# virtuoso/clap

Hardware: AMD Instinct MI355X
Metric: entity updates/sec (transform hierarchy + inverse + AABB + frustum cull + visible list) (higher is better)
Workload: dtype f32; 1 GPU; BASELINE configs[1]: 1000000 entities/GPU, 125000 chains x depth 8, tiles SoA layout, all dirty, fused frustum cull + ordered visible list (303309 visible); entities_per_gpu=1000000, levels=8, particles_per_gpu=0, exchange=none

## Files before the change

### clap_amd/_lib.py

```python
import ctypes as C
import os
import subprocess

_HERE = os.path.dirname(os.path.abspath(__file__))
LIB_PATH = os.environ.get("CLAPGPU_LIB") or os.path.join(_HERE, "lib", "libclapgpu.so")
CSRC = os.path.join(_HERE, "csrc")
ABI_VERSION = 34

OK = 0
ERR_NOMEM = -1
ERR_INVALID_ARGUMENTS = -2
ERR_NOT_SUPPORTED = -3
ERR_TOO_LARGE = -11
ERR_INIT_FAILED = -14
ERR_OUT_OF_BOUNDS = -26
ERR_UNKNOWN = -32

E_VISIBLE = 1 << 0
E_SKIP_CULLING = 1 << 14
E_DIRTY = 1 << 16
E_JOINT_ATTACHED = 1 << 17
E_ALIVE = 1 << 31
RAY_INVALID = 1 << 0
RAY_UNRESOLVED = 1 << 1
RAY_MOVED_TARGET = 1 << 2
UPDATE_ALL_DIRTY = 1 << 0

_ERR_NAMES = {ERR_NOMEM: "NOMEM", ERR_INVALID_ARGUMENTS: "INVALID_ARGUMENTS", ERR_NOT_SUPPORTED: "NOT_SUPPORTED",
              ERR_TOO_LARGE: "TOO_LARGE", ERR_INIT_FAILED: "INITIALIZATION_FAILED",
              ERR_OUT_OF_BOUNDS: "OUT_OF_BOUNDS", ERR_UNKNOWN: "UNKNOWN_ERROR"}


class ClapGpuError(RuntimeError):
    def __init__(self, code, where, detail=""):
        self.code = code
        super().__init__(f"{where}: CERR_{_ERR_NAMES.get(code, code)} ({code}) {detail}".rstrip())


class Frustum(C.Structure):
    _fields_ = [("planes", C.c_float * 24), ("corners", C.c_float * 32)]


class BvQuery(C.Structure):
    _fields_ = [("cam_pos", C.c_float * 3), ("has_ctl", C.c_uint32), ("ctl_pos", C.c_float * 3),
                ("ctl_entity", C.c_uint32), ("result", C.c_void_p), ("inside_mask", C.c_void_p)]


EXTRA_VIEWS_MAX = 4


class Views(C.Structure):
    _fields_ = [("n", C.c_uint32), ("pad", C.c_uint32), ("frustum", Frustum * EXTRA_VIEWS_MAX),
                ("vis_mask", C.c_void_p * EXTRA_VIEWS_MAX), ("vis_row_pop", C.c_void_p * EXTRA_VIEWS_MAX),
                ("host_vis_mask", C.c_void_p * EXTRA_VIEWS_MAX)]


class Entities(C.Structure):
    _fields_ = [("n", C.c_uint32), ("n_models", C.c_uint32),
                ("pos_scale", C.c_void_p), ("rot", C.c_void_p), ("parent", C.c_void_p),
                ("model", C.c_void_p), ("model_table", C.c_void_p), ("flags", C.c_void_p),
                ("seqs", C.c_void_p), ("mx", C.c_void_p), ("inv_mx", C.c_void_p),
                ("aabb", C.c_void_p), ("center", C.c_void_p), ("vis_mask", C.c_void_p),
                ("vis_row_pop", C.c_void_p), ("n_attach", C.c_uint32), ("pad", C.c_uint32),
                ("attach", C.c_void_p), ("jt_pool", C.c_void_p), ("bind_pool", C.c_void_p),
                ("attach_local", C.c_void_p), ("bv", C.POINTER(BvQuery)), ("rebuilt_mask", C.c_void_p),
                ("views", C.POINTER(Views))]


class Particles(C.Structure):
    _fields_ = [("n", C.c_uint32), ("n_sys", C.c_uint32), ("sys", C.c_void_p), ("row_sys", C.c_void_p),
                ("pos", C.c_void_p), ("vel", C.c_void_p), ("rng_state", C.c_void_p),
                ("billboard_mx", C.c_void_p), ("respawn_mask", C.c_void_p), ("respawn_row_pop", C.c_void_p),
                ("respawn_list", C.c_void_p), ("respawn_count", C.c_void_p), ("scratch", C.c_void_p),
                ("respawn_groups", C.c_void_p)]


class AnimClock(C.Structure):
    _fields_ = [("n_chars", C.c_uint32), ("n_anims", C.c_uint32), ("anim", C.c_void_p), ("time_end", C.c_void_p),
                ("ani_time", C.c_void_p), ("speed", C.c_void_p), ("restart", C.c_void_p), ("frame_time", C.c_void_p),
                ("ended", C.c_void_p)]


class Skeleton(C.Structure):
    _fields_ = [("nr_joints", C.c_uint32), ("n_levels", C.c_uint32), ("parent", C.c_void_p), ("depth", C.c_void_p),
                ("root_pose", C.c_void_p), ("invmx", C.c_void_p), ("bind", C.c_void_p)]


class Animations(C.Structure):
    _fields_ = [("n_anims", C.c_uint32), ("n_times", C.c_uint32), ("chan_table", C.c_void_p),
                ("times", C.c_void_p), ("data", C.c_void_p), ("packed", C.c_void_p), ("packed_keys", C.c_uint32),
                ("packed_layout", C.c_uint32), ("n_data", C.c_uint32), ("pad", C.c_uint32)]


class PoseBatch(C.Structure):
    _fields_ = [("n_chars", C.c_uint32), ("skip", C.c_uint32), ("anim", C.c_void_p), ("frame_time", C.c_void_p), ("entity", C.c_void_p),
                ("entity_mx", C.c_void_p), ("trs", C.c_void_p), ("joint_transforms", C.c_void_p),
                ("joint_pos", C.c_void_p)]


class SkinBatch(C.Structure):
    _fields_ = [("n_chars", C.c_uint32), ("nr_joints", C.c_uint32), ("vert_first", C.c_void_p),
                ("vert_count", C.c_void_p), ("out_first", C.c_void_p), ("position", C.c_void_p),
                ("normal", C.c_void_p), ("joints", C.c_void_p), ("weights", C.c_void_p),
                ("joint_transforms", C.c_void_p), ("out_position", C.c_void_p), ("out_normal", C.c_void_p),
                ("out_w", C.c_void_p)]


class World(C.Structure):
    _fields_ = [("gravity", C.c_double * 3), ("linear_damping", C.c_double),
                ("linear_damping_threshold_sq", C.c_double), ("adis_linear_threshold_sq", C.c_double),
                ("adis_angular_threshold_sq", C.c_double), ("adis_time", C.c_double),
                ("adis_steps", C.c_int32), ("pad", C.c_int32)]


class Bodies(C.Structure):
    _fields_ = [("n", C.c_uint32), ("adis_average_samples", C.c_uint32), ("pos", C.c_void_p), ("quat", C.c_void_p),
                ("lvel", C.c_void_p), ("avel", C.c_void_p), ("mass", C.c_void_p), ("radius", C.c_void_p),
                ("yoffset", C.c_void_p), ("bflags", C.c_void_p), ("adis_steps_left", C.c_void_p),
                ("adis_time_left", C.c_void_p), ("body_entity", C.c_void_p),
                ("length", C.c_void_p), ("inertia", C.c_void_p), ("geom_offset_R", C.c_double * 12),
                ("aabb", C.c_void_p), ("axis", C.c_void_p), ("adis_samples", C.c_void_p), ("adis_counter", C.c_void_p),
                ("geom_records", C.c_void_p)]


class Geoms(C.Structure):
    _fields_ = [("n", C.c_uint32), ("pad", C.c_uint32), ("pos", C.c_void_p), ("axis", C.c_void_p),
                ("radius", C.c_void_p), ("length", C.c_void_p), ("kind", C.c_void_p), ("aabb", C.c_void_p),
                ("material", C.c_void_p), ("records", C.c_void_p)]


class TrimeshDesc(C.Structure):
    _fields_ = [("n_meshes", C.c_uint32), ("n_statics", C.c_uint32), ("static_index", C.c_void_p), ("vx_first", C.c_void_p),
                ("tri_first", C.c_void_p), ("vx", C.c_void_p), ("idx", C.c_void_p), ("scale", C.c_void_p),
                ("pos", C.c_void_p), ("quat", C.c_void_p)]


POSE_SKIP_TRS, POSE_SKIP_JOINT_POS, POSE_JOINT_POS_MODEL = 1, 2, 4
BODY_DISABLED, BODY_AUTO_DISABLE, BODY_NO_GRAVITY, BODY_GYROSCOPIC, BODY_HAS_JOINT = 1, 2, 4, 8, 16
GEOM_SPHERE, GEOM_CAPSULE, GEOM_BOX, GEOM_OTHER = 0, 1, 2, 3
CONTACT_DEEP = 0x80000000


def mesh_contact_scratch(static_capacity):
    return (int(static_capacity) + 63) // 64 + 1


class Characters(C.Structure):
    _fields_ = [("n", C.c_uint32), ("limbo_height", C.c_float), ("entity", C.c_void_p), ("body", C.c_void_p),
                ("hist_pos", C.c_void_p), ("hist_head", C.c_void_p), ("hist_wrapped", C.c_void_p),
                ("airborne", C.c_void_p), ("moved", C.c_void_p)]


class Lights(C.Structure):
    _fields_ = [("nr_lights", C.c_uint32), ("pad", C.c_uint32), ("pos", C.c_void_p), ("color", C.c_void_p),
                ("attenuation", C.c_void_p), ("is_dir", C.c_void_p), ("active", C.c_void_p)]


class Frame(C.Structure):
    _fields_ = [("entities", C.POINTER(Entities)), ("tile_row_start", C.c_void_p), ("n_tiles", C.c_uint32),
                ("level_start", C.c_void_p), ("n_levels", C.c_uint32), ("frustum", C.POINTER(Frustum)),
                ("bodies", C.POINTER(Bodies)), ("world", C.POINTER(World)), ("bp", C.c_void_p),
                ("pairs", C.c_void_p), ("pair_capacity", C.c_uint32), ("pair_total", C.c_void_p),
                ("static_pairs", C.c_void_p), ("static_pair_capacity", C.c_uint32), ("static_pair_total", C.c_void_p),
                ("body_geoms", C.POINTER(Geoms)), ("static_geoms", C.POINTER(Geoms)),
                ("contacts", C.c_void_p), ("static_contacts", C.c_void_p),
                ("contact_total", C.c_void_p), ("static_contact_total", C.c_void_p),
                ("n_body_links", C.c_uint32), ("link_body", C.c_void_p), ("link_entity", C.c_void_p),
                ("characters", C.POINTER(Characters)),
                ("lights", C.POINTER(Lights)),
                ("n_light_carriers", C.c_uint32), ("carrier_entity", C.c_void_p), ("carrier_light", C.c_void_p),
                ("carrier_offset", C.c_void_p),
                ("light_width", C.c_uint32), ("light_height", C.c_uint32), ("light_cell", C.c_uint32), ("light_tiles", C.c_void_p),
                ("view_mx", C.POINTER(C.c_float)), ("proj_mx", C.POINTER(C.c_float)),
                ("anim_clock", C.POINTER(AnimClock)), ("now_dev", C.c_void_p),
                ("skeleton", C.POINTER(Skeleton)), ("animations", C.POINTER(Animations)), ("pose", C.POINTER(PoseBatch)),
                ("skin", C.POINTER(SkinBatch)),
                ("particles", C.POINTER(Particles)),
                ("index_base", C.c_uint32), ("visible", C.c_void_p), ("visible_count", C.c_void_p), ("visible_scratch", C.c_void_p),
                ("cam_pos", C.c_float * 3), ("force_lod", C.c_void_p), ("cur_lod", C.c_void_p), ("draw_lod", C.c_void_p),
                ("flags", C.c_uint32),
                ("meshes", C.c_void_p), ("mesh_contacts", C.c_void_p), ("mesh_ref", C.c_void_p),
                ("mesh_contact_capacity", C.c_uint32), ("mesh_contact_total", C.c_void_p), ("mesh_capped", C.c_void_p),
                ("mesh_scratch", C.c_void_p)]


LIGHTS_MAX = 128


SYMBOLS = {
    "clapgpu_device_count": (C.c_int, []),
    "clapgpu_init": (C.c_int, [C.c_int]),
    "clapgpu_last_error": (C.c_char_p, []),
    "clapgpu_test_fail_after": (None, [C.c_int]),
    "clapgpu_abi_version": (C.c_uint32, []),
    "clapgpu_malloc": (C.c_int, [C.POINTER(C.c_void_p), C.c_size_t]),
    "clapgpu_free": (C.c_int, [C.c_void_p]),
    "clapgpu_host_malloc": (C.c_int, [C.POINTER(C.c_void_p), C.c_size_t]),
    "clapgpu_host_free": (C.c_int, [C.c_void_p]),
    "clapgpu_memcpy_h2d": (C.c_int, [C.c_void_p, C.c_void_p, C.c_size_t, C.c_void_p]),
    "clapgpu_memcpy_d2h": (C.c_int, [C.c_void_p, C.c_void_p, C.c_size_t, C.c_void_p]),
    "clapgpu_memset": (C.c_int, [C.c_void_p, C.c_int, C.c_size_t, C.c_void_p]),
    "clapgpu_stream_sync": (C.c_int, [C.c_void_p]),
    "clapgpu_view_matrix": (None, [C.POINTER(C.c_float), C.POINTER(C.c_float), C.POINTER(C.c_float)]),
    "clapgpu_perspective": (None, [C.c_float, C.c_float, C.c_float, C.c_float, C.c_int, C.POINTER(C.c_float)]),
    "clapgpu_frustum_calc": (None, [C.POINTER(C.c_float), C.POINTER(C.c_float), C.c_int, C.POINTER(Frustum)]),
    "clapgpu_entities_update": (C.c_int, [C.c_void_p, C.POINTER(Entities), C.POINTER(C.c_uint32), C.c_uint32,
                                          C.c_uint32, C.POINTER(Frustum)]),
    "clapgpu_entities_update_level": (C.c_int, [C.c_void_p, C.POINTER(Entities), C.c_uint32, C.c_uint32,
                                                C.c_uint32, C.POINTER(Frustum)]),
    "clapgpu_entities_update_tiles": (C.c_int, [C.c_void_p, C.POINTER(Entities), C.c_void_p, C.c_uint32,
                                                C.c_uint32, C.POINTER(Frustum)]),
    "clapgpu_entities_lod": (C.c_int, [C.c_void_p, C.POINTER(Entities), C.c_void_p, C.c_void_p, C.c_uint32,
                                       C.POINTER(C.c_float), C.c_void_p, C.c_void_p, C.c_void_p]),
    "clapgpu_entities_cull": (C.c_int, [C.c_void_p, C.POINTER(Entities), C.POINTER(Frustum)]),
    "clapgpu_visible_scratch_bytes": (C.c_size_t, [C.c_uint32]),
    "clapgpu_visible_compact": (C.c_int, [C.c_void_p, C.c_void_p, C.c_void_p, C.c_uint32, C.c_uint32, C.c_void_p,
                                          C.c_void_p, C.c_void_p]),
    "clapgpu_animation_time": (C.c_int, [C.c_void_p, C.POINTER(AnimClock), C.c_double]),
    "clapgpu_animation_time_dev": (C.c_int, [C.c_void_p, C.POINTER(AnimClock), C.c_void_p]),
    "clapgpu_animations_packed_bytes": (C.c_size_t, [C.c_uint32, C.c_uint32, C.c_uint32]),
    "clapgpu_animations_pack": (C.c_int, [C.c_void_p, C.POINTER(Animations), C.c_uint32, C.c_uint32, C.c_void_p, C.POINTER(C.c_uint32)]),
    "clapgpu_joint_pos_world": (C.c_int, [C.c_void_p, C.POINTER(Skeleton), C.POINTER(PoseBatch)]),
    "clapgpu_pose_update": (C.c_int, [C.c_void_p, C.POINTER(Skeleton), C.POINTER(Animations), C.POINTER(PoseBatch)]),
    "clapgpu_skin": (C.c_int, [C.c_void_p, C.POINTER(SkinBatch)]),
    "clapgpu_phys_step_schedule": (C.c_int, [C.POINTER(C.c_double), C.c_double]),
    "clapgpu_world_defaults": (None, [C.POINTER(World)]),
    "clapgpu_bodies_step": (C.c_int, [C.c_void_p, C.POINTER(Bodies), C.POINTER(World), C.c_double]),
    "clapgpu_phys_body_update": (C.c_int, [C.c_void_p, C.POINTER(Bodies), C.c_uint32, C.c_void_p, C.c_void_p, C.c_void_p,
                                           C.c_void_p]),
    "clapgpu_geom_offset_rotation": (None, [C.POINTER(C.c_double)]),
    "clapgpu_mass_sphere_total": (None, [C.c_double, C.c_double, C.POINTER(C.c_double)]),
    "clapgpu_mass_capsule_total": (None, [C.c_double, C.c_int, C.c_double, C.c_double, C.POINTER(C.c_double)]),
    "clapgpu_capsule_geom": (None, [C.c_float, C.c_float, C.c_float, C.c_double, C.c_double, C.POINTER(C.c_float),
                                    C.POINTER(C.c_float), C.POINTER(C.c_float), C.POINTER(C.c_int), C.POINTER(C.c_float)]),
    "clapgpu_bodies_aabb": (C.c_int, [C.c_void_p, C.POINTER(Bodies)]),
    "clapgpu_bp_create": (C.c_int, [C.POINTER(C.c_void_p), C.c_uint32, C.c_double, C.c_uint32, C.c_void_p]),
    "clapgpu_bp_destroy": (None, [C.c_void_p]),
    "clapgpu_bp_collide": (C.c_int, [C.c_void_p, C.c_void_p, C.c_uint32, C.c_void_p, C.c_void_p, C.c_uint32, C.c_void_p,
                                     C.c_void_p, C.c_uint32, C.c_void_p]),
    "clapgpu_bp_status": (C.c_int, [C.c_void_p, C.c_void_p, C.POINTER(C.c_uint32)]),
    "clapgpu_bp_static_aabb": (C.c_void_p, [C.c_void_p]),
    "clapgpu_contacts_geoms": (C.c_int, [C.c_void_p, C.POINTER(Geoms), C.POINTER(Geoms), C.c_void_p, C.c_void_p, C.c_uint32,
                                         C.c_void_p, C.c_void_p, C.c_void_p, C.c_void_p]),
    "clapgpu_contacts_geoms_both": (C.c_int, [C.c_void_p, C.c_void_p, C.POINTER(Geoms), C.POINTER(Geoms), C.c_void_p, C.c_void_p,
                                              C.c_uint32, C.c_void_p, C.c_void_p, C.c_void_p, C.c_void_p, C.c_uint32, C.c_void_p,
                                              C.c_void_p, C.c_void_p]),
    "clapgpu_sweep_capsules": (C.c_int, [C.c_void_p, C.POINTER(Geoms), C.POINTER(Geoms), C.c_uint32, C.c_void_p, C.c_void_p,
                                         C.c_void_p, C.c_void_p, C.c_void_p, C.c_void_p, C.c_void_p]),
    "clapgpu_bodies_rotate_from_entities": (C.c_int, [C.c_void_p, C.POINTER(Bodies), C.POINTER(Entities), C.c_uint32,
                                                      C.c_uint32, C.c_void_p, C.c_void_p]),
    "clapgpu_contacts_spheres": (C.c_int, [C.c_void_p, C.POINTER(Bodies), C.c_void_p, C.c_void_p, C.c_uint32,
                                           C.c_void_p, C.c_void_p, C.c_void_p]),
    "clapgpu_contacts_sphere_box": (C.c_int, [C.c_void_p, C.POINTER(Bodies), C.c_uint32, C.c_void_p, C.c_void_p,
                                              C.c_void_p, C.c_uint32, C.c_void_p, C.c_void_p, C.c_void_p, C.c_void_p]),
    "clapgpu_shard_tile_range": (C.c_int, [C.c_void_p, C.c_uint32, C.c_uint32, C.c_uint32, C.POINTER(C.c_uint32),
                                           C.POINTER(C.c_uint32)]),
    "clapgpu_bodies_step_prebin": (C.c_int, [C.c_void_p, C.POINTER(Bodies), C.POINTER(World), C.c_double, C.c_void_p]),
    "clapgpu_bp_invalidate": (C.c_int, [C.c_void_p, C.c_void_p]),
    "clapgpu_bp_index": (C.c_int, [C.c_void_p, C.c_void_p, C.c_uint32, C.c_void_p]),
    "clapgpu_bp_index_status": (C.c_int, [C.c_void_p, C.c_void_p, C.POINTER(C.c_uint32)]),
    "clapgpu_ray_cast": (C.c_int, [C.c_void_p, C.c_void_p, C.POINTER(Geoms), C.POINTER(Geoms), C.c_uint32, C.c_void_p,
                                   C.c_void_p, C.c_void_p, C.c_void_p, C.c_void_p, C.c_void_p]),
    "clapgpu_bodies_ground_collide": (C.c_int, [C.c_void_p, C.c_void_p, C.POINTER(Bodies), C.POINTER(Geoms), C.c_uint32,
                                                C.c_void_p, C.c_void_p, C.c_void_p, C.c_void_p, C.c_void_p, C.c_void_p,
                                                C.c_void_p, C.c_void_p, C.c_void_p]),
    "clapgpu_trimesh_create": (C.c_int, [C.c_void_p, C.POINTER(C.c_void_p), C.POINTER(TrimeshDesc)]),
    "clapgpu_trimesh_pose": (C.c_int, [C.c_void_p, C.c_void_p, C.c_void_p, C.c_void_p]),
    "clapgpu_trimesh_status": (C.c_int, [C.c_void_p, C.c_void_p, C.POINTER(C.c_uint32), C.POINTER(C.c_uint32)]),
    "clapgpu_trimesh_destroy": (None, [C.c_void_p]),
    "clapgpu_ray_cast_meshes": (C.c_int, [C.c_void_p, C.c_void_p, C.POINTER(Geoms), C.POINTER(Geoms), C.c_void_p, C.c_uint32,
                                          C.c_void_p, C.c_void_p, C.c_void_p, C.c_void_p, C.c_void_p, C.c_void_p]),
    "clapgpu_bodies_ground_collide_meshes": (C.c_int, [C.c_void_p, C.c_void_p, C.POINTER(Bodies), C.POINTER(Geoms), C.c_void_p,
                                                       C.c_uint32, C.c_void_p, C.c_void_p, C.c_void_p, C.c_void_p, C.c_void_p,
                                                       C.c_void_p, C.c_void_p, C.c_void_p, C.c_void_p]),
    "clapgpu_contacts_meshes": (C.c_int, [C.c_void_p, C.POINTER(Geoms), C.POINTER(Geoms), C.c_void_p, C.c_void_p, C.c_void_p,
                                          C.c_uint32, C.c_void_p, C.c_uint32, C.c_void_p, C.c_void_p, C.c_void_p, C.c_void_p,
                                          C.c_void_p]),
    "clapgpu_sweep_capsules_meshes": (C.c_int, [C.c_void_p, C.POINTER(Geoms), C.POINTER(Geoms), C.c_void_p, C.c_uint32, C.c_void_p,
                                                C.c_void_p, C.c_void_p, C.c_void_p, C.c_void_p, C.c_void_p, C.c_void_p]),
    "clapgpu_visible_compact_lod": (C.c_int, [C.c_void_p, C.c_void_p, C.c_uint32, C.c_void_p, C.c_void_p, C.c_void_p, C.c_void_p,
                                              C.c_void_p, C.c_void_p, C.c_void_p]),
    "clapgpu_characters_update_clock": (C.c_int, [C.c_void_p, C.c_void_p, C.c_void_p, C.c_void_p, C.c_void_p, C.c_double, C.c_void_p]),
    "clapgpu_host_malloc_mapped": (C.c_int, [C.POINTER(C.c_void_p), C.POINTER(C.c_void_p), C.c_size_t]),
    "clapgpu_entities_apply_inputs": (C.c_int, [C.c_void_p, C.c_void_p, C.c_void_p, C.c_uint32]),
    "clapgpu_entities_place": (C.c_int, [C.c_void_p, C.c_void_p, C.c_void_p, C.c_uint32, C.c_void_p]),
    "clapgpu_entities_export_rebuilt": (C.c_int, [C.c_void_p, C.c_void_p, C.c_void_p]),
    "clapgpu_entities_export_rows": (C.c_int, [C.c_void_p, C.c_void_p, C.c_void_p, C.c_void_p]),
    "clapgpu_entities_update_tiles_hostio": (C.c_int, [C.c_void_p, C.c_void_p, C.c_void_p, C.c_uint32, C.c_uint32, C.c_void_p,
                                                       C.c_void_p]),
    "clapgpu_wait_word": (C.c_int, [C.c_void_p, C.c_uint32, C.c_void_p]),
    "clapgpu_exchange_set_library": (None, [C.c_char_p]),
    "clapgpu_exchange_available": (C.c_int, []),
    "clapgpu_exchange_unique_id": (C.c_int, [C.c_void_p]),
    "clapgpu_exchange_create": (C.c_int, [C.POINTER(C.c_void_p), C.c_void_p, C.c_int, C.c_int]),
    "clapgpu_exchange_info": (C.c_int, [C.c_void_p, C.POINTER(C.c_int), C.POINTER(C.c_int), C.c_char_p]),
    "clapgpu_exchange_destroy": (None, [C.c_void_p]),
    "clapgpu_exchange_visible": (C.c_int, [C.c_void_p, C.c_void_p, C.c_void_p, C.c_uint32, C.c_void_p, C.c_void_p, C.c_void_p,
                                           C.c_void_p]),
    "clapgpu_exchange_visible_ranges": (C.c_int, [C.c_void_p, C.c_void_p, C.c_void_p, C.c_uint32, C.c_void_p, C.c_void_p, C.c_void_p,
                                                  C.c_void_p, C.c_void_p, C.c_void_p]),
    "clapgpu_visible_compact_ranges": (C.c_int, [C.c_void_p, C.c_void_p, C.c_uint32, C.c_uint32, C.c_void_p, C.c_void_p, C.c_void_p,
                                                 C.c_void_p, C.c_void_p]),
    "clapgpu_visible_expand_ranges_host": (C.c_uint32, [C.c_void_p, C.c_uint32, C.c_uint32, C.c_void_p, C.c_void_p, C.c_void_p, C.c_uint32]),
    "clapgpu_shard_bases": (C.c_int, [C.c_void_p, C.c_uint32, C.c_uint32, C.c_void_p, C.c_void_p, C.POINTER(C.c_uint32)]),
    "clapgpu_mat4_invert": (None, [C.POINTER(C.c_float), C.POINTER(C.c_float)]),
    "clapgpu_mat4_from_quat": (None, [C.POINTER(C.c_float), C.POINTER(C.c_float)]),
    "clapgpu_frame_issue": (C.c_int, [C.c_void_p, C.POINTER(Frame), C.c_double, C.c_uint32]),
    "clapgpu_particles_update": (C.c_int, [C.c_void_p, C.POINTER(Particles), C.POINTER(C.c_float)]),
    "clapgpu_characters_update": (C.c_int, [C.c_void_p, C.POINTER(Characters), C.POINTER(Entities),
                                            C.POINTER(Bodies)]),
    "clapgpu_light_grid_dims": (None, [C.c_uint32, C.c_uint32, C.c_uint32, C.POINTER(C.c_uint32),
                                       C.POINTER(C.c_uint32)]),
    "clapgpu_light_grid_compute": (C.c_int, [C.c_void_p, C.POINTER(Lights), C.POINTER(C.c_float),
                                             C.POINTER(C.c_float), C.c_uint32, C.c_uint32, C.c_uint32, C.c_void_p]),
    "clapgpu_lights_from_entities": (C.c_int, [C.c_void_p, C.POINTER(Entities), C.c_uint32, C.c_uint32, C.c_void_p,
                                               C.c_void_p, C.c_void_p, C.POINTER(Lights)]),
}

_lib = None


def build(verbose=False):
    subprocess.run(["make", "-C", CSRC] + ([] if verbose else ["-s"]), check=True)


def lib():
    global _lib
    if _lib is None:
        if not os.path.exists(LIB_PATH):
            raise ClapGpuError(ERR_INIT_FAILED, "clap_amd",
                               f"{LIB_PATH} is missing: run `python -c 'import __graft_entry__ as g; g.build()'` "
                               "(there is no CPU fallback)")
        try:
            import torch
        except ImportError:
            pass
        L = C.CDLL(LIB_PATH)
        for name, (res, args) in SYMBOLS.items():
            fn = getattr(L, name)
            fn.restype = res
            fn.argtypes = args
        got = L.clapgpu_abi_version()
        if got & 0x80000000 and os.environ.get("CLAPGPU_ALLOW_EXPERIMENT") == "1":
            got &= 0x7FFFFFFF
        if got != ABI_VERSION:
            raise ClapGpuError(ERR_INIT_FAILED, "clap_amd",
                               "libclapgpu ABI version mismatch; rebuild" if not got & 0x80000000 else
                               "libclapgpu is an EXPERIMENT build (-DCLAPGPU_EXPERIMENT: kernels compiled with parts "
                               "switched off); rebuild without EXTRA=, or set CLAPGPU_ALLOW_EXPERIMENT=1 for an A/B run")
        _lib = L
    return _lib


def check(rc, where):
    if rc != OK:
        detail = lib().clapgpu_last_error()
        raise ClapGpuError(rc, where, detail.decode() if detail else "")
```

### clap_amd/csrc/entities.hip

```cpp
#include <string.h>
#include <math.h>
#include <type_traits>
#include "common.h"
#include "lm_dev.h"
#include "entities_row.h"

namespace clapgpu {

template <bool CULL, bool XV = false>
__device__ __forceinline__ void process_row_fast(const EntK &e, const RowIn &in, float4 *tile, const float4 *mt,
                                                 const int lane, const uint32_t row_first, const uint32_t mode,
                                                 const lmd::FrustumK &fr, const int src, const uint32_t parent_seq_now,
                                                 float (&carry_mx)[16], uint32_t &carry_seq, const XViewsK *xv = nullptr)
{
    const uint32_t i = row_first + lane;
    const uint32_t fl = in.fl;
    const int32_t p = in.p;
    uint32_t seq = in.sq & 0xffffu, pseq = in.sq >> 16;
    float pm[16];
#pragma unroll
    for (int k = 0; k < 16; k++) pm[k] = __shfl(carry_mx[k], src);
    if (p >= 0) pseq = parent_seq_now;

    const float4 lo = mt[2 * in.mi], hi = mt[2 * in.mi + 1];
    float mx[16], inv[16], bb[6], ctr[3], local_mx[16];
    lmd::trs(local_mx, in.ps.x, in.ps.y, in.ps.z, in.ps.w, in.q.x, in.q.y, in.q.z, in.q.w);
    if (p >= 0) {
        lmd::mul(mx, pm, local_mx);
    } else {
#pragma unroll
        for (int k = 0; k < 16; k++) mx[k] = local_mx[k];
    }
#ifdef CLAPGPU_EXP_NO_INVERT
#pragma unroll
    for (int k = 0; k < 16; k++) inv[k] = mx[k];
#else
    lmd::invert(inv, mx);
#endif
#ifdef CLAPGPU_EXP_NO_AABB
#pragma unroll
    for (int k = 0; k < 6; k++) bb[k] = mx[12 + k % 3] + (k < 3 ? lo.x : hi.x);
#pragma unroll
    for (int k = 0; k < 3; k++) ctr[k] = mx[12 + k];
#else
    lmd::world_aabb(bb, ctr, mx, lo.x, lo.y, lo.z, hi.x, hi.y, hi.z);
#endif
    seq = (seq + 1) & 0xffffu;
#pragma unroll
    for (int k = 0; k < 16; k++) carry_mx[k] = mx[k];
    carry_seq = seq;

    const size_t e0 = row_first;
    float4 *tile_a = tile, *tile_b = tile + 256;
    float *tile_f = reinterpret_cast<float *>(tile);
    float4 va[4], vb[4];
    stage_mat4(tile_a, mx, lane);
    stage_mat4(tile_b, inv, lane);
    wave_lds_fence();
    unstage_mat4(tile_a, va, lane);
    unstage_mat4(tile_b, vb, lane);
    store_mat4_rows(e.mx + 16 * e0, va, lane, WAVE);
    store_mat4_rows(e.inv_mx + 16 * e0, vb, lane, WAVE);
    e.seqs[i] = seq | (pseq << 16);
    wave_lds_fence();
    stage_rows<6>(tile_f, bb, lane);
    wave_lds_fence();
    {
        float *ab = e.aabb + 6 * e0;
        store_stream(&reinterpret_cast<float4 *>(ab)[lane], reinterpret_cast<const float4 *>(tile_f)[lane]);
        const float2 t2 = reinterpret_cast<const float2 *>(tile_f + 4 * WAVE)[lane];
        const clapgpu_f2 v2 = { t2.x, t2.y };
        const clapgpu_f3 v3 = { ctr[0], ctr[1], ctr[2] };
#ifdef CLAPGPU_PLAIN_STORES
        reinterpret_cast<clapgpu_f2 *>(ab + 4 * WAVE)[lane] = v2;
        *reinterpret_cast<clapgpu_f3 *>(e.center + 3 * (e0 + lane)) = v3;
#else
        __builtin_nontemporal_store(v2, reinterpret_cast<clapgpu_f2 *>(ab + 4 * WAVE) + lane);
        __builtin_nontemporal_store(v3, reinterpret_cast<clapgpu_f3 *>(e.center + 3 * (e0 + lane)));
#endif
    }
    wave_lds_fence();
    if (!(mode & CLAPGPU_UPDATE_ALL_DIRTY) && (fl & CLAPGPU_E_DIRTY))
        e.flags[i] = fl & ~CLAPGPU_E_DIRTY;
    if (e.rebuilt_mask && lane == 0) e.rebuilt_mask[row_first >> 6] = ~0ull;
    if (CULL) {
        bool vis = (fl & CLAPGPU_E_VISIBLE) != 0;
        if (vis && !(fl & CLAPGPU_E_SKIP_CULLING))
            vis = lmd::aabb_in_frustum_fast(fr, bb);
        const uint64_t m = __ballot(vis);
        e.vis_mask[e0 >> 6] = m;
        e.vis_row_pop[e0 >> 6] = (uint8_t)__popcll(m);
        if constexpr (XV) cull_extra_views(*xv, (fl & CLAPGPU_E_VISIBLE) != 0, fl, bb, (uint32_t)(e0 >> 6), lane);
    }
}

__global__ __launch_bounds__(ENT_BLOCK)
void k_attach_prepare(EntK e)
{
    const uint32_t k = blockIdx.x * ENT_BLOCK + threadIdx.x;
    if (k >= e.n_attach) return;
    const clapgpu_attach at = e.attach[k];
    const float4 ps = e.pos_scale[at.entity], q = e.rot[at.entity];
    float local_mx[16], jt[16], bd[16], joint_mx[16], out[16];
    lmd::trs(local_mx, ps.x, ps.y, ps.z, ps.w, q.x, q.y, q.z, q.w);
    load_mat4(jt, e.jt_pool + 16 * (size_t)at.jt);
    load_mat4(bd, e.bind_pool + 16 * (size_t)at.bind);
    lmd::mul(joint_mx, jt, bd);
    lmd::mul(out, joint_mx, local_mx);
    float4 *d = reinterpret_cast<float4 *>(e.attach_local + 16 * (size_t)k);
#pragma unroll
    for (int c = 0; c < 4; c++)
        d[c] = make_float4(out[4 * c], out[4 * c + 1], out[4 * c + 2], out[4 * c + 3]);
}


template <bool CULL>
__global__ __launch_bounds__(ENT_BLOCK)
void k_entities_level(EntK e, uint32_t first, uint32_t count, uint32_t mode, lmd::FrustumK fr)
{
    __shared__ float4 lds_tiles[ENT_BLOCK / WAVE][LDS_F4_PER_WAVE];
    const int lane = lane_id();
    const int wave = threadIdx.x / WAVE;
    const uint32_t wave_local0 = blockIdx.x * ENT_BLOCK + wave * WAVE;
    if (wave_local0 >= count)
        return;
    const uint32_t row_count = count - wave_local0 < WAVE ? count - wave_local0 : WAVE;
    float carry_mx[16];
    uint32_t carry_seq = 0;
    bool carry_valid = false;
    const RowIn in = load_row(e, lane, first + wave_local0, row_count);
    process_row<CULL, false>(e, in, lds_tiles[wave], lane, first + wave_local0, row_count, mode, fr,
                             false, 0, carry_mx, carry_seq, carry_valid);
}

constexpr int ENT_MT_CAP = 256;
constexpr int ENT_TILE_WAVES = 1;
template <bool CULL>
__global__ __launch_bounds__(ENT_BLOCK, ENT_TILE_WAVES)
void k_entities_tiles(lmd::FrustumK fr_arg, EntK e, const uint32_t *tile_row_start, uint32_t n_tiles, uint32_t n,
                      uint32_t mode)
{
#define TILES_XV 0
#define TILES_XV_PTR nullptr
#include "entities_tiles_body.inc"
#undef TILES_XV
#undef TILES_XV_PTR
}

__global__ __launch_bounds__(ENT_BLOCK, ENT_TILE_WAVES)
void k_entities_tiles_xv(lmd::FrustumK fr_arg, EntK e, const uint32_t *tile_row_start, uint32_t n_tiles, uint32_t n,
                         uint32_t mode, XViewsK xv)
{
    constexpr bool CULL = true;
#define TILES_XV 1
#define TILES_XV_PTR (&xv)
#include "entities_tiles_body.inc"
#undef TILES_XV
#undef TILES_XV_PTR
}

__global__ __launch_bounds__(ENT_BLOCK)
void k_entities_level_xv(EntK e, uint32_t first, uint32_t count, uint32_t mode, lmd::FrustumK fr, XViewsK xv)
{
    __shared__ float4 lds_tiles[ENT_BLOCK / WAVE][LDS_F4_PER_WAVE];
    const int lane = lane_id();
    const int wave = threadIdx.x / WAVE;
    const uint32_t wave_local0 = blockIdx.x * ENT_BLOCK + wave * WAVE;
    if (wave_local0 >= count)
        return;
    const uint32_t row_count = count - wave_local0 < WAVE ? count - wave_local0 : WAVE;
    float carry_mx[16];
    uint32_t carry_seq = 0;
    bool carry_valid = false;
    const RowIn in = load_row(e, lane, first + wave_local0, row_count);
    process_row<true, false, false, true>(e, in, lds_tiles[wave], lane, first + wave_local0, row_count, mode, fr,
                                          false, 0, carry_mx, carry_seq, carry_valid, nullptr, nullptr, &xv);
}

__global__ __launch_bounds__(ENT_BLOCK)
void k_entities_cull_xv(const uint32_t *flags, const float *aabb, uint64_t *vis_mask, uint8_t *vis_row_pop,
                        uint32_t n, lmd::FrustumK fr, XViewsK xv)
{
    const uint32_t i = blockIdx.x * ENT_BLOCK + threadIdx.x;
    const int lane = lane_id();
    bool base = false, vis = false;
    uint32_t fl = 0;
    float bb[6] = { 0, 0, 0, 0, 0, 0 };
    if (i < n) {
        fl = flags[i];
        base = (fl & CLAPGPU_E_ALIVE) && (fl & CLAPGPU_E_VISIBLE);
        vis = base;
        if (base && !(fl & CLAPGPU_E_SKIP_CULLING)) {
#pragma unroll
            for (int k = 0; k < 6; k++) bb[k] = aabb[6 * (size_t)i + k];
            vis = lmd::aabb_in_frustum_fast(fr, bb);
        }
    }
    if ((i - lane) >= n) return;
    const uint64_t m = __ballot(vis);
    if (lane == 0) {
        vis_mask[i >> 6] = m;
        vis_row_pop[i >> 6] = (uint8_t)__popcll(m);
    }
    cull_extra_views(xv, base, fl, bb, i >> 6, lane);
}

__global__ __launch_bounds__(ENT_BLOCK)
void k_entities_cull(const uint32_t *flags, const float *aabb, uint64_t *vis_mask, uint8_t *vis_row_pop,
                     uint32_t n, lmd::FrustumK fr)
{
    const uint32_t i = blockIdx.x * ENT_BLOCK + threadIdx.x;
    bool vis = false;
    if (i < n) {
        const uint32_t fl = flags[i];
        vis = (fl & CLAPGPU_E_ALIVE) && (fl & CLAPGPU_E_VISIBLE);
        if (vis && !(fl & CLAPGPU_E_SKIP_CULLING)) {
            float bb[6];
#pragma unroll
            for (int k = 0; k < 6; k++) bb[k] = aabb[6 * (size_t)i + k];
            vis = lmd::aabb_in_frustum_fast(fr, bb);
        }
    }
    const uint64_t m = __ballot(vis);
    if (lane_id() == 0 && (i - lane_id()) < n) {
        vis_mask[i >> 6] = m;
        vis_row_pop[i >> 6] = (uint8_t)__popcll(m);
    }
}

constexpr int GROUP_WORDS = 64;

__device__ __forceinline__ uint64_t load_mask_word(const uint64_t *vis_mask, uint32_t w, uint32_t n)
{
    const uint32_t nwords = (n + 63) / 64;
    if (w >= nwords)
        return 0;
    uint64_t v = vis_mask[w];
    const uint32_t rem = n - w * 64;
    if (rem < 64)
        v &= (1ull << rem) - 1ull;
    return v;
}

__device__ __forceinline__ uint32_t wave_sum(uint32_t v)
{
#pragma unroll
    for (int off = 32; off > 0; off >>= 1)
        v += __shfl_xor(v, off);
    return v;
}

__global__ __launch_bounds__(WAVE)
void k_mask_group_count(const uint64_t *vis_mask, uint32_t n, uint32_t *group_count)
{
    const uint32_t w = blockIdx.x * GROUP_WORDS + threadIdx.x;
    const uint32_t c = wave_sum(__popcll(load_mask_word(vis_mask, w, n)));
    if (threadIdx.x == 0)
        group_count[blockIdx.x] = c;
}

__global__ __launch_bounds__(WAVE)
void k_visible_expand(const uint64_t *vis_mask, uint32_t n, const uint32_t *group_count,
                      uint32_t n_groups, uint32_t index_base, uint32_t *visible, uint32_t *count)
{
    const int lane = threadIdx.x;
    const uint32_t g = blockIdx.x;

    uint32_t pre = 0;
    for (uint32_t j = lane; j < g; j += WAVE)
        pre += group_count[j];
    pre = wave_sum(pre);

    const uint64_t word = load_mask_word(vis_mask, g * GROUP_WORDS + lane, n);
    const uint32_t cnt = __popcll(word);
    uint32_t incl = cnt;
#pragma unroll
    for (int off = 1; off < WAVE; off <<= 1) {
        uint32_t t = __shfl_up(incl, off);
        if (lane >= off) incl += t;
    }
    const uint32_t excl = incl - cnt;

    for (int k = 0; k < GROUP_WORDS; k++) {
        const uint64_t wk = __shfl(word, k);
        if (wk == 0) continue;
        const uint32_t base = pre + __shfl(excl, k);
        if ((wk >> lane) & 1ull) {
            const uint32_t rank = __popcll(wk & ((1ull << lane) - 1ull));
            visible[base + rank] = index_base + (g * GROUP_WORDS + k) * 64u + lane;
        }
    }
    if (g == n_groups - 1 && lane == WAVE - 1)
        *count = pre + incl;
}

constexpr int MAX_SEGMENTS = 64;
struct SegK { uint32_t cap_words, n_seg; uint32_t base[MAX_SEGMENTS], n_words[MAX_SEGMENTS]; };

__device__ __forceinline__ uint64_t load_seg_word(const uint64_t *mask, const SegK &sg, uint32_t w, uint32_t *id_base)
{
    const uint32_t r = w / sg.cap_words, lw = w - r * sg.cap_words;
    if (r >= sg.n_seg || lw >= sg.n_words[r]) { *id_base = 0; return 0ull; }
    *id_base = sg.base[r] + lw * 64u;
    return mask[w];
}

__global__ __launch_bounds__(WAVE)
void k_mask_group_count_seg(const uint64_t *mask, SegK sg, uint32_t *group_count)
{
    uint32_t idb;
    const uint32_t c = wave_sum(__popcll(load_seg_word(mask, sg, blockIdx.x * GROUP_WORDS + threadIdx.x, &idb)));
    if (threadIdx.x == 0)
        group_count[blockIdx.x] = c;
}

__global__ __launch_bounds__(WAVE)
void k_visible_expand_seg(const uint64_t *mask, SegK sg, const uint32_t *group_count, uint32_t n_groups, uint32_t *visible,
                          uint32_t *count)
{
    const int lane = threadIdx.x;
    const uint32_t g = blockIdx.x;
    uint32_t pre = 0;
    for (uint32_t j = lane; j < g; j += WAVE)
        pre += group_count[j];
    pre = wave_sum(pre);
    uint32_t idb;
    const uint64_t word = load_seg_word(mask, sg, g * GROUP_WORDS + lane, &idb);
    const uint32_t cnt = __popcll(word);
    uint32_t incl = cnt;
#pragma unroll
    for (int off = 1; off < WAVE; off <<= 1) {
        uint32_t t = __shfl_up(incl, off);
        if (lane >= off) incl += t;
    }
    const uint32_t excl = incl - cnt;
    for (int k = 0; k < GROUP_WORDS; k++) {
        const uint64_t wk = __shfl(word, k);
        if (wk == 0) continue;
        const uint32_t base = pre + __shfl(excl, k), ids = __shfl(idb, k);
        if ((wk >> lane) & 1ull) {
            const uint32_t rank = __popcll(wk & ((1ull << lane) - 1ull));
            visible[base + rank] = ids + lane;
        }
    }
    if (g == n_groups - 1 && lane == WAVE - 1)
        *count = pre + incl;
}

constexpr int RP_ROWS = 16;
constexpr uint32_t RP_MAX_ROWS = 1u << 16;

__device__ __forceinline__ uint32_t sum_bytes(uint32_t v, uint32_t acc)
{
    return __builtin_amdgcn_sad_u8(v, 0u, acc);
}

__global__ __launch_bounds__(ENT_BLOCK)
void k_visible_expand_rp(const uint64_t *vis_mask, const uint8_t *row_pop, uint32_t n,
                         uint32_t index_base, uint32_t *visible, uint32_t *count)
{
    const int lane = lane_id();
    const uint32_t g = blockIdx.x * (ENT_BLOCK / WAVE) + threadIdx.x / WAVE;
    const uint32_t n_rows = (n + 63) / 64;
    const uint32_t row0 = g * RP_ROWS;
    if (row0 >= n_rows)
        return;

    const uint32_t pre = wave_byte_sum(row_pop, row0, lane);

    const uint64_t word = lane < RP_ROWS ? load_mask_word(vis_mask, row0 + lane, n) : 0ull;
    const uint32_t cnt = __popcll(word);
    uint32_t incl = cnt;
#pragma unroll
    for (int off = 1; off < RP_ROWS; off <<= 1) {
        uint32_t t = __shfl_up(incl, off);
        if (lane >= off) incl += t;
    }
    const uint32_t excl = incl - cnt;
    const uint32_t lo = (uint32_t)word, hi = (uint32_t)(word >> 32);

#pragma unroll
    for (int k = 0; k < RP_ROWS; k++) {
        const uint64_t wk = (uint64_t)(uint32_t)__builtin_amdgcn_readlane(lo, k) |
                            ((uint64_t)(uint32_t)__builtin_amdgcn_readlane(hi, k) << 32);
        if (wk == 0) continue;
        const uint32_t base = pre + (uint32_t)__builtin_amdgcn_readlane(excl, k);
        if ((wk >> lane) & 1ull) {
            const uint32_t rank = __popcll(wk & ((1ull << lane) - 1ull));
            visible[base + rank] = index_base + (row0 + k) * 64u + lane;
        }
    }
    if (row0 + RP_ROWS >= n_rows && lane == RP_ROWS - 1)
        *count = pre + incl;
}

__device__ __forceinline__ float cbrtf_glibc(float x)
{
    int xe;
    const float xm = frexpf(fabsf(x), &xe);
    if (xe == 0 && (x == 0.0f || x != x || isinf(x)))
        return x + x;
    const float u = (float)(0.492659620528969547 + (0.697570460207922770 - 0.191502161678719066 * (double)xm) * (double)xm);
    const float t2 = u * u * u;
    const int r = xe % 3;
    const double f = r == -2 ? 1.0 / 1.5874010519681994748 : r == -1 ? 1.0 / 1.2599210498948731648
                   : r == 0 ? 1.0 : r == 1 ? 1.2599210498948731648 : 1.5874010519681994748;
    const float ym = (float)((double)u * ((double)t2 + 2.0 * (double)xm) / (2.0 * (double)t2 + (double)xm) * f);
    return ldexpf(x > 0.0f ? ym : -ym, xe / 3);
}

struct LodK {
    float cx, cy, cz;
    const float *aabb, *center;
    const float4 *pos_scale;
    const int32_t *model;
    const float4 *model_table;
    const int32_t *force_lod;
    int32_t *cur_lod;
    uint32_t n_models;
};

__device__ __forceinline__ int32_t lod_pick(const LodK &k, uint32_t i)
{
    int32_t lod = k.cur_lod[i];
    const int32_t forced = k.force_lod ? k.force_lod[i] : -1;
    if (forced >= 0) {
        lod = forced;
    } else {
        const float *b = k.aabb + 6 * (size_t)i;
        const bool inside = k.cx >= b[0] && k.cx <= b[3] && k.cy >= b[1] && k.cy <= b[4] && k.cz >= b[2] && k.cz <= b[5];
        if (!inside) {
            const float *c = k.center + 3 * (size_t)i;
            const float dx = c[0] - k.cx, dy = c[1] - k.cy, dz = c[2] - k.cz;
            float dd = 0.f;
            dd += dx * dx;
            dd += dy * dy;
            dd += dz * dz;
            const int32_t mraw = k.model[i];
            const int32_t mi = (uint32_t)mraw < k.n_models ? mraw : 0;
            const float4 lo = k.model_table[2 * mi], hi = k.model_table[2 * mi + 1];
            const float s = k.pos_scale[i].w;
            const float X = fabsf(hi.x - lo.x) * s, Y = fabsf(hi.y - lo.y) * s, Z = fabsf(hi.z - lo.z) * s;
            const float side = cbrtf_glibc(X * Y * Z);
            const float scale = (float)((double)fabsf(dd - side * side) / 3600.0);
            const uint32_t lm = __float_as_uint(hi.w);
            const int lmin = (int)(lm & 0xffu), lmax = (int)((lm >> 8) & 0xffu);
            const int req = (int)scale;
            lod = req < lmin ? lmin : (req > lmax ? lmax : req);
        }
    }
    k.cur_lod[i] = lod;
    return lod;
}

__global__ __launch_bounds__(ENT_BLOCK)
void k_entities_lod(const uint32_t *visible, const uint32_t *count, uint32_t index_base, LodK lk, int32_t *draw_lod, uint32_t n)
{
    const uint32_t total = *count < n ? *count : n;
    for (uint32_t k = blockIdx.x * ENT_BLOCK + threadIdx.x; k < total; k += gridDim.x * ENT_BLOCK) {
// ... 5 lines not shown

__global__ __launch_bounds__(ENT_BLOCK)
void k_entities_apply_inputs(float4 *pos_scale, float4 *rot, uint32_t *flags, const clapgpu_entity_input *list,
                             uint32_t n_list, uint32_t n)
{
    const uint32_t k = blockIdx.x * ENT_BLOCK + threadIdx.x;
    if (k >= n_list) return;
    const uint32_t *r = reinterpret_cast<const uint32_t *>(list + k);
    const uint2 h = *reinterpret_cast<const uint2 *>(r);
    const uint32_t slot = h.x;
    if (slot >= n) return;
    const uint2 a = *reinterpret_cast<const uint2 *>(r + 2), b = *reinterpret_cast<const uint2 *>(r + 4);
    const uint2 c = *reinterpret_cast<const uint2 *>(r + 6), d = *reinterpret_cast<const uint2 *>(r + 8);
    pos_scale[slot] = make_float4(__uint_as_float(a.x), __uint_as_float(a.y), __uint_as_float(b.x), __uint_as_float(b.y));
    rot[slot] = make_float4(__uint_as_float(c.x), __uint_as_float(c.y), __uint_as_float(d.x), __uint_as_float(d.y));
    flags[slot] = h.y;
}

__global__ __launch_bounds__(WAVE)
void k_entities_place(int32_t *parent, int32_t *model, float *aabb, float *center, const clapgpu_entity_place *list, uint32_t n_list,
                      uint32_t n, unsigned long long *stale)
{
    const uint32_t k = blockIdx.x * WAVE + threadIdx.x;
    if (k >= n_list) return;
    const uint4 r = *reinterpret_cast<const uint4 *>(list + k);
    const uint32_t slot = r.x;
    if (slot >= n) return;
    parent[slot] = (int32_t)r.y;
    model[slot] = (int32_t)r.z;
    if ((r.w & CLAPGPU_PLACE_CLEAR_STALE) && stale)
        atomicAnd(&stale[slot >> 6], ~(1ull << (slot & 63)));
    if (r.w & CLAPGPU_PLACE_ZERO_BOX) {
        float2 *b = reinterpret_cast<float2 *>(aabb + 6 * (size_t)slot);
        b[0] = b[1] = b[2] = make_float2(0.f, 0.f);
        float *c = center + 3 * (size_t)slot;
        c[0] = c[1] = c[2] = 0.f;
    }
}

struct ExportK {
    const float *mx, *inv_mx, *aabb, *center;
    const uint64_t *vis_mask, *rebuilt_mask, *inside_mask;
    const uint64_t *select;
    uint64_t *stale;
    float *o_mx, *o_inv, *o_aabb, *o_center;
    uint64_t *o_vis, *o_rebuilt, *o_inside;
    uint32_t *counter, *done, done_value, n_rows;
};

__global__ __launch_bounds__(ENT_BLOCK)
void k_entities_export_rebuilt(ExportK x)
{
    const int lane = lane_id();
    const uint32_t row = blockIdx.x * (ENT_BLOCK / WAVE) + threadIdx.x / WAVE;
    if (row < x.n_rows) {
        const uint64_t m = x.select ? x.select[row] : x.rebuilt_mask[row];
        if (lane == 0 && x.select && x.stale && m) x.stale[row] &= ~m;
        if (lane == 0 && !x.select) {
            x.o_rebuilt[row] = m;
            if (x.vis_mask) x.o_vis[row] = x.vis_mask[row];
            if (x.o_inside) x.o_inside[row] = x.inside_mask ? x.inside_mask[row] : 0ull;
        }
        if ((m >> lane) & 1ull) {
            const size_t i = (size_t)row * WAVE + lane;
            const float4 *a = reinterpret_cast<const float4 *>(x.mx + 16 * i), *b = reinterpret_cast<const float4 *>(x.inv_mx + 16 * i);
            float4 *oa = reinterpret_cast<float4 *>(x.o_mx + 16 * i), *ob = reinterpret_cast<float4 *>(x.o_inv + 16 * i);
            const float4 a0 = a[0], a1 = a[1], a2 = a[2], a3 = a[3], b0 = b[0], b1 = b[1], b2 = b[2], b3 = b[3];
            const float2 *bb = reinterpret_cast<const float2 *>(x.aabb + 6 * i);
            const float2 c0 = bb[0], c1 = bb[1], c2 = bb[2];
            const float *ct = x.center + 3 * i;
            const float t0 = ct[0], t1 = ct[1], t2 = ct[2];
            oa[0] = a0; oa[1] = a1; oa[2] = a2; oa[3] = a3;
            ob[0] = b0; ob[1] = b1; ob[2] = b2; ob[3] = b3;
            float2 *obb = reinterpret_cast<float2 *>(x.o_aabb + 6 * i);
            obb[0] = c0; obb[1] = c1; obb[2] = c2;
            float *oc = x.o_center + 3 * i;
            oc[0] = t0; oc[1] = t1; oc[2] = t2;
        }
    }
    __threadfence_system();
    __syncthreads();
    if (threadIdx.x == 0) {
        const uint32_t arrived = atomicAdd(x.counter, 1u);
        if (arrived == gridDim.x - 1) {
            *x.counter = 0;
            __threadfence_system();
            __hip_atomic_store(x.done, x.done_value, __ATOMIC_RELEASE, __HIP_MEMORY_SCOPE_SYSTEM);
        }
    }
}

template <class F> struct first_param;
template <class R, class A0, class... A> struct first_param<R (*)(A0, A...)> { using type = A0; };
static_assert(std::is_same<first_param<decltype(&k_entities_tiles<true>)>::type, lmd::FrustumK>::value &&
              std::is_same<first_param<decltype(&k_entities_tiles<false>)>::type, lmd::FrustumK>::value,
              "k_entities_tiles: the frustum must stay the first kernel argument (it is read at kernarg offset 0)");
static_assert(std::is_same<first_param<decltype(&k_entities_tiles_xv)>::type, lmd::FrustumK>::value, "k_entities_tiles_xv: the same");
static_assert(alignof(lmd::FrustumK) <= 8, "kernarg offset 0 holds for any alignment the segment start guarantees");

}

using namespace clapgpu;

static EntK to_kernel_args(const clapgpu_entities *e)
{
    EntK k;
    k.pos_scale = reinterpret_cast<const float4 *>(e->pos_scale);
    k.rot = reinterpret_cast<const float4 *>(e->rot);
    k.parent = e->parent;
    k.model = e->model;
    k.model_table = reinterpret_cast<const float4 *>(e->model_table);
    k.flags = e->flags;
    k.seqs = e->seqs;
    k.mx = e->mx;
    k.inv_mx = e->inv_mx;
    k.aabb = e->aabb;
    k.center = e->center;
    k.vis_mask = e->vis_mask;
    k.vis_row_pop = e->vis_row_pop;
    k.n_attach = (e->attach && e->jt_pool && e->bind_pool && e->attach_local) ? e->n_attach : 0;
    k.attach = e->attach;
    k.attach_local = e->attach_local;
    k.jt_pool = e->jt_pool;
    k.bind_pool = e->bind_pool;
    k.n = e->n;
    k.n_models = e->n_models ? e->n_models : 1;
    k.bv_result = nullptr;
    k.bv_inside = nullptr;
    k.rebuilt_mask = e->rebuilt_mask;
    k.bv_has_ctl = k.bv_ctl_entity = k.bv_on = 0;
    for (int a = 0; a < 3; a++) k.bv_cam[a] = k.bv_ctl[a] = 0.f;
    if (e->bv && (e->bv->result || e->bv->inside_mask)) {
        k.bv_on = 1;
        memcpy(k.bv_cam, e->bv->cam_pos, 12);
        memcpy(k.bv_ctl, e->bv->ctl_pos, 12);
        k.bv_has_ctl = e->bv->has_ctl;
        k.bv_ctl_entity = e->bv->ctl_entity;
        k.bv_result = reinterpret_cast<unsigned long long *>(e->bv->result);
        k.bv_inside = e->bv->inside_mask;
    }
    return k;
}

static lmd::FrustumK make_frustum_k(const clapgpu_frustum *frustum)
{
    static_assert(sizeof(lmd::Frustum) == sizeof(clapgpu_frustum), "frustum layout");
    lmd::FrustumK k = {};
    if (!frustum)
        return k;
    memcpy(&k.f, frustum, sizeof(k.f));
    for (int ax = 0; ax < 3; ax++) {
        float lo = INFINITY, hi = -INFINITY;
        bool nan = false;
        for (int i = 0; i < 8; i++) {
            const float c = k.f.corners[i][ax];
            nan = nan || (c != c);
            lo = c < lo ? c : lo;
            hi = c > hi ? c : hi;
        }
        k.cmin[ax] = nan ? NAN : lo;
        k.cmax[ax] = nan ? NAN : hi;
    }
    k.finite = 1;
    for (int i = 0; i < 6; i++)
        for (int c = 0; c < 4; c++)
            if (!(fabsf(k.f.planes[i][c]) <= 3.402823466e+38f))
                k.finite = 0;
    return k;
}

static bool aligned16(const void *p) { return (reinterpret_cast<uintptr_t>(p) & 15u) == 0; }

namespace clapgpu {
bool make_xviews_k(const clapgpu_entities *e, bool hostio, XViewsK *out)
{
    memset(out, 0, sizeof(*out));
    const clapgpu_views *v = e->views;
    if (!v || !v->n) return true;
    if (v->n > CLAPGPU_EXTRA_VIEWS_MAX) return false;
    out->n = v->n;
    for (uint32_t k = 0; k < v->n; k++) {
        if (!v->vis_mask[k] || !v->vis_row_pop[k]) return false;
        out->mask[k] = v->vis_mask[k]; out->pop[k] = v->vis_row_pop[k];
        out->o_mask[k] = hostio ? v->host_vis_mask[k] : nullptr;
        out->fr[k] = make_frustum_k(&v->frustum[k]);
    }
    return true;
}
}

static int check_entities(const clapgpu_entities *e, bool need_mask)
{
    if (!e || !e->pos_scale || !e->rot || !e->parent || !e->model || !e->model_table || !e->flags ||
        !e->seqs || !e->mx || !e->inv_mx || !e->aabb || !e->center)
        return CLAPGPU_ERR_INVALID_ARGUMENTS;
    if (need_mask && (!e->vis_mask || !e->vis_row_pop))
        return CLAPGPU_ERR_INVALID_ARGUMENTS;
    if (!aligned16(e->pos_scale) || !aligned16(e->rot) || !aligned16(e->model_table) || !aligned16(e->mx) ||
        !aligned16(e->inv_mx) || !aligned16(e->aabb) || !aligned16(e->center))
        return CLAPGPU_ERR_INVALID_ARGUMENTS;
    return CLAPGPU_OK;
}

static int prepare_attachments(void *stream, const EntK &k)
{
    if (!k.n_attach)
        return CLAPGPU_OK;
    hipLaunchKernelGGL(k_attach_prepare, dim3((k.n_attach + ENT_BLOCK - 1) / ENT_BLOCK), dim3(ENT_BLOCK), 0,
                       as_stream(stream), k);
    CLAPGPU_LAUNCH_CHECK("k_attach_prepare");
    return CLAPGPU_OK;
}

static int launch_level(void *stream, const EntK &k, uint32_t first, uint32_t count, uint32_t mode,
                        const clapgpu_frustum *frustum, const XViewsK &xv)
{
    const lmd::FrustumK fr = make_frustum_k(frustum);
    const dim3 grid((count + ENT_BLOCK - 1) / ENT_BLOCK), block(ENT_BLOCK);
    if (frustum && xv.n)
        hipLaunchKernelGGL(k_entities_level_xv, grid, block, 0, as_stream(stream), k, first, count, mode, fr, xv);
    else if (frustum)
        hipLaunchKernelGGL(k_entities_level<true>, grid, block, 0, as_stream(stream), k, first, count, mode, fr);
    else
        hipLaunchKernelGGL(k_entities_level<false>, grid, block, 0, as_stream(stream), k, first, count, mode, fr);
    CLAPGPU_LAUNCH_CHECK("k_entities_level");
    return CLAPGPU_OK;
}

extern "C" int clapgpu_entities_update_level(void *stream, const clapgpu_entities *e,
                                             uint32_t first, uint32_t count,
                                             uint32_t mode, const clapgpu_frustum *frustum)
{
    int rc = check_entities(e, frustum != nullptr);
    if (rc) return rc;
    if (first & 63u)
        return CLAPGPU_ERR_INVALID_ARGUMENTS;
    if (first > e->n || count > e->n - first)
        return CLAPGPU_ERR_OUT_OF_BOUNDS;
    if (!count)
        return CLAPGPU_OK;
    const EntK k = to_kernel_args(e);
    XViewsK xv;
    if (!make_xviews_k(e, false, &xv)) return CLAPGPU_ERR_INVALID_ARGUMENTS;
    rc = prepare_attachments(stream, k);
    if (rc) return rc;
    return launch_level(stream, k, first, count, mode, frustum, xv);
}

extern "C" int clapgpu_entities_update(void *stream, const clapgpu_entities *e,
                                       const uint32_t *level_start, uint32_t n_levels,
                                       uint32_t mode, const clapgpu_frustum *frustum)
{
    int rc = check_entities(e, frustum != nullptr);
    if (rc) return rc;
    if (!level_start || (e->n && !n_levels))
        return CLAPGPU_ERR_INVALID_ARGUMENTS;
    if (e->n == 0)
        return CLAPGPU_OK;
    if (level_start[0] != 0 || level_start[n_levels] != e->n)
        return CLAPGPU_ERR_OUT_OF_BOUNDS;
    for (uint32_t l = 0; l < n_levels; l++)
        if (level_start[l] > level_start[l + 1] || (level_start[l] & 63u))
            return CLAPGPU_ERR_INVALID_ARGUMENTS;

    const EntK k = to_kernel_args(e);
    XViewsK xv;
    if (!make_xviews_k(e, false, &xv)) return CLAPGPU_ERR_INVALID_ARGUMENTS;
    if (k.bv_result)
        CLAPGPU_HIP(hipMemsetAsync(k.bv_result, 0, sizeof(uint64_t), as_stream(stream)));
    rc = prepare_attachments(stream, k);
    if (rc) return rc;
    for (uint32_t l = 0; l < n_levels; l++) {
        const uint32_t first = level_start[l], count = level_start[l + 1] - first;
        if (!count)
            continue;
        rc = launch_level(stream, k, first, count, mode, frustum, xv);
        if (rc) return rc;
    }
    return CLAPGPU_OK;
}

extern "C" int clapgpu_entities_update_tiles(void *stream, const clapgpu_entities *e,
                                             const uint32_t *tile_row_start, uint32_t n_tiles,
                                             uint32_t mode, const clapgpu_frustum *frustum)
{
    int rc = check_entities(e, frustum != nullptr);
    if (rc) return rc;
    if (e->n == 0 || n_tiles == 0)
        return CLAPGPU_OK;
    if (!tile_row_start)
        return CLAPGPU_ERR_INVALID_ARGUMENTS;
    const lmd::FrustumK fr = make_frustum_k(frustum);
    const EntK k = to_kernel_args(e);
    XViewsK xv;
    if (!make_xviews_k(e, false, &xv)) return CLAPGPU_ERR_INVALID_ARGUMENTS;
    if (k.bv_result)
        CLAPGPU_HIP(hipMemsetAsync(k.bv_result, 0, sizeof(uint64_t), as_stream(stream)));
    rc = prepare_attachments(stream, k);
    if (rc) return rc;
    const uint32_t per_block = ENT_BLOCK / WAVE;
    const dim3 grid((n_tiles + per_block - 1) / per_block), block(ENT_BLOCK);
    if (frustum && xv.n)
        hipLaunchKernelGGL(k_entities_tiles_xv, grid, block, 0, as_stream(stream), fr, k, tile_row_start, n_tiles, e->n, mode, xv);
    else if (frustum)
        hipLaunchKernelGGL(k_entities_tiles<true>, grid, block, 0, as_stream(stream), fr, k, tile_row_start, n_tiles,
                           e->n, mode);
    else
        hipLaunchKernelGGL(k_entities_tiles<false>, grid, block, 0, as_stream(stream), fr, k, tile_row_start, n_tiles,
                           e->n, mode);
    CLAPGPU_LAUNCH_CHECK("k_entities_tiles");
    return CLAPGPU_OK;
}

extern "C" int clapgpu_entities_cull(void *stream, const clapgpu_entities *e, const clapgpu_frustum *frustum)
{
    if (!e || !frustum || !e->flags || !e->aabb || !e->vis_mask || !e->vis_row_pop)
        return CLAPGPU_ERR_INVALID_ARGUMENTS;
    if (e->n == 0)
        return CLAPGPU_OK;
    const lmd::FrustumK fr = make_frustum_k(frustum);
    XViewsK xv;
    if (!make_xviews_k(e, false, &xv)) return CLAPGPU_ERR_INVALID_ARGUMENTS;
    const dim3 grid((e->n + ENT_BLOCK - 1) / ENT_BLOCK), block(ENT_BLOCK);
    if (xv.n)
        hipLaunchKernelGGL(k_entities_cull_xv, grid, block, 0, as_stream(stream), e->flags, e->aabb, e->vis_mask,
                           e->vis_row_pop, e->n, fr, xv);
    else
    hipLaunchKernelGGL(k_entities_cull, grid, block, 0, as_stream(stream), e->flags, e->aabb, e->vis_mask,
                       e->vis_row_pop, e->n, fr);
    CLAPGPU_LAUNCH_CHECK("k_entities_cull");
    return CLAPGPU_OK;
}

extern "C" int clapgpu_entities_apply_inputs(void *stream, const clapgpu_entities *e, const clapgpu_entity_input *list,
                                             uint32_t n_list)
{
    static_assert(sizeof(clapgpu_entity_input) == 40, "record layout");
    if (!e || !e->pos_scale || !e->rot || !e->flags || (n_list && !list))
        return CLAPGPU_ERR_INVALID_ARGUMENTS;
    if (!n_list || !e->n)
        return CLAPGPU_OK;
    hipLaunchKernelGGL(k_entities_apply_inputs, dim3((n_list + ENT_BLOCK - 1) / ENT_BLOCK), dim3(ENT_BLOCK), 0, as_stream(stream),
                       reinterpret_cast<float4 *>(const_cast<float *>(e->pos_scale)),
                       reinterpret_cast<float4 *>(const_cast<float *>(e->rot)), e->flags, list, n_list, e->n);
    CLAPGPU_LAUNCH_CHECK("k_entities_apply_inputs");
    return CLAPGPU_OK;
}

extern "C" int clapgpu_entities_place(void *stream, const clapgpu_entities *e, const clapgpu_entity_place *list, uint32_t n_list,
                                      uint64_t *stale_mask)
{
    if (!e || !e->parent || !e->model || !e->aabb || !e->center || (n_list && !list))
        return CLAPGPU_ERR_INVALID_ARGUMENTS;
    if (!n_list || !e->n)
        return CLAPGPU_OK;
    hipLaunchKernelGGL(k_entities_place, dim3((n_list + WAVE - 1) / WAVE), dim3(WAVE), 0, as_stream(stream),
                       const_cast<int32_t *>(e->parent), const_cast<int32_t *>(e->model), e->aabb, e->center, list, n_list, e->n,
                       reinterpret_cast<unsigned long long *>(stale_mask));
    CLAPGPU_LAUNCH_CHECK("k_entities_place");
    return CLAPGPU_OK;
}

extern "C" int clapgpu_entities_export_rebuilt(void *stream, const clapgpu_entities *e, const clapgpu_entities_export *x)
{
    if (!e || !x || !e->mx || !e->inv_mx || !e->aabb || !e->center || !e->rebuilt_mask || !x->mx || !x->inv_mx || !x->aabb ||
        !x->center || !x->rebuilt_mask || !x->counter || !x->done || (e->vis_mask && !x->vis_mask))
        return CLAPGPU_ERR_INVALID_ARGUMENTS;
    if (e->n & 63u)
        return CLAPGPU_ERR_INVALID_ARGUMENTS;
    ExportK k;
    k.mx = e->mx; k.inv_mx = e->inv_mx; k.aabb = e->aabb; k.center = e->center;
    k.vis_mask = e->vis_mask; k.rebuilt_mask = e->rebuilt_mask; k.select = nullptr; k.stale = nullptr;
    k.inside_mask = (e->bv && e->bv->inside_mask) ? e->bv->inside_mask : nullptr;
    k.o_mx = x->mx; k.o_inv = x->inv_mx; k.o_aabb = x->aabb; k.o_center = x->center;
    k.o_vis = x->vis_mask; k.o_rebuilt = x->rebuilt_mask; k.o_inside = x->inside_mask;
    k.counter = x->counter; k.done = x->done; k.done_value = x->done_value; k.n_rows = e->n / 64;
    const uint32_t per_block = ENT_BLOCK / WAVE;
    const uint32_t blocks = k.n_rows ? (k.n_rows + per_block - 1) / per_block : 1;
    hipLaunchKernelGGL(k_entities_export_rebuilt, dim3(blocks), dim3(ENT_BLOCK), 0, as_stream(stream), k);
    CLAPGPU_LAUNCH_CHECK("k_entities_export_rebuilt");
    return CLAPGPU_OK;
}

extern "C" int clapgpu_entities_export_rows(void *stream, const clapgpu_entities *e, const clapgpu_entities_export *x,
                                            const uint64_t *select_mask)
{
    if (!e || !x || !select_mask || !e->mx || !e->inv_mx || !e->aabb || !e->center || !x->mx || !x->inv_mx || !x->aabb ||
        !x->center || !x->counter || !x->done)
        return CLAPGPU_ERR_INVALID_ARGUMENTS;
    if (e->n & 63u)
        return CLAPGPU_ERR_INVALID_ARGUMENTS;
    ExportK k = {};
    k.mx = e->mx; k.inv_mx = e->inv_mx; k.aabb = e->aabb; k.center = e->center;
    k.select = select_mask; k.stale = x->stale_mask;
    k.o_mx = x->mx; k.o_inv = x->inv_mx; k.o_aabb = x->aabb; k.o_center = x->center;
    k.counter = x->counter; k.done = x->done; k.done_value = x->done_value; k.n_rows = e->n / 64;
    const uint32_t per_block = ENT_BLOCK / WAVE;
    const uint32_t blocks = k.n_rows ? (k.n_rows + per_block - 1) / per_block : 1;
    hipLaunchKernelGGL(k_entities_export_rebuilt, dim3(blocks), dim3(ENT_BLOCK), 0, as_stream(stream), k);
    CLAPGPU_LAUNCH_CHECK("k_entities_export_rows");
    return CLAPGPU_OK;
}

extern "C" int clapgpu_entities_update_tiles_hostio(void *stream, const clapgpu_entities *e,
                                                    const uint32_t *tile_row_start, uint32_t n_tiles, uint32_t mode,
                                                    const clapgpu_frustum *frustum, const clapgpu_entities_hostio *io)
{
    int rc = check_entities(e, frustum != nullptr);
    if (rc) return rc;
    if (!io || !io->mx || !io->inv_mx || !io->aabb || !io->center || !io->rebuilt_mask || !io->counter || !io->done ||
        (frustum && !io->vis_mask) || (io->touched && (!io->pos_scale || !io->rot || !io->flags)) || (n_tiles && !tile_row_start))
        return CLAPGPU_ERR_INVALID_ARGUMENTS;
    if (!aligned16(io->mx) || !aligned16(io->inv_mx) || (reinterpret_cast<uintptr_t>(io->aabb) & 7u) ||
        (io->touched && (!aligned16(io->pos_scale) || !aligned16(io->rot))))
        return CLAPGPU_ERR_INVALID_ARGUMENTS;
    const lmd::FrustumK fr = make_frustum_k(frustum);
    const EntK k = to_kernel_args(e);
    if (k.bv_result)
        CLAPGPU_HIP(hipMemsetAsync(k.bv_result, 0, sizeof(uint64_t), as_stream(stream)));
    rc = prepare_attachments(stream, k);
    if (rc) return rc;
    HostIO h;
    h.pos_scale = reinterpret_cast<const float4 *>(io->pos_scale); h.rot = reinterpret_cast<const float4 *>(io->rot);
    h.flags = io->flags; h.touched = io->touched;
    h.o_mx = io->mx; h.o_inv = io->inv_mx; h.o_aabb = io->aabb; h.o_center = io->center;
    h.o_vis = io->vis_mask; h.o_rebuilt = io->rebuilt_mask; h.o_inside = io->inside_mask;
    h.counter = io->counter; h.done = io->done; h.done_value = io->done_value;
    h.keep = io->keep_mask; h.o_exported = io->exported_mask; h.stale = io->stale_mask;
    h.late_ok = io->options & CLAPGPU_HOSTIO_EXPORT_STALE_READ;
    const uint32_t tiles = e->n ? n_tiles : 0;
    XViewsK xv;
    if (!make_xviews_k(e, true, &xv)) return CLAPGPU_ERR_INVALID_ARGUMENTS;
    rc = launch_entities_tiles_host(as_stream(stream), frustum != nullptr, fr, k, h, tile_row_start, tiles, e->n, mode, xv);
    if (rc) return rc;
    return CLAPGPU_OK;
}

extern "C" size_t clapgpu_visible_scratch_bytes(uint32_t n)
{
    const uint32_t n_groups = (n + GROUP_WORDS * 64 - 1) / (GROUP_WORDS * 64);
    return (size_t)(n_groups ? n_groups : 1) * sizeof(uint32_t);
}

extern "C" int clapgpu_visible_compact(void *stream, const uint64_t *vis_mask, const uint8_t *vis_row_pop,
                                       uint32_t n, uint32_t index_base, uint32_t *visible, uint32_t *count,
                                       void *scratch)
{
    if (!count || (n && (!vis_mask || !visible)))
        return CLAPGPU_ERR_INVALID_ARGUMENTS;
    if (n == 0) {
        CLAPGPU_HIP(hipMemsetAsync(count, 0, sizeof(uint32_t), as_stream(stream)));
        return CLAPGPU_OK;
    }
    const uint32_t n_rows = (n + 63) / 64;
    if (vis_row_pop && n_rows <= RP_MAX_ROWS && aligned16(vis_row_pop)) {
        const uint32_t waves = (n_rows + RP_ROWS - 1) / RP_ROWS, per_block = ENT_BLOCK / WAVE;
        hipLaunchKernelGGL(k_visible_expand_rp, dim3((waves + per_block - 1) / per_block), dim3(ENT_BLOCK), 0,
                           as_stream(stream), vis_mask, vis_row_pop, n, index_base, visible, count);
        CLAPGPU_LAUNCH_CHECK("k_visible_expand_rp");
        return CLAPGPU_OK;
    }
    if (!scratch)
        return CLAPGPU_ERR_INVALID_ARGUMENTS;
    const uint32_t n_groups = (n + GROUP_WORDS * 64 - 1) / (GROUP_WORDS * 64);
    uint32_t *group_count = static_cast<uint32_t *>(scratch);
    hipLaunchKernelGGL(k_mask_group_count, dim3(n_groups), dim3(WAVE), 0, as_stream(stream), vis_mask, n, group_count);
    CLAPGPU_LAUNCH_CHECK("k_mask_group_count");
    hipLaunchKernelGGL(k_visible_expand, dim3(n_groups), dim3(WAVE), 0, as_stream(stream), vis_mask, n,
                       group_count, n_groups, index_base, visible, count);
    CLAPGPU_LAUNCH_CHECK("k_visible_expand");
    return CLAPGPU_OK;
}

static int check_ranges(uint32_t n_ranges, uint32_t cap_pad, const uint32_t *base, const uint32_t *n_pad)
{
    if (!n_ranges || n_ranges > (uint32_t)MAX_SEGMENTS || !cap_pad || (cap_pad & 63u) || !base) return CLAPGPU_ERR_INVALID_ARGUMENTS;
    uint64_t end = 0;
    for (uint32_t r = 0; r < n_ranges; r++) {
        const uint32_t np = n_pad ? n_pad[r] : cap_pad;
        if ((np & 63u) || np > cap_pad || (base[r] & 63u) || base[r] < end) return CLAPGPU_ERR_INVALID_ARGUMENTS;
        end = (uint64_t)base[r] + np;
        if (end > 0xffffffffull) return CLAPGPU_ERR_TOO_LARGE;
    }
    return CLAPGPU_OK;
}

extern "C" int clapgpu_visible_compact_ranges(void *stream, const uint64_t *gathered_mask, uint32_t n_ranges, uint32_t cap_pad,
                                              const uint32_t *base, const uint32_t *n_pad, uint32_t *visible, uint32_t *count,
                                              void *scratch)
{
    if (!gathered_mask || !visible || !count || !scratch) return CLAPGPU_ERR_INVALID_ARGUMENTS;
    int rc = check_ranges(n_ranges, cap_pad, base, n_pad);
    if (rc) return rc;
    SegK sg = {};
    sg.cap_words = cap_pad / 64; sg.n_seg = n_ranges;
    for (uint32_t r = 0; r < n_ranges; r++) { sg.base[r] = base[r]; sg.n_words[r] = (n_pad ? n_pad[r] : cap_pad) / 64; }
    const uint64_t total_words = (uint64_t)sg.cap_words * n_ranges;
    if (total_words * 64 > 0xffffffffull) return CLAPGPU_ERR_TOO_LARGE;
    const uint32_t n_groups = (uint32_t)((total_words + GROUP_WORDS - 1) / GROUP_WORDS);
    uint32_t *group_count = static_cast<uint32_t *>(scratch);
    hipLaunchKernelGGL(k_mask_group_count_seg, dim3(n_groups), dim3(WAVE), 0, as_stream(stream), gathered_mask, sg, group_count);
    CLAPGPU_LAUNCH_CHECK("k_mask_group_count_seg");
    hipLaunchKernelGGL(k_visible_expand_seg, dim3(n_groups), dim3(WAVE), 0, as_stream(stream), gathered_mask, sg, group_count, n_groups,
                       visible, count);
    CLAPGPU_LAUNCH_CHECK("k_visible_expand_seg");
    return CLAPGPU_OK;
}

extern "C" uint32_t clapgpu_visible_expand_ranges_host(const uint64_t *gathered_mask, uint32_t n_ranges, uint32_t cap_pad,
                                                       const uint32_t *base, const uint32_t *n_pad, uint32_t *visible, uint32_t capacity)
{
    if (!gathered_mask || check_ranges(n_ranges, cap_pad, base, n_pad)) return 0;
    const uint32_t cap_words = cap_pad / 64;
    uint32_t cnt = 0;
    for (uint32_t r = 0; r < n_ranges; r++) {
        const uint32_t words = (n_pad ? n_pad[r] : cap_pad) / 64;
        for (uint32_t w = 0; w < words; w++) {
            uint64_t m = gathered_mask[(size_t)r * cap_words + w];
            while (m) {
                const uint32_t id = base[r] + w * 64u + (uint32_t)__builtin_ctzll(m);
                m &= m - 1;
                if (visible && cnt < capacity) visible[cnt] = id;
                cnt++;
            }
        }
    }
    return cnt;
}

static LodK lod_args(const clapgpu_entities *e, const float cam_pos[3], const int32_t *force_lod, int32_t *cur_lod)
{
    LodK k;
    k.cx = cam_pos[0]; k.cy = cam_pos[1]; k.cz = cam_pos[2];
    k.aabb = e->aabb; k.center = e->center;
    k.pos_scale = reinterpret_cast<const float4 *>(e->pos_scale);
    k.model = e->model;
    k.model_table = reinterpret_cast<const float4 *>(e->model_table);
    k.force_lod = force_lod; k.cur_lod = cur_lod;
    k.n_models = e->n_models ? e->n_models : 1;
    return k;
}

extern "C" int clapgpu_entities_lod(void *stream, const clapgpu_entities *e, const uint32_t *visible,
                                    const uint32_t *count, uint32_t index_base, const float cam_pos[3],
                                    const int32_t *force_lod, int32_t *cur_lod, int32_t *draw_lod)
{
    if (!e || !visible || !count || !cam_pos || !cur_lod || !draw_lod || !e->aabb || !e->center ||
        !e->pos_scale || !e->model || !e->model_table)
        return CLAPGPU_ERR_INVALID_ARGUMENTS;
    if (e->n == 0)
        return CLAPGPU_OK;
    uint32_t blocks = (e->n + ENT_BLOCK - 1) / ENT_BLOCK;
    if (blocks > 2048) blocks = 2048;
    hipLaunchKernelGGL(k_entities_lod, dim3(blocks), dim3(ENT_BLOCK), 0, as_stream(stream), visible, count, index_base,
                       lod_args(e, cam_pos, force_lod, cur_lod), draw_lod, e->n);
    CLAPGPU_LAUNCH_CHECK("k_entities_lod");
    return CLAPGPU_OK;
}

extern "C" int clapgpu_visible_compact_lod(void *stream, const clapgpu_entities *e, uint32_t index_base, const float cam_pos[3],
                                           const int32_t *force_lod, int32_t *cur_lod, uint32_t *visible, uint32_t *count,
                                           int32_t *draw_lod, void *scratch)
{
    if (!e || !count || !cam_pos || !cur_lod || !draw_lod || (e->n && (!e->vis_mask || !visible)) || !e->aabb || !e->center ||
        !e->pos_scale || !e->model || !e->model_table)
        return CLAPGPU_ERR_INVALID_ARGUMENTS;
    const uint32_t n = e->n;
    int rc = clapgpu_visible_compact(stream, e->vis_mask, e->vis_row_pop, n, index_base, visible, count, scratch);
    if (rc) return rc;
    return clapgpu_entities_lod(stream, e, visible, count, index_base, cam_pos, force_lod, cur_lod, draw_lod);
}
```

### clap_amd/csrc/entities_row.h

```cpp
#pragma once
#include <string.h>
#include <math.h>
#include "common.h"
#include "lm_dev.h"

namespace clapgpu {

struct EntK {
    const float4   *pos_scale;
    const float4   *rot;
    const int32_t  *parent;
    const int32_t  *model;
    const float4   *model_table;
    uint32_t       *flags;
    uint32_t       *seqs;
    float          *mx;
    float          *inv_mx;
    float          *aabb;
    float          *center;
    uint64_t       *vis_mask;
    uint8_t        *vis_row_pop;
    uint32_t        n_attach;
    const clapgpu_attach *attach;
    const float    *jt_pool;
    const float    *bind_pool;
    float          *attach_local;
    float           bv_cam[3], bv_ctl[3];
    uint32_t        bv_has_ctl, bv_ctl_entity, bv_on;
    unsigned long long *bv_result;
    uint64_t       *bv_inside;
    uint64_t       *rebuilt_mask;
    uint32_t        n, n_models;
};

struct XViewsK {
    uint32_t n, pad;
    uint64_t *mask[CLAPGPU_EXTRA_VIEWS_MAX];
    uint8_t  *pop[CLAPGPU_EXTRA_VIEWS_MAX];
    uint64_t *o_mask[CLAPGPU_EXTRA_VIEWS_MAX];
    lmd::FrustumK fr[CLAPGPU_EXTRA_VIEWS_MAX];
};

__device__ __forceinline__ bool extra_view_test(const lmd::FrustumK &k, const float (&bb)[6], const float (&lo)[3], const float (&hi)[3],
                                                const bool box_finite)
{
    if (!(k.finite && box_finite))
        return lmd::aabb_in_frustum(k.f, bb);
    bool in = true;
#pragma unroll
    for (int i = 0; i < 6; i++) {
        const float x = (k.f.planes[i][0] >= 0.f) ? hi[0] : lo[0];
        const float y = (k.f.planes[i][1] >= 0.f) ? hi[1] : lo[1];
        const float z = (k.f.planes[i][2] >= 0.f) ? hi[2] : lo[2];
        float p = 0.f;
        p += x * k.f.planes[i][0];
        p += y * k.f.planes[i][1];
        p += z * k.f.planes[i][2];
        p += 1.0f * k.f.planes[i][3];
        in = in & !(p < 0.0f);
    }
#pragma unroll
    for (int ax = 0; ax < 3; ax++)
        in = in & !(k.cmin[ax] > bb[3 + ax]) & !(k.cmax[ax] < bb[ax]);
    return in;
}

__device__ __forceinline__ uint64_t cull_extra_views(const XViewsK &xv, const bool base, const uint32_t fl, const float (&bb)[6],
                                                     const uint32_t word, const int lane)
{
    uint64_t any = 0;
    const float lo[3] = { fminf(bb[0], bb[3]), fminf(bb[1], bb[4]), fminf(bb[2], bb[5]) };
    const float hi[3] = { fmaxf(bb[0], bb[3]), fmaxf(bb[1], bb[4]), fmaxf(bb[2], bb[5]) };
    bool box_finite = true;
#pragma unroll
    for (int a = 0; a < 6; a++) box_finite = box_finite && (fabsf(bb[a]) <= 3.402823466e+38f);
    const bool tested = base && !(fl & CLAPGPU_E_SKIP_CULLING);
    for (uint32_t v = 0; v < xv.n; v++) {
        const bool vis = tested ? extra_view_test(xv.fr[v], bb, lo, hi, box_finite) : base;
        const uint64_t m = __ballot(vis);
        if (lane == 0) {
            xv.mask[v][word] = m;
            xv.pop[v][word] = (uint8_t)__popcll(m);
            if (xv.o_mask[v]) xv.o_mask[v][word] = m;
        }
        any |= m;
    }
    return any;
}

constexpr int ENT_BLOCK = 256;
constexpr int LDS_F4_PER_WAVE = 512;

__device__ __forceinline__ void load_mat4(float (&m)[16], const float *src)
{
    const float4 *p = reinterpret_cast<const float4 *>(src);
#pragma unroll
    for (int c = 0; c < 4; c++) {
        float4 v = p[c];
        m[4 * c] = v.x; m[4 * c + 1] = v.y; m[4 * c + 2] = v.z; m[4 * c + 3] = v.w;
    }
}

struct RowIn {
    uint32_t fl, sq;
    int32_t  p, mi;
    float4   ps, q;
};

__device__ __forceinline__ RowIn load_row(const EntK &e, const int lane, const uint32_t row_first,
                                          const uint32_t row_count)
{
    const uint32_t i = row_first + ((uint32_t)lane < row_count ? lane : 0);
    RowIn r;
    r.fl = e.flags[i];
    r.p = e.parent[i];
    r.sq = e.seqs[i];
    r.mi = e.model[i];
    if ((uint32_t)r.p >= e.n) r.p = -1;
    if ((uint32_t)r.mi >= e.n_models) r.mi = 0;
    r.ps = e.pos_scale[i];
    r.q = e.rot[i];
    return r;
}

struct HostIO {
    const float4   *pos_scale, *rot;
    const uint32_t *flags;
    const uint64_t *touched;
    uint64_t *stale;
    uint32_t late_ok;
    float          *o_mx, *o_inv, *o_aabb, *o_center;
    uint64_t       *o_vis, *o_rebuilt, *o_inside;
    uint32_t       *counter, *done, done_value;
    const uint64_t *keep;
    uint64_t       *o_exported;
};

__device__ __forceinline__ RowIn load_row_host(const EntK &e, const HostIO &h, const int lane, const uint32_t row_first,
                                               const uint32_t row_count, const uint64_t touched)
{
    RowIn r = load_row(e, lane, row_first, row_count);
    if ((uint32_t)lane < row_count && ((touched >> lane) & 1ull)) {
        const uint32_t i = row_first + lane;
        r.fl = h.flags[i];
        r.ps = h.pos_scale[i];
        r.q = h.rot[i];
    }
    return r;
}

struct RowPre {
    float2   bb0, bb1, bb2;
    float4   lo, hi;
    float4   pm[4];
    uint32_t pseq;
};

__device__ __forceinline__ void load_row_box(const EntK &e, RowPre &r, const int lane, const uint32_t row_first, const uint32_t row_count)
{
    const uint32_t i = row_first + ((uint32_t)lane < row_count ? lane : 0);
    const float2 *b = reinterpret_cast<const float2 *>(e.aabb + 6 * (size_t)i);
    r.bb0 = b[0]; r.bb1 = b[1]; r.bb2 = b[2];
}

__device__ __forceinline__ void load_row_pre(const EntK &e, RowPre &r, const RowIn &in)
{
    r.lo = e.model_table[2 * in.mi];
    r.hi = e.model_table[2 * in.mi + 1];
    const size_t p = in.p >= 0 ? (size_t)in.p : 0;
    const float4 *m = reinterpret_cast<const float4 *>(e.mx + 16 * p);
    r.pm[0] = m[0]; r.pm[1] = m[1]; r.pm[2] = m[2]; r.pm[3] = m[3];
    r.pseq = e.seqs[p];
}

__device__ __forceinline__ int find_attach(const EntK &e, uint32_t i)
{
    uint32_t lo = 0, hi = e.n_attach;
    while (lo < hi) {
        const uint32_t mid = (lo + hi) >> 1;
        if (e.attach[mid].entity < i) lo = mid + 1; else hi = mid;
    }
    return (lo < e.n_attach && e.attach[lo].entity == i) ? (int)lo : -1;
}

__device__ __forceinline__ bool point_in_box(const float (&p)[3], const float (&bb)[6])
{
    return p[0] >= bb[0] && p[0] <= bb[3] && p[1] >= bb[1] && p[1] <= bb[4] && p[2] >= bb[2] && p[2] <= bb[5];
}

template <bool CULL, bool TILE, bool HOST = false, bool XV = false>
__device__ __forceinline__ void process_row(const EntK &e, const RowIn &in, float4 *tile, const int lane,
                                            const uint32_t row_first, const uint32_t row_count,
                                            const uint32_t mode, const lmd::FrustumK &fr,
                                            const bool have_prev, const uint32_t prev_first,
                                            float (&carry_mx)[16], uint32_t &carry_seq, bool &carry_valid,
                                            const HostIO *hio = nullptr, const RowPre *pre = nullptr,
                                            const XViewsK *xv = nullptr)
{
    const bool in_range = (uint32_t)lane < row_count;
    const uint32_t i = row_first + (in_range ? lane : 0);
    uint64_t host_want = ~0ull;
    bool host_filter = false;
    uint64_t stale_w = 0;
    if constexpr (HOST) {
        host_filter = hio->keep != nullptr;
        host_want = host_filter ? hio->keep[row_first >> 6] : ~0ull;
        if (hio->stale) stale_w = hio->stale[row_first >> 6];
    }

    const uint32_t fl = in.fl;
    const bool alive = in_range && (fl & CLAPGPU_E_ALIVE);
    const bool dirty = (mode & CLAPGPU_UPDATE_ALL_DIRTY) ? true : (fl & CLAPGPU_E_DIRTY) != 0;
    const int32_t p = in.p;
    uint32_t seq = in.sq & 0xffffu, pseq = in.sq >> 16;

    bool in_prev = false;
    float pm[16];
    uint32_t parent_seq_now = 0;
    bool parent_in_regs = false;
    if (TILE) {
        in_prev = have_prev && p >= 0 && (uint32_t)p >= prev_first && (uint32_t)p < prev_first + WAVE;
        const int src = in_prev ? (int)((uint32_t)p - prev_first) : lane;
#pragma unroll
        for (int k = 0; k < 16; k++) pm[k] = __shfl(carry_mx[k], src);
        parent_seq_now = __shfl(carry_seq, src);
        if constexpr (HOST) {
            const int valid = __shfl((int)carry_valid, src);
            parent_in_regs = in_prev && valid != 0;
        } else
            parent_in_regs = in_prev && (__shfl((int)carry_valid, src) != 0);
    }
    if (p >= 0 && !in_prev)
        parent_seq_now = (HOST ? pre->pseq : e.seqs[p]) & 0xffffu;

    bool rebuild = alive;
    int at = -1;
    if (alive && p >= 0 && (fl & CLAPGPU_E_JOINT_ATTACHED) && e.n_attach)
        at = find_attach(e, i);
    const bool attached = at >= 0;
    if (p >= 0) {
        if (!attached && pseq == parent_seq_now && !dirty)
            rebuild = false;
        else
            pseq = parent_seq_now;
    } else if (!dirty) {
        rebuild = false;
    }

    float mx[16], inv[16], bb[6], ctr[3];
    bool has_aabb = false;

    if (rebuild) {
        const float4 lo = HOST ? pre->lo : e.model_table[2 * in.mi];
        const float4 hi = HOST ? pre->hi : e.model_table[2 * in.mi + 1];
        float local_mx[16];
        if (attached)
            load_mat4(local_mx, e.attach_local + 16 * (size_t)at);
        else
            lmd::trs(local_mx, in.ps.x, in.ps.y, in.ps.z, in.ps.w, in.q.x, in.q.y, in.q.z, in.q.w);
        if (p >= 0) {
            if (!parent_in_regs) {
                if constexpr (HOST) {
#pragma unroll
                    for (int c = 0; c < 4; c++) {
                        pm[4 * c] = pre->pm[c].x; pm[4 * c + 1] = pre->pm[c].y; pm[4 * c + 2] = pre->pm[c].z; pm[4 * c + 3] = pre->pm[c].w;
                    }
                } else
                    load_mat4(pm, e.mx + 16 * (size_t)p);
            }
            lmd::mul(mx, pm, local_mx);
        } else {
#pragma unroll
            for (int k = 0; k < 16; k++) mx[k] = local_mx[k];
        }
#ifdef CLAPGPU_EXP_NO_INVERT
#pragma unroll
        for (int k = 0; k < 16; k++) inv[k] = mx[k];
#else
        lmd::invert(inv, mx);
#endif

        has_aabb = __float_as_uint(lo.w) == 0u;
#ifdef CLAPGPU_EXP_NO_AABB
        if (has_aabb) {
#pragma unroll
            for (int k = 0; k < 6; k++) bb[k] = mx[12 + k % 3] + (k < 3 ? lo.x : hi.x);
#pragma unroll
            for (int k = 0; k < 3; k++) ctr[k] = mx[12 + k];
        }
#else
        if (has_aabb)
            lmd::world_aabb(bb, ctr, mx, lo.x, lo.y, lo.z, hi.x, hi.y, hi.z);
#endif

        seq = (seq + 1) & 0xffffu;
        e.seqs[i] = seq | (pseq << 16);
        if (!(mode & CLAPGPU_UPDATE_ALL_DIRTY) && (fl & CLAPGPU_E_DIRTY))
            e.flags[i] = fl & ~CLAPGPU_E_DIRTY;
    }

    if (TILE) {
#pragma unroll
        for (int k = 0; k < 16; k++) carry_mx[k] = mx[k];
        carry_seq = seq;
        carry_valid = rebuild;
    }

    const uint64_t rebuilt_mask = __ballot(rebuild);
    if (e.rebuilt_mask && lane == 0) e.rebuilt_mask[row_first >> 6] = rebuilt_mask;
    const uint64_t aabb_mask = __ballot(rebuild && has_aabb);
    const uint64_t full = row_count == WAVE ? ~0ull : ((1ull << row_count) - 1ull);
    const size_t e0 = row_first;
    float4 *tile_a = tile, *tile_b = tile + 256;
    float *tile_f = reinterpret_cast<float *>(tile);

    if (rebuilt_mask == full) {
        float4 va[4], vb[4];
        stage_mat4(tile_a, mx, lane);
        stage_mat4(tile_b, inv, lane);
        wave_lds_fence();
        unstage_mat4(tile_a, va, lane);
        unstage_mat4(tile_b, vb, lane);
        store_mat4_rows(e.mx + 16 * e0, va, lane, (int)row_count);
        store_mat4_rows(e.inv_mx + 16 * e0, vb, lane, (int)row_count);
        wave_lds_fence();
    } else if (rebuild) {
        float4 *dm = reinterpret_cast<float4 *>(e.mx + 16 * (size_t)i);
        float4 *di = reinterpret_cast<float4 *>(e.inv_mx + 16 * (size_t)i);
#pragma unroll
        for (int c = 0; c < 4; c++) {
            dm[c] = make_float4(mx[4 * c], mx[4 * c + 1], mx[4 * c + 2], mx[4 * c + 3]);
            di[c] = make_float4(inv[4 * c], inv[4 * c + 1], inv[4 * c + 2], inv[4 * c + 3]);
        }
    }
    if (aabb_mask == full) {
        stage_rows<6>(tile_f, bb, lane);
        stage_rows<3>(tile_f + 6 * WAVE, ctr, lane);
        wave_lds_fence();
        store_rows<6>(tile_f, e.aabb + 6 * e0, lane, (int)row_count);
        store_rows<3>(tile_f + 6 * WAVE, e.center + 3 * e0, lane, (int)row_count);
        wave_lds_fence();
    } else if (rebuild && has_aabb) {
#pragma unroll
        for (int k = 0; k < 6; k++) e.aabb[6 * (size_t)i + k] = bb[k];
#pragma unroll
        for (int k = 0; k < 3; k++) e.center[3 * (size_t)i + k] = ctr[k];
    }

    const bool want_bv = e.bv_on != 0;
    if (CULL || want_bv) {
        if (in_range && !(rebuild && has_aabb)) {
            if constexpr (HOST) {
                bb[0] = pre->bb0.x; bb[1] = pre->bb0.y; bb[2] = pre->bb1.x; bb[3] = pre->bb1.y; bb[4] = pre->bb2.x; bb[5] = pre->bb2.y;
            } else {
#pragma unroll
                for (int k = 0; k < 6; k++) bb[k] = e.aabb[6 * (size_t)i + k];
            }
        }
    }
    if (want_bv) {
        bool inside = in_range && (fl & CLAPGPU_E_ALIVE) && point_in_box(e.bv_cam, bb);
        if (!inside && e.bv_has_ctl)
            inside = in_range && (fl & CLAPGPU_E_ALIVE) && point_in_box(e.bv_ctl, bb);
        if (inside && e.bv_has_ctl && i == e.bv_ctl_entity)
            inside = false;
        const uint64_t inside_mask = __ballot(inside);
        if (e.bv_inside && lane == 0) e.bv_inside[e0 >> 6] = inside_mask;
        if constexpr (HOST) {
            if (hio->o_inside && lane == 0) hio->o_inside[e0 >> 6] = inside_mask;
            host_want |= inside_mask;
        }
        if (inside_mask) {
            unsigned long long key = 0;
            if (inside) {
                const float4 lo = e.model_table[2 * in.mi], hi = e.model_table[2 * in.mi + 1];
                const float X = fabsf(hi.x - lo.x) * in.ps.w, Y = fabsf(hi.y - lo.y) * in.ps.w,
                            Z = fabsf(hi.z - lo.z) * in.ps.w;
                const float vol = X * Y * Z;
                key = ((unsigned long long)__float_as_uint(vol) << 32) | (0xFFFFFFFFu - i);
            }
#pragma unroll
            for (int off = 32; off > 0; off >>= 1) {
                const unsigned long long o = __shfl_xor(key, off);
                key = o > key ? o : key;
            }
            if (lane == 0 && key && e.bv_result)
                atomicMax(e.bv_result, key);
        }
    }
    if (CULL) {
        bool vis = in_range && (fl & CLAPGPU_E_ALIVE) && (fl & CLAPGPU_E_VISIBLE);
        if (vis && !(fl & CLAPGPU_E_SKIP_CULLING))
            vis = lmd::aabb_in_frustum_fast(fr, bb);
        const uint64_t m = __ballot(vis);
        if (lane == 0) {
            e.vis_mask[e0 >> 6] = m;
            e.vis_row_pop[e0 >> 6] = (uint8_t)__popcll(m);
            if constexpr (HOST) hio->o_vis[e0 >> 6] = m;
        }
        if constexpr (HOST) host_want |= m;
        if constexpr (XV) {
            const uint64_t mx_any = cull_extra_views(*xv, in_range && (fl & CLAPGPU_E_ALIVE) && (fl & CLAPGPU_E_VISIBLE), fl, bb,
                                                     (uint32_t)(e0 >> 6), lane);
            if constexpr (HOST) host_want |= mx_any;
        }
    } else {
        if constexpr (HOST) host_want = ~0ull;
    }

    if constexpr (HOST) {
        const uint64_t exported = host_filter ? (rebuilt_mask & host_want) : rebuilt_mask;
        if (rebuild && ((exported >> lane) & 1ull)) {
            float4 *hm = reinterpret_cast<float4 *>(hio->o_mx + 16 * (size_t)i);
            float4 *hi = reinterpret_cast<float4 *>(hio->o_inv + 16 * (size_t)i);
#pragma unroll
            for (int c = 0; c < 4; c++) {
                hm[c] = make_float4(mx[4 * c], mx[4 * c + 1], mx[4 * c + 2], mx[4 * c + 3]);
                hi[c] = make_float4(inv[4 * c], inv[4 * c + 1], inv[4 * c + 2], inv[4 * c + 3]);
            }
            if (has_aabb) {
                float2 *hb = reinterpret_cast<float2 *>(hio->o_aabb + 6 * (size_t)i);
                hb[0] = make_float2(bb[0], bb[1]); hb[1] = make_float2(bb[2], bb[3]); hb[2] = make_float2(bb[4], bb[5]);
                float *hc = hio->o_center + 3 * (size_t)i;
                hc[0] = ctr[0]; hc[1] = ctr[1]; hc[2] = ctr[2];
            }
        }
        const uint64_t late = hio->late_ok ? stale_w & host_want & ~rebuilt_mask & __ballot(alive) : 0ull;
        if ((late >> lane) & 1ull) {
            const float4 *sm = reinterpret_cast<const float4 *>(e.mx + 16 * (size_t)i);
            const float4 *si = reinterpret_cast<const float4 *>(e.inv_mx + 16 * (size_t)i);
            float4 *hm = reinterpret_cast<float4 *>(hio->o_mx + 16 * (size_t)i);
            float4 *hi = reinterpret_cast<float4 *>(hio->o_inv + 16 * (size_t)i);
#pragma unroll
            for (int c = 0; c < 4; c++) { hm[c] = sm[c]; hi[c] = si[c]; }
            const float2 *sb = reinterpret_cast<const float2 *>(e.aabb + 6 * (size_t)i);
            float2 *hb = reinterpret_cast<float2 *>(hio->o_aabb + 6 * (size_t)i);
            hb[0] = sb[0]; hb[1] = sb[1]; hb[2] = sb[2];
            const float *sc = e.center + 3 * (size_t)i;
            float *hc = hio->o_center + 3 * (size_t)i;
            hc[0] = sc[0]; hc[1] = sc[1]; hc[2] = sc[2];
        }
        if (lane == 0) {
            hio->o_rebuilt[row_first >> 6] = rebuilt_mask;
            if (hio->o_exported) hio->o_exported[row_first >> 6] = exported | late;
            if (hio->stale) {
                const uint64_t ns = (stale_w | rebuilt_mask) & ~(exported | late);
                if (ns != stale_w) hio->stale[row_first >> 6] = ns;
            }
        }
    }
}


int launch_entities_tiles_host(hipStream_t stream, bool cull, const lmd::FrustumK &fr, const EntK &e, const HostIO &h,
                               const uint32_t *tile_row_start, uint32_t n_tiles, uint32_t n, uint32_t mode, const XViewsK &xv);

}
```

### clap_amd/csrc/entities_tiles_body.inc

```
#if defined(__HIP_DEVICE_COMPILE__)
    (void)fr_arg;
    typedef const __attribute__((address_space(4))) lmd::FrustumK *frustum_ptr;
    frustum_ptr frp = (frustum_ptr)__builtin_amdgcn_kernarg_segment_ptr();
#else
    typedef const lmd::FrustumK *frustum_ptr;
    frustum_ptr frp = &fr_arg;
#endif
    __shared__ float4 lds_tiles[ENT_BLOCK / WAVE][LDS_F4_PER_WAVE];
    __shared__ float4 mt_lds[2 * ENT_MT_CAP];
    const int lane = lane_id();
    const int wave = __builtin_amdgcn_readfirstlane(threadIdx.x / WAVE);
    const bool mt_cached = e.n_models <= (uint32_t)ENT_MT_CAP;
    if (mt_cached)
        for (uint32_t k = threadIdx.x; k < 2 * e.n_models; k += ENT_BLOCK) mt_lds[k] = e.model_table[k];
    __syncthreads();
    const uint32_t t = blockIdx.x * (ENT_BLOCK / WAVE) + wave;
    if (t >= n_tiles)
        return;
    const uint32_t n_rows = (n + WAVE - 1) / WAVE;
    uint32_t row = tile_row_start[t], row_end = tile_row_start[t + 1];
    if (row_end > n_rows) row_end = n_rows;
    if (row >= row_end)
        return;

    float carry_mx[16];
#pragma unroll
    for (int k = 0; k < 16; k++) carry_mx[k] = 0.f;
    uint32_t carry_seq = 0;
    bool carry_valid = false;
    bool have_prev = false;

    uint32_t row_first = row * WAVE;
    uint32_t row_count = n - row_first < WAVE ? n - row_first : WAVE;
    RowIn cur = load_row(e, lane, row_first, row_count);

    if (mt_cached && !e.bv_on) {
        asm volatile("" : : "v"(cur.ps.w), "v"(cur.q.w), "v"(cur.fl), "v"(cur.sq), "v"(cur.mi), "v"(cur.p));
        for (;;) {
            const uint32_t fl = cur.fl;
            const int32_t p = cur.p;
            const bool in_prev = have_prev && p >= 0 && (uint32_t)p >= row_first - WAVE && (uint32_t)p < row_first;
            const int src = in_prev ? (int)((uint32_t)p - (row_first - WAVE)) : lane;
            const uint32_t parent_seq_now = __shfl(carry_seq, src);
            const bool parent_ok = p < 0 || (in_prev && __shfl((int)carry_valid, src) != 0);
            const bool dirty = (mode & CLAPGPU_UPDATE_ALL_DIRTY) ? true : (fl & CLAPGPU_E_DIRTY) != 0;
            const bool rebuild = p >= 0 ? !((cur.sq >> 16) == parent_seq_now && !dirty) : dirty;
            const bool lane_ok = (fl & CLAPGPU_E_ALIVE) && rebuild && parent_ok &&
                                 !((fl & CLAPGPU_E_JOINT_ATTACHED) && e.n_attach) &&
                                 __float_as_uint(mt_lds[2 * cur.mi].w) == 0u;
            if (row_count != WAVE || __ballot(lane_ok) != ~0ull)
                break;
            const uint32_t next = row + 1;
            const bool more = next < row_end;
            const uint32_t nfirst = more ? next * WAVE : row_first;
            const uint32_t ncount = n - nfirst < WAVE ? n - nfirst : WAVE;
            const RowIn nxt = load_row(e, lane, nfirst, ncount);
            frustum_ptr frr = frp;
            asm volatile("" : "+s"(frr));
            process_row_fast<CULL, TILES_XV != 0>(e, cur, lds_tiles[wave], mt_lds, lane, row_first, mode, *(const lmd::FrustumK *)frr, src, parent_seq_now,
                                       carry_mx, carry_seq, TILES_XV_PTR);
            carry_valid = true;
            if (!more)
                return;
            have_prev = true;
            cur = nxt;
            row = next;
            row_first = nfirst;
            row_count = ncount;
        }
    }
    for (;;) {
        const uint32_t next = row + 1;
        const bool more = next < row_end;
        const uint32_t nfirst = more ? next * WAVE : row_first;
        const uint32_t ncount = n - nfirst < WAVE ? n - nfirst : WAVE;
        const RowIn nxt = load_row(e, lane, nfirst, ncount);
        frustum_ptr frr = frp;
        asm volatile("" : "+s"(frr));
        process_row<CULL, true, false, TILES_XV != 0>(e, cur, lds_tiles[wave], lane, row_first, row_count, mode, *(const lmd::FrustumK *)frr,
                                           have_prev, row_first - WAVE, carry_mx, carry_seq, carry_valid, nullptr, nullptr, TILES_XV_PTR);
        if (!more)
            break;
        have_prev = true;
        cur = nxt;
        row = next;
        row_first = nfirst;
        row_count = ncount;
    }
```

### clap_amd/csrc/physics2.hip

```cpp
#include <string.h>
#include <stdlib.h>
#include <vector>
#include "common.h"
#include "phys_dev.h"
#include "bp_grid.h"

namespace clapgpu {

constexpr int PB = 256;

struct WorldK2 {
    double  gravity[3];
    double  linear_damping;
    double  linear_damping_threshold_sq;
    double  adis_linear_threshold_sq;
    double  adis_angular_threshold_sq;
    double  adis_time;
    int32_t adis_steps;
    int32_t pad;
};
static_assert(sizeof(WorldK2) == sizeof(clapgpu_world), "world layout");
static_assert(true, "");

struct BodiesK {
    uint32_t n, samples;
    double *pos, *quat, *lvel, *avel;
    const double *mass, *radius;
    uint32_t *bflags;
    int32_t *adis_steps_left;
    double *adis_time_left;
    const double *length, *inertia;
    double Roff[12];
    double *aabb, *axis, *adis_samples;
    uint32_t *adis_counter;
    double *geom_records;
};

struct BinK { double cell; uint32_t mask; uint32_t *key, *rank, *cell_cnt, *ctrl; };
__device__ __forceinline__ void bin_body(const BinK &bin, uint32_t i, const double (&bb)[6]);

__device__ __forceinline__ void write_geom(const BodiesK &b, uint32_t i, const double (&p)[3], const double (&q)[4],
                                           double (*bb_out)[6] = nullptr)
{
    if (!b.aabb && !b.axis && !b.geom_records) return;
    double R[12], axis[3], bb[6];
    phd::q_to_R(q, R);
    phd::capsule_axis(R, b.Roff, axis);
    const double lz = b.length ? b.length[i] : 0.0;
    phd::geom_aabb(p, b.radius[i], lz, axis, bb);
    if (b.geom_records) {
        double2 *r = reinterpret_cast<double2 *>(b.geom_records + 8 * (size_t)i);
        r[0] = make_double2(p[0], p[1]); r[1] = make_double2(p[2], axis[0]);
        r[2] = make_double2(axis[1], axis[2]); r[3] = make_double2(b.radius[i], lz);
    }
    if (b.axis) { double *a = b.axis + 3 * (size_t)i; a[0] = axis[0]; a[1] = axis[1]; a[2] = axis[2]; }
    if (b.aabb) {
        double2 *o = reinterpret_cast<double2 *>(b.aabb + 6 * (size_t)i);
        o[0] = make_double2(bb[0], bb[1]); o[1] = make_double2(bb[2], bb[3]); o[2] = make_double2(bb[4], bb[5]);
    }
    if (bb_out)
#pragma unroll
        for (int a = 0; a < 6; a++) (*bb_out)[a] = bb[a];
}

__device__ __forceinline__ void bin_stored(const BinK &bin, const BodiesK &b, uint32_t i)
{
    const double2 *p = reinterpret_cast<const double2 *>(b.aabb + 6 * (size_t)i);
    const double2 x = p[0], y = p[1], z = p[2];
    const double bb[6] = { x.x, x.y, y.x, y.y, z.x, z.y };
    bin_body(bin, i, bb);
}

__global__ __launch_bounds__(PB)
void k_bodies_aabb(BodiesK b)
{
    const uint32_t i = blockIdx.x * PB + threadIdx.x;
    if (i >= b.n) return;
    const double p[3] = { b.pos[3 * (size_t)i], b.pos[3 * (size_t)i + 1], b.pos[3 * (size_t)i + 2] };
    const double q[4] = { b.quat[4 * (size_t)i], b.quat[4 * (size_t)i + 1], b.quat[4 * (size_t)i + 2], b.quat[4 * (size_t)i + 3] };
    write_geom(b, i, p, q);
}

template <bool BIN>
__global__ __launch_bounds__(PB)
void k_bodies_step(BodiesK b, WorldK2 w, double h, BinK bin)
{
    const uint32_t i = blockIdx.x * PB + threadIdx.x;
    if (BIN && i == 0) bin.ctrl[3] = bin.ctrl[3] + 1;
    if (i >= b.n) return;
    uint32_t fl = b.bflags[i];
    if (fl & CLAPGPU_BODY_DISABLED) { if (BIN) bin_stored(bin, b, i); return; }
    double *pp = b.pos + 3 * (size_t)i, *qp = b.quat + 4 * (size_t)i, *vp = b.lvel + 3 * (size_t)i, *op = b.avel + 3 * (size_t)i;
    double v[3] = { vp[0], vp[1], vp[2] }, om[3] = { op[0], op[1], op[2] };

    if ((fl & CLAPGPU_BODY_AUTO_DISABLE) && (fl & CLAPGPU_BODY_HAS_JOINT)) {
        bool idle = false;
        double al[3], aa[3];
        const uint32_t S = b.samples > 1 ? b.samples : 1;
        if (S == 1) {
            for (int a = 0; a < 3; a++) { al[a] = v[a]; aa[a] = om[a]; }
            idle = true;
        } else {
            double *ring = b.adis_samples + (size_t)i * S * 6;
            uint32_t c = b.adis_counter[i] & 0x7fffffffu, ready = b.adis_counter[i] >> 31;
            for (int a = 0; a < 3; a++) { ring[6 * (size_t)c + a] = v[a]; ring[6 * (size_t)c + 3 + a] = om[a]; }
            if (++c >= S) { c = 0; ready = 1; }
            b.adis_counter[i] = c | ready << 31;
            if (ready) {
                idle = true;
                for (int a = 0; a < 3; a++) { al[a] = ring[a]; aa[a] = ring[3 + a]; }
                for (uint32_t s = 1; s < S; s++)
                    for (int a = 0; a < 3; a++) { al[a] += ring[6 * (size_t)s + a]; aa[a] += ring[6 * (size_t)s + 3 + a]; }
                const double r1 = 1.0 / (double)S;
                for (int a = 0; a < 3; a++) { al[a] *= r1; aa[a] *= r1; }
            }
        }
        if (idle) {
            if (al[0] * al[0] + al[1] * al[1] + al[2] * al[2] > w.adis_linear_threshold_sq) idle = false;
            else if (aa[0] * aa[0] + aa[1] * aa[1] + aa[2] * aa[2] > w.adis_angular_threshold_sq) idle = false;
        }
        int32_t sl = b.adis_steps_left[i];
        double tl = b.adis_time_left[i];
        if (idle) { sl--; tl -= h; } else { sl = w.adis_steps; tl = w.adis_time; }
        b.adis_steps_left[i] = sl;
        b.adis_time_left[i] = tl;
        if (sl <= 0 && tl <= 0) {
            b.bflags[i] = (fl | CLAPGPU_BODY_DISABLED) & ~CLAPGPU_BODY_HAS_JOINT;
            vp[0] = vp[1] = vp[2] = 0;
            op[0] = op[1] = op[2] = 0;
            if (BIN) bin_stored(bin, b, i);
            return;
        }
    }
    if (fl & CLAPGPU_BODY_HAS_JOINT)
        b.bflags[i] = fl & ~CLAPGPU_BODY_HAS_JOINT;

    double q[4] = { qp[0], qp[1], qp[2], qp[3] };
    double tacc[3] = { 0, 0, 0 }, invIw[12];
    const bool have_inertia = b.inertia != nullptr;
    if (have_inertia) {
        const double Ib[3] = { b.inertia[3 * (size_t)i], b.inertia[3 * (size_t)i + 1], b.inertia[3 * (size_t)i + 2] };
        const double invIb[3] = { 1.0 / Ib[0], 1.0 / Ib[1], 1.0 / Ib[2] };
        double R[12];
        phd::q_to_R(q, R);
        phd::world_tensor(R, invIb, invIw);
        if (fl & CLAPGPU_BODY_GYROSCOPIC) {
            double Iw[12], L[3], Itild[12], itInv[12];
            phd::world_tensor(R, Ib, Iw);
            phd::mul331(L, Iw, om);
            for (int k = 0; k < 12; k++) Itild[k] = 0;
            Itild[1] = L[2]; Itild[2] = -L[1];
            Itild[4] = -L[2]; Itild[6] = L[0];
            Itild[8] = L[1]; Itild[9] = -L[0];
            for (int k = 0; k < 12; k++) Itild[k] = Itild[k] * h + Iw[k];
            const double rh = 1.0 / h;
            L[0] *= rh; L[1] *= rh; L[2] *= rh;
            if (phd::invert3(itInv, Itild)) {
                double T[12], tau0[3];
                for (int r = 0; r < 3; r++) {
                    for (int c = 0; c < 3; c++)
                        T[4 * r + c] = Iw[4 * r] * itInv[c] + Iw[4 * r + 1] * itInv[4 + c] + Iw[4 * r + 2] * itInv[8 + c];
                    T[4 * r + 3] = 0;
                }
                T[0] -= 1; T[5] -= 1; T[10] -= 1;
                phd::mul331(tau0, T, L);
                tacc[0] += tau0[0]; tacc[1] += tau0[1]; tacc[2] += tau0[2];
            }
        }
    }
    const double m = b.mass[i];
    const double k = h * (1.0 / m);
    const bool grav = !(fl & CLAPGPU_BODY_NO_GRAVITY);
    for (int j = 0; j < 3; j++)
        v[j] += k * (grav ? m * w.gravity[j] : 0.0);
    if (have_inertia) {
        double d[3];
        tacc[0] *= h; tacc[1] *= h; tacc[2] *= h;
        phd::mul331(d, invIw, tacc);
        om[0] += d[0]; om[1] += d[1]; om[2] += d[2];
        op[0] = om[0]; op[1] = om[1]; op[2] = om[2];
    }
    double p[3] = { pp[0], pp[1], pp[2] };
    for (int j = 0; j < 3; j++) p[j] += h * v[j];
    pp[0] = p[0]; pp[1] = p[1]; pp[2] = p[2];
    const double d0 = 0.5 * (-om[0] * q[1] - om[1] * q[2] - om[2] * q[3]);
    const double d1 = 0.5 * ( om[0] * q[0] + om[1] * q[3] - om[2] * q[2]);
    const double d2 = 0.5 * (-om[0] * q[3] + om[1] * q[0] + om[2] * q[1]);
    const double d3 = 0.5 * ( om[0] * q[2] - om[1] * q[1] + om[2] * q[0]);
    q[0] += h * d0; q[1] += h * d1; q[2] += h * d2; q[3] += h * d3;
    double l = q[0] * q[0] + q[1] * q[1] + q[2] * q[2] + q[3] * q[3];
    if (l > 0) {
        l = 1.0 / sqrt(l);
        q[0] *= l; q[1] *= l; q[2] *= l; q[3] *= l;
    } else {
        q[0] = 1; q[1] = q[2] = q[3] = 0;
    }
    qp[0] = q[0]; qp[1] = q[1]; qp[2] = q[2]; qp[3] = q[3];
    if (w.linear_damping != 0.0) {
        const double speed2 = v[0] * v[0] + v[1] * v[1] + v[2] * v[2];
        if (speed2 > w.linear_damping_threshold_sq) {
            const double s = 1 - w.linear_damping;
            v[0] *= s; v[1] *= s; v[2] *= s;
        }
    }
    vp[0] = v[0]; vp[1] = v[1]; vp[2] = v[2];
    if (BIN) {
        double bb[6];
        write_geom(b, i, p, q, &bb);
        bin_body(bin, i, bb);
    } else
        write_geom(b, i, p, q);
}

constexpr int BP_LIST = 16;
constexpr int BP_TILE = 16;
constexpr int BP_WORK = 512;
constexpr int BP_EMIT_TILE = 1024;
#ifndef BP_SEARCH_IN_FLIGHT
#define BP_SEARCH_IN_FLIGHT 1
#endif
constexpr int CTRL_STATUS = 2, CTRL_EPOCH = 3, CTRL_CONTACT_WORD = 8;


struct BpRec { double bb[6]; uint32_t idx; int32_t cell[3]; };
static_assert(CTRL_EPOCH == CTRL_BIN_EPOCH, "bp_grid.h's view of the control words");
static_assert(sizeof(BpRec) == sizeof(GridRec) && offsetof(BpRec, idx) == offsetof(GridRec, idx) &&
              offsetof(BpRec, cell) == offsetof(GridRec, cell), "bp_grid.h's view of the records");

struct BpK {
    uint32_t n;
    double cell;
    uint32_t mask;
    const double *aabb;
    uint32_t *cell_cnt;
    uint2    *cell_range;
    uint32_t *key, *rank;
    uint32_t *entries;
    struct BpRec *recs;
    uint32_t *cnt, *scnt;
    uint32_t *partners, *spartners;
    uint64_t *lb_body, *lb_static;
    uint64_t *lb_cells;
    uint32_t *ctrl;
    uint32_t n_tiles;
    const uint32_t *s_start;
    const uint32_t *s_entries;
    const double *s_aabb;
    const uint32_t *s_large;
    const struct BpRec *s_recs;
    const struct BpRec *s_lrecs;
    uint32_t n_large, n_static;
    uint32_t *pairs, capacity, *pair_total;
    uint32_t *spairs, scapacity, *spair_total;
};

__device__ __forceinline__ void load_box(const double *aabb, uint32_t i, double (&bb)[6])
{
    const double2 *p = reinterpret_cast<const double2 *>(aabb + 6 * (size_t)i);
    const double2 a = p[0], b = p[1], c = p[2];
    bb[0] = a.x; bb[1] = a.y; bb[2] = b.x; bb[3] = b.y; bb[4] = c.x; bb[5] = c.y;
}

__device__ __forceinline__ void box_cell(const double (&bb)[6], double cell, int32_t &cx, int32_t &cy, int32_t &cz)
{
    cx = cell_coord((bb[0] + bb[1]) * 0.5, cell);
    cy = cell_coord((bb[2] + bb[3]) * 0.5, cell);
    cz = cell_coord((bb[4] + bb[5]) * 0.5, cell);
}

__device__ __forceinline__ bool boxes_overlap(const double (&a)[6], const double (&b)[6])
{
    return !(a[0] > b[1] || a[1] < b[0] || a[2] > b[3] || a[3] < b[2] || a[4] > b[5] || a[5] < b[4]);
}

__device__ __forceinline__ void bin_body(const BinK &bin, uint32_t i, const double (&bb)[6])
{
    if (bb[1] - bb[0] > bin.cell || bb[3] - bb[2] > bin.cell || bb[5] - bb[4] > bin.cell)
        atomicOr(&bin.ctrl[CTRL_STATUS], 1u);
    int32_t cx, cy, cz;
    box_cell(bb, bin.cell, cx, cy, cz);
    const uint32_t slot = cell_slot(cx, cy, cz, bin.mask);
    bin.key[i] = slot;
    bin.rank[i] = atomicAdd(&bin.cell_cnt[slot], 1u);
}

__global__ __launch_bounds__(PB)
void k_bp_bin(BpK k)
{
    const uint32_t i = blockIdx.x * PB + threadIdx.x;
    if (i == 0) k.ctrl[CTRL_EPOCH] = k.ctrl[CTRL_EPOCH] + 1;
    if (i >= k.n) return;
    double bb[6];
    load_box(k.aabb, i, bb);
    if (bb[1] - bb[0] > k.cell || bb[3] - bb[2] > k.cell || bb[5] - bb[4] > k.cell)
        atomicOr(&k.ctrl[CTRL_STATUS], 1u);
    int32_t cx, cy, cz;
    box_cell(bb, k.cell, cx, cy, cz);
    const uint32_t slot = cell_slot(cx, cy, cz, k.mask);
    k.key[i] = slot;
    k.rank[i] = atomicAdd(&k.cell_cnt[slot], 1u);
}

constexpr uint64_t LB_AGG = 1ull << 62, LB_PREFIX = 2ull << 62, LB_FLAGS = 3ull << 62;
__device__ __forceinline__ uint64_t lb_word(uint64_t flag, uint32_t epoch, uint32_t value)
{
    return flag | ((uint64_t)(epoch & 0x3fffffffu) << 32) | value;
}

__device__ __forceinline__ uint32_t lb_exclusive(uint64_t *state, uint32_t b, uint32_t sum, uint32_t epoch, uint32_t *status)
{
    const int lane = lane_id();
    if (b == 0) {
        if (lane == 0) __hip_atomic_store(&state[0], lb_word(LB_PREFIX, epoch, sum), __ATOMIC_RELAXED, __HIP_MEMORY_SCOPE_AGENT);
        return 0;
    }
    if (lane == 0) __hip_atomic_store(&state[b], lb_word(LB_AGG, epoch, sum), __ATOMIC_RELAXED, __HIP_MEMORY_SCOPE_AGENT);
    uint32_t excl = 0;
    for (int64_t top = (int64_t)b - 1; top >= 0; top -= WAVE) {
        const int64_t t = top - lane;
        uint64_t w = 0;
        if (t >= 0) {
            uint32_t spins = 0;
            do {
                w = __hip_atomic_load(&state[t], __ATOMIC_RELAXED, __HIP_MEMORY_SCOPE_AGENT);
                if ((w & LB_FLAGS) && (uint32_t)((w >> 32) & 0x3fffffffu) == (epoch & 0x3fffffffu)) break;
                w = 0;
                __builtin_amdgcn_s_sleep(1);
            } while (++spins < (1u << 22));
            if (!w) atomicOr(status, 4u);
        }
        const uint64_t is_prefix = __ballot(t >= 0 && (w & LB_FLAGS) == LB_PREFIX);
        const int stop = is_prefix ? __builtin_ctzll(is_prefix) : WAVE - 1;
        uint32_t v = (t >= 0 && lane <= stop) ? (uint32_t)w : 0u;
#pragma unroll
        for (int o = 32; o > 0; o >>= 1) v += __shfl_xor(v, o);
        excl += v;
        if (is_prefix) break;
    }
    if (lane == 0) __hip_atomic_store(&state[b], lb_word(LB_PREFIX, epoch, excl + sum), __ATOMIC_RELAXED, __HIP_MEMORY_SCOPE_AGENT);
    return excl;
}

constexpr int BP_CELLS_BLOCK = 1024;
__global__ __launch_bounds__(BP_CELLS_BLOCK)
void k_bp_cells(BpK k)
{
    __shared__ uint32_t tot[BP_CELLS_BLOCK / WAVE];
    __shared__ uint32_t excl_s;
    const int lane = lane_id(), wave = threadIdx.x / WAVE;
    const uint32_t b = blockIdx.x * (BP_CELLS_BLOCK / WAVE) + wave;
    uint32_t block_total = 0, c = 0, before = 0;
    if (b <= k.mask) {
        c = k.cell_cnt[(size_t)b * 64 + lane];
        k.cell_cnt[(size_t)b * 64 + lane] = 0;
        uint32_t incl = c;
#pragma unroll
        for (int o = 1; o < WAVE; o <<= 1) {
            const uint32_t u = __shfl_up(incl, o);
            if (lane >= o) incl += u;
        }
        before = incl - c;
        block_total = __shfl(incl, WAVE - 1);
    }
    if (lane == 0) tot[wave] = block_total;
    __syncthreads();
    if (wave == 0) {
        uint32_t sum = 0;
#pragma unroll
        for (int q = 0; q < BP_CELLS_BLOCK / WAVE; q++) sum += tot[q];
        const uint32_t excl = lb_exclusive(k.lb_cells, blockIdx.x, sum, k.ctrl[CTRL_EPOCH], k.ctrl + CTRL_STATUS);
        if (lane == 0) excl_s = excl;
    }
    __syncthreads();
    if (b <= k.mask) {
        uint32_t start = excl_s;
        for (int q = 0; q < wave; q++) start += tot[q];
        k.cell_range[(size_t)b * 64 + lane] = make_uint2(start + before, c);
    }
}

__global__ __launch_bounds__(PB)
void k_bp_scatter(BpK k)
{
    const uint32_t i = blockIdx.x * PB + threadIdx.x;
    if (i >= k.n) return;
    const uint32_t slot = k.key[i];
    const uint32_t at = k.cell_range[slot].x + k.rank[i];
    k.entries[at] = i;
    const double2 *p = reinterpret_cast<const double2 *>(k.aabb + 6 * (size_t)i);
    double2 *o = reinterpret_cast<double2 *>(k.recs + at);
    const double2 b0 = p[0], b1 = p[1], b2 = p[2];
    o[0] = b0; o[1] = b1; o[2] = b2;
    const int32_t cx = cell_coord((b0.x + b0.y) * 0.5, k.cell), cy = cell_coord((b1.x + b1.y) * 0.5, k.cell),
                  cz = cell_coord((b2.x + b2.y) * 0.5, k.cell);
    reinterpret_cast<int4 *>(o)[3] = make_int4((int)i, cx, cy, cz);
}

__global__ __launch_bounds__(PB)
void k_bp_search(BpK k)
{
    constexpr int WAVES = PB / WAVE, T = BP_TILE, LOOKUPS = 4;
    constexpr uint32_t WL = BP_WORK, OWN = 0x80000000u, STAT = 0x40000000u, IDX = 0x3fffffffu;
    constexpr int LARGE_TILE = 32;
    constexpr uint32_t HITS = 64;
    static_assert(T * 15 <= WAVE * LOOKUPS && T <= 16, "tile lookups");
    __shared__ __attribute__((aligned(8))) uint32_t work[WAVES][WL][2];
    __shared__ double abox[WAVES][T][6];
    __shared__ uint32_t aidx[WAVES][T];
    __shared__ int32_t lead[WAVES][2 * T][4];
    __shared__ uint32_t shits[WAVES][T];
    __shared__ uint32_t hits[WAVES][HITS][2], nhits[WAVES];
    __shared__ BpRec large[LARGE_TILE];
    const int lane = lane_id(), wave = threadIdx.x / WAVE;
    const uint32_t t0 = (blockIdx.x * WAVES + wave) * T;
    const uint32_t nA = t0 < k.n ? (k.n - t0 < (uint32_t)T ? k.n - t0 : (uint32_t)T) : 0;
    const bool statics = k.n_static != 0;

    const uint32_t m0 = statics ? (k.n_large < LARGE_TILE ? k.n_large : LARGE_TILE) : 0;
    if (threadIdx.x < m0) large[threadIdx.x] = k.s_lrecs[threadIdx.x];
    int32_t cx = 0, cy = 0, cz = 0;
    uint32_t ob = 0;
    const bool isA = (uint32_t)lane < nA;
    if (isA) {
        const BpRec me = k.recs[t0 + lane];
#pragma unroll
        for (int x = 0; x < 6; x++) abox[wave][lane][x] = me.bb[x];
        aidx[wave][lane] = me.idx;
        cx = me.cell[0]; cy = me.cell[1]; cz = me.cell[2];
        ob = block_hash(cx >> 2, cy >> 2, cz >> 2, k.mask);
    }
    if (lane < T) shits[wave][lane] = 0;
    if (lane == 0) nhits[wave] = 0;
    const int32_t px = __shfl_up(cx, 1), py = __shfl_up(cy, 1), pz = __shfl_up(cz, 1);
    const uint32_t pob = __shfl_up(ob, 1);
    const bool cell_leader = isA && (lane == 0 || px != cx || py != cy || pz != cz);
    const bool block_leader = isA && statics && (lane == 0 || pob != ob);
    const uint32_t cmask = (uint32_t)__ballot(cell_leader), bmask = (uint32_t)__ballot(block_leader);
    const uint32_t n_lead = __popc(cmask), n_blead = __popc(bmask);
    if (isA) {
        const uint32_t below = (1u << lane) - 1u;
        if (cell_leader) {
            const uint32_t above = cmask >> (lane + 1);
            const uint32_t hi = above ? lane + 1 + __builtin_ctz(above) : nA;
            int32_t *d = lead[wave][__popc(cmask & below)];
            d[0] = cx; d[1] = cy; d[2] = cz; d[3] = (int32_t)((uint32_t)lane | hi << 8);
        }
        if (block_leader) {
            const uint32_t above = bmask >> (lane + 1);
            const uint32_t hi = above ? lane + 1 + __builtin_ctz(above) : nA;
            int32_t *d = lead[wave][T + __popc(bmask & below)];
            d[0] = (int32_t)ob; d[3] = (int32_t)((uint32_t)lane | hi << 8);
        }
    }
    wave_lds_fence();
    const uint32_t n_cell_runs = n_lead * 14u, n_runs = n_cell_runs + n_blead;
    uint32_t b0[LOOKUPS], len[LOOKUPS], rng[LOOKUPS], mylen = 0;
    uint32_t slot[LOOKUPS], sidx[LOOKUPS];
    bool is_cell[LOOKUPS], is_stat[LOOKUPS], own[LOOKUPS];
#pragma unroll
    for (int r = 0; r < LOOKUPS; r++) {
        const uint32_t u = lane + WAVE * r;
        is_cell[r] = u < n_cell_runs;
        is_stat[r] = !is_cell[r] && u < n_runs;
        const uint32_t l = is_cell[r] ? u / 14u : 0u, cq = 13u + u % 14u;
        const int32_t *d = lead[wave][is_stat[r] ? T + (u - n_cell_runs) : l];
        const int32_t d0 = d[0], d1 = d[1], d2 = d[2];
        rng[r] = (is_cell[r] || is_stat[r]) ? (uint32_t)d[3] : 0u;
        own[r] = is_cell[r] && cq == 13u;
        slot[r] = is_cell[r] ? cell_slot(d0 - 1 + (int32_t)(cq % 3), d1 - 1 + (int32_t)((cq / 3) % 3), d2 - 1 + (int32_t)(cq / 9), k.mask) : 0u;
        sidx[r] = is_stat[r] ? (uint32_t)d0 : 0u;
    }
    uint2 v_cr[LOOKUPS];
    uint32_t v_s0[LOOKUPS], v_s1[LOOKUPS];
#pragma unroll
    for (int r = 0; r < LOOKUPS; r++) v_cr[r] = k.cell_range[slot[r]];
    if (statics) {
#pragma unroll
        for (int r = 0; r < LOOKUPS; r++) { v_s0[r] = k.s_start[sidx[r]]; v_s1[r] = k.s_start[sidx[r] + 1]; }
    } else {
#pragma unroll
        for (int r = 0; r < LOOKUPS; r++) { v_s0[r] = 0; v_s1[r] = 0; }
    }
#pragma unroll
    for (int r = 0; r < LOOKUPS; r++) {
        b0[r] = is_cell[r] ? (v_cr[r].x | (own[r] ? OWN : 0u)) : is_stat[r] ? (v_s0[r] | STAT) : 0u;
        len[r] = is_cell[r] ? v_cr[r].y : is_stat[r] ? v_s1[r] - v_s0[r] : 0u;
        mylen += len[r];
    }
    uint32_t incl = mylen;
#pragma unroll
    for (int o = 1; o < WAVE; o <<= 1) {
        const uint32_t up = __shfl_up(incl, o);
        if (lane >= o) incl += up;
    }
    const uint32_t total = __shfl(incl, WAVE - 1);
    const uint32_t first = incl - mylen;

    auto flush_hits = [&]() {
        wave_lds_fence();
        const uint32_t nh = nhits[wave] < HITS ? nhits[wave] : HITS;
        for (uint32_t h = lane; h < nh; h += WAVE) {
            const uint32_t lo = hits[wave][h][0], hi = hits[wave][h][1];
            const uint32_t at = atomicAdd(&k.cnt[lo], 1u);
            if (at < BP_LIST) k.partners[(size_t)lo * BP_LIST + at] = hi;
        }
        wave_lds_fence();
        if (lane == 0) nhits[wave] = 0;
        wave_lds_fence();
    };
    auto test = [&](uint32_t w, uint32_t range, const BpRec &r) {
        const uint32_t j = r.idx, a_hi = range >> 8;
        for (uint32_t x = range & 0xffu; x < a_hi; x++) {
            const double2 *ab = reinterpret_cast<const double2 *>(abox[wave][x]);
            const double2 a01 = ab[0], a23 = ab[1], a45 = ab[2];
            const bool apart = (a01.x > r.bb[1]) | (a01.y < r.bb[0]) | (a23.x > r.bb[3]) | (a23.y < r.bb[2]) |
                               (a45.x > r.bb[5]) | (a45.y < r.bb[4]);
            if (apart) continue;
            const uint32_t i = aidx[wave][x];
            if (w & STAT) {
                const uint32_t at = atomicAdd(&shits[wave][x], 1u);
                if (at < BP_LIST) k.spartners[(size_t)i * BP_LIST + at] = j;
            } else if (j != i && (!(w & OWN) || j > i)) {
                const uint32_t lo = i < j ? i : j, hi = i < j ? j : i;
                const uint32_t h = atomicAdd(&nhits[wave], 1u);
                if (h < HITS) { hits[wave][h][0] = lo; hits[wave][h][1] = hi; }
                else {
                    const uint32_t at = atomicAdd(&k.cnt[lo], 1u);
                    if (at < BP_LIST) k.partners[(size_t)lo * BP_LIST + at] = hi;
                }
            }
        }
    };

    for (uint32_t base = 0; base < total; base += WL) {
        uint32_t off = first;
#pragma unroll
        for (int r = 0; r < LOOKUPS; r++) {
            for (uint32_t e = 0; __any(e < len[r]); e++) {
                if (e < len[r]) {
                    const uint32_t o = off + e - base;
                    if (o < WL) *reinterpret_cast<uint2 *>(work[wave][o]) = make_uint2(b0[r] + e, rng[r]);
                }
            }
            off += len[r];
        }
        wave_lds_fence();
        const uint32_t todo = total - base < WL ? total - base : WL;
#if BP_SEARCH_IN_FLIGHT == 2
        for (uint32_t e = lane; e < todo + lane; e += 2 * WAVE) {
            const bool v0 = e < todo, v1 = e + WAVE < todo;
            const uint2 e0 = v0 ? *reinterpret_cast<const uint2 *>(work[wave][e]) : make_uint2(0u, 0u);
            const uint2 e1 = v1 ? *reinterpret_cast<const uint2 *>(work[wave][e + WAVE]) : make_uint2(0u, 0u);
            const uint32_t w0 = e0.x, g0 = e0.y, w1 = e1.x, g1 = e1.y;
            BpRec r0, r1;
            if (v0) r0 = ((w0 & STAT) ? k.s_recs : k.recs)[w0 & IDX];
            if (v1) r1 = ((w1 & STAT) ? k.s_recs : k.recs)[w1 & IDX];
            if (v0) test(w0, g0, r0);
            if (v1) test(w1, g1, r1);
        }
#else
        for (uint32_t e = lane; e < todo; e += WAVE) {
            const uint2 e0 = *reinterpret_cast<const uint2 *>(work[wave][e]);
            const BpRec r0 = ((e0.x & STAT) ? k.s_recs : k.recs)[e0.x & IDX];
            test(e0.x, e0.y, r0);
        }
#endif
        flush_hits();
    }
    if (!statics) return;
    for (uint32_t base = 0; base < k.n_large; base += LARGE_TILE) {
        const uint32_t m = k.n_large - base < LARGE_TILE ? k.n_large - base : LARGE_TILE;
        if (base) {
            __syncthreads();
            if (threadIdx.x < m) large[threadIdx.x] = k.s_lrecs[base + threadIdx.x];
        }
        __syncthreads();
        const uint32_t x = lane % T;
        if (x < nA) {
            double a[6];
#pragma unroll
            for (int y = 0; y < 6; y++) a[y] = abox[wave][x][y];
            for (uint32_t e = lane / T; e < m; e += WAVE / T) {
                double bs[6];
#pragma unroll
                for (int y = 0; y < 6; y++) bs[y] = large[e].bb[y];
                if (boxes_overlap(a, bs)) {
                    const uint32_t at = atomicAdd(&shits[wave][x], 1u);
                    if (at < BP_LIST) k.spartners[(size_t)aidx[wave][x] * BP_LIST + at] = large[e].idx;
                }
            }
        }
    }
    wave_lds_fence();
    if (isA) k.scnt[aidx[wave][lane]] = shits[wave][lane];
}

template <typename F>
__device__ __forceinline__ void research_body(const BpK &k, uint32_t i, F &&emit_sorted)
{
    double a[6];
    load_box(k.aabb, i, a);
    int32_t cx, cy, cz;
    box_cell(a, k.cell, cx, cy, cz);
    uint32_t last = i;
    for (;;) {
        uint32_t best = 0xffffffffu;
        for (int cq = 0; cq < 27; cq++) {
            const uint32_t slot = cell_slot(cx - 1 + cq % 3, cy - 1 + (cq / 3) % 3, cz - 1 + cq / 9, k.mask);
            const uint2 cr = k.cell_range[slot];
            const uint32_t s0 = cr.x, s1 = cr.x + cr.y;
            for (uint32_t s = s0; s < s1; s++) {
                const uint32_t j = k.entries[s];
                if (j <= last || j >= best) continue;
                double bj[6];
                load_box(k.aabb, j, bj);
                if (boxes_overlap(a, bj)) best = j;
            }
        }
        if (best == 0xffffffffu) break;
        emit_sorted(best);
        last = best;
    }
}

__global__ __launch_bounds__(BP_EMIT_TILE)
void k_bp_emit(BpK k)
{
    __shared__ uint32_t lds[2][BP_EMIT_TILE / WAVE];
    __shared__ uint32_t tile_excl[2];
    const uint32_t i = blockIdx.x * BP_EMIT_TILE + threadIdx.x;
    const int lane = lane_id(), wave = threadIdx.x / WAVE;
    const bool with_statics = k.n_static != 0;
    uint32_t c[2] = { 0, 0 };
    if (i < k.n) {
        c[0] = k.cnt[i];
        k.cnt[i] = 0;
        if (with_statics) { c[1] = k.scnt[i]; k.scnt[i] = 0; }
    }
    uint4 pl[2][BP_LIST / 4];
#pragma unroll
    for (int t = 0; t < 2; t++)
#pragma unroll
        for (int q = 0; q < BP_LIST / 4; q++) pl[t][q] = make_uint4(0, 0, 0, 0);
    if (c[0] && c[0] <= (uint32_t)BP_LIST) {
// ... 602 lines not shown
```

### clap_amd/csrc/runtime.hip

```cpp
#include <string.h>
#include <stdlib.h>
#include <math.h>
#include <string>
#include <atomic>
#include "common.h"
#include "lm_dev.h"

#ifdef CLAPGPU_EXPERIMENT
#define CLAPGPU_ABI_VERSION (34u | 0x80000000u)
#else
#define CLAPGPU_ABI_VERSION 34u
#endif

namespace clapgpu {

static thread_local std::string g_last_error;

int hip_fail(hipError_t err, const char *what)
{
    g_last_error = std::string(what) + ": " + hipGetErrorString(err);
    (void)hipGetLastError();
    if (err == hipErrorOutOfMemory)
        return CLAPGPU_ERR_NOMEM;
    if (err == hipErrorInvalidValue || err == hipErrorInvalidDevicePointer)
        return CLAPGPU_ERR_INVALID_ARGUMENTS;
    return CLAPGPU_ERR_UNKNOWN;
}

void set_last_error(const char *what) { g_last_error = what; }

static std::atomic<int> g_fail_after{-1};

hipError_t launch_error()
{
    const hipError_t e = hipGetLastError();
    int left = g_fail_after.load(std::memory_order_relaxed);
    if (left < 0 || e != hipSuccess) return e;
    while (left > 0)
        if (g_fail_after.compare_exchange_weak(left, left - 1, std::memory_order_relaxed)) return e;
    return left == 0 ? hipErrorLaunchFailure : e;
}

}

using namespace clapgpu;

extern "C" void clapgpu_test_fail_after(int launches)
{
    static const bool armed = getenv("CLAPGPU_TEST_HOOKS") != nullptr;
    if (armed || launches < 0) g_fail_after.store(launches, std::memory_order_relaxed);
}

extern "C" uint32_t clapgpu_abi_version(void) { return CLAPGPU_ABI_VERSION; }

extern "C" const char *clapgpu_last_error(void) { return g_last_error.c_str(); }

extern "C" int clapgpu_device_count(void)
{
    int n = 0;
    if (hipGetDeviceCount(&n) != hipSuccess) {
        (void)hipGetLastError();
        return 0;
    }
    return n;
}

extern "C" int clapgpu_init(int device)
{
    int n = 0;
    if (hipGetDeviceCount(&n) != hipSuccess || n <= 0) {
        (void)hipGetLastError();
        g_last_error = "no HIP device";
        return CLAPGPU_ERR_INIT_FAILED;
    }
    if (device < 0 || device >= n)
        return CLAPGPU_ERR_INVALID_ARGUMENTS;
    CLAPGPU_HIP(hipSetDevice(device));
    hipDeviceProp_t prop;
    CLAPGPU_HIP(hipGetDeviceProperties(&prop, device));
    if (!strstr(prop.gcnArchName, "gfx950")) {
        g_last_error = std::string("device is ") + prop.gcnArchName + ", libclapgpu is built for gfx950";
        return CLAPGPU_ERR_NOT_SUPPORTED;
    }
    return CLAPGPU_OK;
}

extern "C" int clapgpu_malloc(void **dev, size_t bytes)
{
    if (!dev) return CLAPGPU_ERR_INVALID_ARGUMENTS;
    CLAPGPU_HIP(hipMalloc(dev, bytes ? bytes : 1));
    return CLAPGPU_OK;
}

extern "C" int clapgpu_free(void *dev)
{
    CLAPGPU_HIP(hipFree(dev));
    return CLAPGPU_OK;
}

extern "C" int clapgpu_host_malloc(void **host, size_t bytes)
{
    if (!host) return CLAPGPU_ERR_INVALID_ARGUMENTS;
    CLAPGPU_HIP(hipHostMalloc(host, bytes ? bytes : 1, hipHostMallocDefault));
    return CLAPGPU_OK;
}

extern "C" int clapgpu_host_malloc_mapped(void **host, void **dev_alias, size_t bytes)
{
    if (!host || !dev_alias) return CLAPGPU_ERR_INVALID_ARGUMENTS;
    CLAPGPU_HIP(hipHostMalloc(host, bytes ? bytes : 1, hipHostMallocMapped | hipHostMallocCoherent));
    const hipError_t e = hipHostGetDevicePointer(dev_alias, *host, 0);
    if (e != hipSuccess) {
        (void)hipHostFree(*host);
        *host = nullptr;
        return hip_fail(e, "hipHostGetDevicePointer");
    }
    return CLAPGPU_OK;
}

extern "C" int clapgpu_wait_word(const volatile uint32_t *word, uint32_t value, void *stream)
{
    if (!word) return CLAPGPU_ERR_INVALID_ARGUMENTS;
    for (uint32_t spins = 0;; spins++) {
        if (*word == value) return CLAPGPU_OK;
        __builtin_ia32_pause();
        if ((spins & 0xffffu) == 0xffffu) {
            const hipError_t e = hipStreamQuery(as_stream(stream));
            if (e == hipSuccess) {
                if (*word == value) return CLAPGPU_OK;
                g_last_error = "clapgpu_wait_word: the stream drained without the word being stored";
                return CLAPGPU_ERR_UNKNOWN;
            }
            if (e != hipErrorNotReady) return hip_fail(e, "hipStreamQuery");
        }
    }
}

extern "C" int clapgpu_host_free(void *host)
{
    CLAPGPU_HIP(hipHostFree(host));
    return CLAPGPU_OK;
}

extern "C" int clapgpu_memcpy_h2d(void *dev, const void *host, size_t bytes, void *stream)
{
    CLAPGPU_HIP(hipMemcpyAsync(dev, host, bytes, hipMemcpyHostToDevice, as_stream(stream)));
    return CLAPGPU_OK;
}

extern "C" int clapgpu_memcpy_d2h(void *host, const void *dev, size_t bytes, void *stream)
{
    CLAPGPU_HIP(hipMemcpyAsync(host, dev, bytes, hipMemcpyDeviceToHost, as_stream(stream)));
    return CLAPGPU_OK;
}

extern "C" int clapgpu_memset(void *dev, int value, size_t bytes, void *stream)
{
    CLAPGPU_HIP(hipMemsetAsync(dev, value, bytes, as_stream(stream)));
    return CLAPGPU_OK;
}

extern "C" int clapgpu_stream_sync(void *stream)
{
    CLAPGPU_HIP(hipStreamSynchronize(as_stream(stream)));
    return CLAPGPU_OK;
}


extern "C" void clapgpu_view_matrix(const float pos[3], const float quat[4], float view_mx[16])
{
    float m[16], r[16];
    lmd::identity(m);
    lmd::from_quat(r, quat[0], quat[1], quat[2], quat[3]);
    lmd::mul(m, m, r);
    float t[16];
    for (int i = 0; i < 16; i++) t[i] = m[i];
    for (int c = 0; c < 3; c++)
        for (int rr = 0; rr < 3; rr++)
            t[4 * c + rr] = m[4 * rr + c];
    lmd::translate_in_place(t, -pos[0], -pos[1], -pos[2]);
    memcpy(view_mx, t, sizeof(t));
}

extern "C" void clapgpu_mat4_invert(const float m[16], float out[16])
{
    float a[16], t[16];
    memcpy(a, m, sizeof(a));
    lmd::invert(t, a);
    memcpy(out, t, sizeof(t));
}

extern "C" void clapgpu_mat4_from_quat(const float quat_xyzw[4], float out[16])
{
    float t[16];
    lmd::from_quat(t, quat_xyzw[0], quat_xyzw[1], quat_xyzw[2], quat_xyzw[3]);
    memcpy(out, t, sizeof(t));
}

extern "C" void clapgpu_perspective(float fov, float aspect, float n, float f,
                                    int ndc_z_zero_one, float proj_mx[16])
{
    const float a = (float)(1.0 / tan((double)(fov / 2.f)));
    memset(proj_mx, 0, 16 * sizeof(float));
    proj_mx[0] = a / aspect;
    proj_mx[5] = a;
    proj_mx[11] = -1.f;
    if (ndc_z_zero_one) {
        proj_mx[10] = -(f / (f - n));
        proj_mx[14] = -((f * n) / (f - n));
    } else {
        proj_mx[10] = -((f + n) / (f - n));
        proj_mx[14] = -((2.f * f * n) / (f - n));
    }
}

extern "C" void clapgpu_frustum_calc(const float view_mx[16], const float proj_mx[16],
                                     int ndc_z_zero_one, clapgpu_frustum *out)
{
    float v[16], p[16], mvp[16], inv[16];
    memcpy(v, view_mx, sizeof(v));
    memcpy(p, proj_mx, sizeof(p));
    lmd::mul(mvp, p, v);
    lmd::invert(inv, mvp);
    for (int k = 0; k < 4; k++) {
        const float r0 = mvp[4 * k + 0], r1 = mvp[4 * k + 1], r2 = mvp[4 * k + 2], r3 = mvp[4 * k + 3];
        out->planes[0][k] = r3 + r0;
        out->planes[1][k] = r3 - r0;
        out->planes[2][k] = r3 + r1;
        out->planes[3][k] = r3 - r1;
        out->planes[4][k] = r3 + r2;
        out->planes[5][k] = r3 - r2;
    }
    const float zn = ndc_z_zero_one ? 0.f : -1.f;
    for (int i = 0; i < 8; i++) {
        const float sx = (i == 0 || i == 3 || i == 4 || i == 7) ? -1.f : 1.f;
        const float sy = ((i & 3) < 2) ? -1.f : 1.f;
        const float c[4] = { sx, sy, i < 4 ? zn : 1.f, 1.f };
        float q[4];
        lmd::mul_vec4(q, inv, c);
        const float s = 1.f / q[3];
        for (int k = 0; k < 4; k++)
            out->corners[i][k] = q[k] * s;
    }
}
```

### clap_amd/entities.py

```python
import ctypes as C

import numpy as np
import torch

from . import _lib
from . import synth


def _ptr(t):
    return C.c_void_p(t.data_ptr()) if t is not None else C.c_void_p(0)


def _stream():
    return C.c_void_p(torch.cuda.current_stream().cuda_stream)


def view_calc_frustum(cam):
    L = _lib.lib()
    f32p = C.POINTER(C.c_float)
    pos = np.ascontiguousarray(cam["cam_pos"], np.float32)
    quat = np.ascontiguousarray(cam["cam_quat"], np.float32)
    view = np.zeros(16, np.float32)
    proj = np.zeros(16, np.float32)
    L.clapgpu_view_matrix(pos.ctypes.data_as(f32p), quat.ctypes.data_as(f32p), view.ctypes.data_as(f32p))
    fov, aspect, near, far = (float(v) for v in cam["persp"])
    z01 = int(cam["ndc_z_zero_one"][0])
    L.clapgpu_perspective(fov, aspect, near, far, z01, proj.ctypes.data_as(f32p))
    fr = _lib.Frustum()
    L.clapgpu_frustum_calc(view.ctypes.data_as(f32p), proj.ctypes.data_as(f32p), z01, C.byref(fr))
    return fr, view, proj


def frustum_arrays(fr):
    return (np.ctypeslib.as_array(fr.planes).reshape(6, 4).copy(),
            np.ctypeslib.as_array(fr.corners).reshape(8, 4).copy())


class EntityBatch:

    IN_KEYS = ("pos_scale", "rot", "parent", "model", "flags", "seqs")

    def __init__(self, scene, device="cuda:0"):
        self.device = torch.device(device)
        dev = self.device
        self.n = int(scene["n"])
        self.n_real = int(scene.get("n_real", self.n))
        self.tiled = "tile_row_start" in scene
        if self.tiled:
            trs = np.ascontiguousarray(scene["tile_row_start"], np.uint32)
            if int(trs[-1]) * 64 != self.n:
                raise ValueError("tile_row_start does not cover the scene")
            self.n_tiles = len(trs) - 1
            self.tile_row_start = torch.from_numpy(trs.view(np.int32)).to(dev)
            self.level_start, self.n_levels = None, 0
        else:
            ls = np.asarray(scene["level_start"], np.uint32)
            if np.any(ls[:-1] % 64):
                raise ValueError("level starts must be multiples of 64: use synth.pad_levels()")
            self.level_start = np.ascontiguousarray(ls)
            self.n_levels = len(ls) - 1
            self._ls_ptr = self.level_start.ctypes.data_as(C.POINTER(C.c_uint32))
        for k in self.IN_KEYS:
            a = scene[k]
            if a.dtype == np.uint32:
                a = a.view(np.int32)
            setattr(self, k, torch.from_numpy(np.ascontiguousarray(a)).to(dev))
        self.model_table = torch.from_numpy(synth.model_table(scene)).to(dev)
        n = self.n
        self.mx = torch.zeros((n, 16), dtype=torch.float32, device=dev)
        self.inv_mx = torch.zeros((n, 16), dtype=torch.float32, device=dev)
        self.aabb = torch.zeros((n, 6), dtype=torch.float32, device=dev)
        self.center = torch.zeros((n, 3), dtype=torch.float32, device=dev)
        self.vis_mask = torch.zeros(((n + 63) // 64 or 1,), dtype=torch.int64, device=dev)
        n_rows = (n + 63) // 64
        self.vis_row_pop = torch.zeros(((n_rows + 15) // 16 * 16 or 16,), dtype=torch.uint8, device=dev)
        self.visible = torch.zeros((max(n, 1),), dtype=torch.int32, device=dev)
        self.visible_count = torch.zeros((1,), dtype=torch.int32, device=dev)
        nscratch = _lib.lib().clapgpu_visible_scratch_bytes(n)
        self.scratch = torch.zeros((nscratch // 4 or 1,), dtype=torch.int32, device=dev)
        self._desc = _lib.Entities(
            n=n, n_models=self.model_table.shape[0],
            pos_scale=self.pos_scale.data_ptr(), rot=self.rot.data_ptr(), parent=self.parent.data_ptr(),
            model=self.model.data_ptr(), model_table=self.model_table.data_ptr(), flags=self.flags.data_ptr(),
            seqs=self.seqs.data_ptr(), mx=self.mx.data_ptr(), inv_mx=self.inv_mx.data_ptr(),
            aabb=self.aabb.data_ptr(), center=self.center.data_ptr(), vis_mask=self.vis_mask.data_ptr(),
            vis_row_pop=self.vis_row_pop.data_ptr())

    def use_vis_buffers(self, vis_mask, vis_row_pop):
        self.vis_mask, self.vis_row_pop = vis_mask, vis_row_pop
        self._desc.vis_mask = vis_mask.data_ptr()
        self._desc.vis_row_pop = vis_row_pop.data_ptr()

    def set_views(self, frusta):
        dev = self.device
        n_rows = (self.n + 63) // 64
        self._views = _lib.Views()
        self._views.n = len(frusta)
        self.view_masks, self.view_row_pops = [], []
        for v, fr in enumerate(frusta[:_lib.EXTRA_VIEWS_MAX]):
            C.memmove(C.byref(self._views.frustum[v]), C.byref(fr), C.sizeof(_lib.Frustum))
            m = torch.zeros((n_rows or 1,), dtype=torch.int64, device=dev)
            p = torch.zeros(((n_rows + 15) // 16 * 16 or 16,), dtype=torch.uint8, device=dev)
            self.view_masks.append(m); self.view_row_pops.append(p)
            self._views.vis_mask[v] = m.data_ptr(); self._views.vis_row_pop[v] = p.data_ptr()
        self._desc.views = C.pointer(self._views) if frusta else None

    def compact_view(self, v, index_base=0):
        rc = _lib.lib().clapgpu_visible_compact(_stream(), _ptr(self.view_masks[v]), _ptr(self.view_row_pops[v]), self.n,
                                                index_base, _ptr(self.visible), _ptr(self.visible_count), _ptr(self.scratch))
        _lib.check(rc, "clapgpu_visible_compact")

    def set_attachments(self, attach, jt_pool, bind_pool):
        a = np.ascontiguousarray(attach)
        assert np.all(np.diff(a["entity"].astype(np.int64)) > 0), "attach table must be sorted by entity"
        self._attach = torch.from_numpy(a.view(np.uint8).reshape(-1, 16).copy()).to(self.device)
        self._jt_pool = jt_pool if torch.is_tensor(jt_pool) else torch.from_numpy(
            np.ascontiguousarray(jt_pool, np.float32)).to(self.device)
        self._bind_pool = torch.from_numpy(np.ascontiguousarray(bind_pool, np.float32)).to(self.device)
        idx = torch.from_numpy(a["entity"].astype(np.int64)).to(self.device)
        self.flags[idx] |= np.int32(_lib.E_JOINT_ATTACHED)
        self._desc.n_attach = a.shape[0]
        self._desc.attach = self._attach.data_ptr()
        self._desc.jt_pool = self._jt_pool.data_ptr()
        self._desc.bind_pool = self._bind_pool.data_ptr()
        self._attach_local = torch.zeros((a.shape[0], 16), dtype=torch.float32, device=self.device)
        self._desc.attach_local = self._attach_local.data_ptr()

    def set_bv_query(self, cam_pos, ctl_pos=None, ctl_entity=0):
        self.bv_result = torch.zeros(1, dtype=torch.int64, device=self.device)
        q = _lib.BvQuery()
        q.cam_pos[:] = [float(v) for v in cam_pos]
        q.has_ctl = 0 if ctl_pos is None else 1
        q.ctl_pos[:] = [0.0, 0.0, 0.0] if ctl_pos is None else [float(v) for v in ctl_pos]
        q.ctl_entity = int(ctl_entity)
        q.result = self.bv_result.data_ptr()
        self._bv = q
        self._desc.bv = C.pointer(q)

    def camera_bv(self):
        key = int(self.bv_result.item()) & 0xFFFFFFFFFFFFFFFF
        if key == 0:
            return -1, 0.0
        return 0xFFFFFFFF - (key & 0xFFFFFFFF), float(np.asarray([key >> 32], np.uint32).view(np.float32)[0])

    def mq_update(self, frustum=None, all_dirty=False):
        mode = _lib.UPDATE_ALL_DIRTY if all_dirty else 0
        fr = C.byref(frustum) if frustum is not None else None
        if self.tiled:
            rc = _lib.lib().clapgpu_entities_update_tiles(_stream(), C.byref(self._desc), _ptr(self.tile_row_start),
                                                          self.n_tiles, mode, fr)
            _lib.check(rc, "clapgpu_entities_update_tiles")
        else:
            rc = _lib.lib().clapgpu_entities_update(_stream(), C.byref(self._desc), self._ls_ptr, self.n_levels,
                                                    mode, fr)
            _lib.check(rc, "clapgpu_entities_update")

    def update_level(self, level, frustum=None, all_dirty=False):
        first = int(self.level_start[level])
        count = int(self.level_start[level + 1]) - first
        mode = _lib.UPDATE_ALL_DIRTY if all_dirty else 0
        rc = _lib.lib().clapgpu_entities_update_level(_stream(), C.byref(self._desc), first, count, mode,
                                                      C.byref(frustum) if frustum is not None else None)
        _lib.check(rc, "clapgpu_entities_update_level")

    def cull(self, frustum):
        rc = _lib.lib().clapgpu_entities_cull(_stream(), C.byref(self._desc), C.byref(frustum))
        _lib.check(rc, "clapgpu_entities_cull")

    def compact_visible(self, index_base=0, two_pass=False):
        rc = _lib.lib().clapgpu_visible_compact(_stream(), _ptr(self.vis_mask),
                                                None if two_pass else _ptr(self.vis_row_pop), self.n, index_base,
                                                _ptr(self.visible), _ptr(self.visible_count), _ptr(self.scratch))
        _lib.check(rc, "clapgpu_visible_compact")

    def alloc_lod(self):
        if not hasattr(self, "cur_lod"):
            self.cur_lod = torch.zeros(max(self.n, 1), dtype=torch.int32, device=self.device)
            self.draw_lod = torch.zeros(max(self.n, 1), dtype=torch.int32, device=self.device)
            self.force_lod = None

    def select_lod(self, cam_pos, force_lod=None):
        self.alloc_lod()
        if force_lod is not None:
            self.force_lod = torch.from_numpy(np.ascontiguousarray(force_lod, np.int32)).to(self.device)
        cp = (C.c_float * 3)(*[float(v) for v in cam_pos])
        rc = _lib.lib().clapgpu_entities_lod(_stream(), C.byref(self._desc), _ptr(self.visible),
                                             _ptr(self.visible_count), 0, cp, _ptr(self.force_lod),
                                             _ptr(self.cur_lod), _ptr(self.draw_lod))
        _lib.check(rc, "clapgpu_entities_lod")

    def compact_visible_lod(self, cam_pos, force_lod=None, index_base=0):
        self.alloc_lod()
        if force_lod is not None:
            self.force_lod = torch.from_numpy(np.ascontiguousarray(force_lod, np.int32)).to(self.device)
        cp = (C.c_float * 3)(*[float(v) for v in cam_pos])
        rc = _lib.lib().clapgpu_visible_compact_lod(_stream(), C.byref(self._desc), index_base, cp, _ptr(self.force_lod),
                                                    _ptr(self.cur_lod), _ptr(self.visible), _ptr(self.visible_count),
                                                    _ptr(self.draw_lod), _ptr(self.scratch))
        _lib.check(rc, "clapgpu_visible_compact_lod")

    def view_entity_in_frustum(self, idx):
        w = int(self.vis_mask[idx >> 6].item()) & 0xFFFFFFFFFFFFFFFF
        return bool((w >> (idx & 63)) & 1)

    def set_transforms(self, idx, pos_scale, rot):
        idx_t = torch.as_tensor(np.asarray(idx, np.int64), device=self.device)
        self.pos_scale[idx_t] = torch.from_numpy(np.ascontiguousarray(pos_scale, np.float32)).to(self.device)
        self.rot[idx_t] = torch.from_numpy(np.ascontiguousarray(rot, np.float32)).to(self.device)
        self.flags[idx_t] |= np.int32(_lib.E_DIRTY)

    def download(self):
        torch.cuda.synchronize(self.device)
        cnt = int(self.visible_count.item())
        return dict(mx=self.mx.cpu().numpy(), inv_mx=self.inv_mx.cpu().numpy(), aabb=self.aabb.cpu().numpy(),
                    center=self.center.cpu().numpy(), flags=self.flags.cpu().numpy().view(np.uint32),
                    seqs=self.seqs.cpu().numpy().view(np.uint32),
                    vis_mask=self.vis_mask.cpu().numpy().view(np.uint64),
                    visible=self.visible[:cnt].cpu().numpy().view(np.uint32), visible_count=cnt)

    def algorithmic_bytes(self):
        par = self.parent.cpu().numpy()
        real = (self.flags.cpu().numpy().view(np.uint32) & np.uint32(_lib.E_ALIVE)) != 0
        children = int(np.count_nonzero((par >= 0) & real))
        roots = int(np.count_nonzero((par < 0) & real))
        return 276 * children + 212 * roots
```

### clap_amd/frame.py

```python
import numpy as np
import torch

from . import entities as ent_mod


class FrameLoop:
    def __init__(self, batch, cam, world=None, feed=None, body_links=None, lights=None, characters=None,
                 particles=None, contacts=False, pose_readers=("trs", "joint_pos"), prebin=False):
        self.batch, self.world, self.feed, self.lights = batch, world, feed, lights
        self.characters, self.particles = characters, particles
        self.body_links, self.contacts = body_links, contacts
        self.prebin = prebin
        self._desc = None
        if characters is not None:
            missing = bool(characters.model.anim_desc.packed_layout & 0x010)
            characters.set_outputs(trs=("trs" in pose_readers) or missing, joint_pos="joint_pos" in pose_readers)
        self.set_camera(cam)

    def set_camera(self, cam):
        self.cam = cam
        self.frustum, self.view_mx, self.proj_mx = ent_mod.view_calc_frustum(cam)
        self._desc = None

    def _build(self):
        import ctypes as C
        from . import _lib
        b, w = self.batch, self.world
        f = _lib.Frame()
        keep = []
        f.entities = C.pointer(b._desc)
        if b.tiled:
            f.tile_row_start, f.n_tiles = b.tile_row_start.data_ptr(), b.n_tiles
        else:
            f.level_start, f.n_levels = b.level_start.ctypes.data, b.n_levels
        f.frustum = C.pointer(self.frustum)
        if w is not None:
            f.bodies, f.world, f.bp = C.pointer(w._desc), C.pointer(w.world), w._bp
            f.pairs, f.pair_capacity, f.pair_total = w.pairs.data_ptr(), w.capacity, w.pair_total.data_ptr()
            if w.n_static:
                f.static_pairs, f.static_pair_capacity = w.static_pairs.data_ptr(), w.static_capacity
                f.static_pair_total = w.static_pair_total.data_ptr()
            if self.contacts:
                w.alloc_contacts()
                g = w.body_geoms()
                keep.append(g)
                f.body_geoms = C.pointer(g)
                f.contacts, f.contact_total = w.contact2_buf.data_ptr(), w.contact2_total.data_ptr()
                if w.n_static:
                    sg = w.static_geoms()
                    keep.append(sg)
                    f.static_geoms = C.pointer(sg)
                    f.static_contacts = w.static_contact2_buf.data_ptr()
                    f.static_contact_total = w.static_contact2_total.data_ptr()
                    if w._meshes is not None:
                        w.alloc_mesh_contacts()
                        f.meshes = w._meshes
                        f.mesh_contacts, f.mesh_ref = w.mesh_contact_buf.data_ptr(), w.mesh_ref.data_ptr()
                        f.mesh_contact_capacity = w.mesh_contact_capacity
                        f.mesh_contact_total, f.mesh_capped = w.mesh_contact_total.data_ptr(), w.mesh_capped.data_ptr()
                        f.mesh_scratch = w.mesh_scratch.data_ptr()
            if self.body_links is not None:
                lb, le = w.upload_links(*self.body_links)
                f.n_body_links, f.link_body, f.link_entity = len(self.body_links[0]), lb.data_ptr(), le.data_ptr()
        if self.feed is not None:
            f.characters = C.pointer(self.feed._desc)
        vm = np.ascontiguousarray(self.view_mx, np.float32)
        pm = np.ascontiguousarray(self.proj_mx, np.float32)
        keep += [vm, pm]
        f.view_mx = vm.ctypes.data_as(C.POINTER(C.c_float))
        f.proj_mx = pm.ctypes.data_as(C.POINTER(C.c_float))
        ls = self.lights
        if ls is not None:
            d = ls._desc()
            keep.append(d)
            f.lights = C.pointer(d)
            if ls._carriers and ls._carriers[0]:
                n, ce, cl, co = ls._carriers
                f.n_light_carriers, f.carrier_entity, f.carrier_light, f.carrier_offset = n, ce.data_ptr(), cl.data_ptr(), co.data_ptr()
            tiles = ls.alloc_tiles()
            if tiles is not None:
                f.light_width, f.light_height, f.light_cell, f.light_tiles = ls.width, ls.height, ls.cell, tiles.data_ptr()
        cb = self.characters
        if cb is not None:
            if getattr(cb, "_clock", None) is None:
                cb.start_clock()
            f.anim_clock = C.pointer(cb._clock)
            f.skeleton, f.animations = C.pointer(cb.model.skel_desc), C.pointer(cb.model.anim_desc)
            f.pose = C.pointer(cb._pose_desc)
            if cb._skin_desc is not None:
                f.skin = C.pointer(cb._skin_desc)
        if self.particles is not None:
            f.particles = C.pointer(self.particles._desc)
        b.alloc_lod()
        f.index_base = 0
        f.visible, f.visible_count, f.visible_scratch = b.visible.data_ptr(), b.visible_count.data_ptr(), b.scratch.data_ptr()
        f.cam_pos[:] = [float(v) for v in self.cam["cam_pos"]]
        f.force_lod = b.force_lod.data_ptr() if b.force_lod is not None else None
        f.cur_lod, f.draw_lod = b.cur_lod.data_ptr(), b.draw_lod.data_ptr()
        self._desc, self._keep = f, keep
        return f

    def capture(self, dt=1.0 / 120.0, warmup_now=0.0):
        self.clap_frame(warmup_now, dt)
        torch.cuda.synchronize()
        self._now_host = torch.zeros(1, dtype=torch.float64).pin_memory()
        self._graph = torch.cuda.CUDAGraph()
        saved = (None if self.world is None else self.world.time_acc.value)
        with torch.cuda.graph(self._graph):
            self._issue(None, steps=1)
        if self.world is not None:
            self.world.time_acc.value = saved

    def clap_frame_replay(self, now):
        self._now_host[0] = float(now)
        if self.characters is not None:
            self.characters.now_dev.copy_(self._now_host, non_blocking=True)
        self._graph.replay()

    def clap_frame(self, now, dt):
        steps = self.world.phys_step_begin(dt) if self.world is not None else 0
        self._issue(now, steps)

    def _issue(self, now, steps):
        import ctypes as C
        from . import _lib
        f = self._desc or self._build()
        if self.lights is not None:
            self.lights._upload()
        f.now_dev = self.characters.now_dev.data_ptr() if (now is None and self.characters is not None) else None
        f.flags = (1 if getattr(self, "overlap", False) else 0) | (2 if self.prebin else 0)
        rc = _lib.lib().clapgpu_frame_issue(C.c_void_p(torch.cuda.current_stream().cuda_stream), C.byref(f),
                                            0.0 if now is None else float(now), int(steps))
        _lib.check(rc, "clapgpu_frame_issue")
```

### include/clapgpu.h

```cpp
#ifndef CLAPGPU_H
#define CLAPGPU_H

#include <stddef.h>
#include <stdint.h>

#ifdef __cplusplus
extern "C" {
#endif

#define CLAPGPU_OK                      0
#define CLAPGPU_ERR_NOMEM              -1
#define CLAPGPU_ERR_INVALID_ARGUMENTS  -2
#define CLAPGPU_ERR_NOT_SUPPORTED      -3
#define CLAPGPU_ERR_TOO_LARGE         -11
#define CLAPGPU_ERR_INIT_FAILED       -14
#define CLAPGPU_ERR_OUT_OF_BOUNDS     -26
#define CLAPGPU_ERR_UNKNOWN           -32

#define CLAPGPU_E_VISIBLE       (1u << 0)
#define CLAPGPU_E_SKIP_CULLING  (1u << 14)
#define CLAPGPU_E_DIRTY         (1u << 16)
#define CLAPGPU_E_JOINT_ATTACHED (1u << 17)
#define CLAPGPU_E_ALIVE         (1u << 31)

int clapgpu_device_count(void);
int clapgpu_init(int device);
const char *clapgpu_last_error(void);
void clapgpu_test_fail_after(int launches);
uint32_t clapgpu_abi_version(void);

int clapgpu_malloc(void **dev, size_t bytes);
int clapgpu_free(void *dev);
int clapgpu_host_malloc(void **host, size_t bytes);
int clapgpu_host_malloc_mapped(void **host, void **dev_alias, size_t bytes);
int clapgpu_host_free(void *host);
int clapgpu_memcpy_h2d(void *dev, const void *host, size_t bytes, void *stream);
int clapgpu_memcpy_d2h(void *host, const void *dev, size_t bytes, void *stream);
int clapgpu_memset(void *dev, int value, size_t bytes, void *stream);
int clapgpu_stream_sync(void *stream);


typedef struct clapgpu_frustum {
    float planes[6][4];
    float corners[8][4];
} clapgpu_frustum;

void clapgpu_view_matrix(const float pos[3], const float quat[4], float view_mx[16]);
void clapgpu_mat4_invert(const float m[16], float out[16]);
void clapgpu_mat4_from_quat(const float quat_xyzw[4], float out[16]);
void clapgpu_perspective(float fov, float aspect, float near_plane, float far_plane,
                         int ndc_z_zero_one, float proj_mx[16]);
void clapgpu_frustum_calc(const float view_mx[16], const float proj_mx[16],
                          int ndc_z_zero_one, clapgpu_frustum *out);

typedef struct clapgpu_attach {
    uint32_t entity, jt, bind, pad;
} clapgpu_attach;

typedef struct clapgpu_bv_query {
    float     cam_pos[3];
    uint32_t  has_ctl;
    float     ctl_pos[3];
    uint32_t  ctl_entity;
    uint64_t *result;
    uint64_t *inside_mask;
} clapgpu_bv_query;

#define CLAPGPU_EXTRA_VIEWS_MAX 4
typedef struct clapgpu_views {
    uint32_t        n, pad;
    clapgpu_frustum frustum[CLAPGPU_EXTRA_VIEWS_MAX];
    uint64_t       *vis_mask[CLAPGPU_EXTRA_VIEWS_MAX];
    uint8_t        *vis_row_pop[CLAPGPU_EXTRA_VIEWS_MAX];
    uint64_t       *host_vis_mask[CLAPGPU_EXTRA_VIEWS_MAX];
} clapgpu_views;

typedef struct clapgpu_entities {
    uint32_t        n;
    uint32_t        n_models;
    const float    *pos_scale;
    const float    *rot;
    const int32_t  *parent;
    const int32_t  *model;
    const float    *model_table;
    uint32_t       *flags;
    uint32_t       *seqs;
    float          *mx;
    float          *inv_mx;
    float          *aabb;
    float          *center;
    uint64_t       *vis_mask;
    uint8_t        *vis_row_pop;
    uint32_t        n_attach;
    uint32_t        pad;
    const clapgpu_attach *attach;
    const float    *jt_pool;
    const float    *bind_pool;
    float          *attach_local;
    const clapgpu_bv_query *bv;
    uint64_t       *rebuilt_mask;
    const clapgpu_views *views;
} clapgpu_entities;

#define CLAPGPU_UPDATE_ALL_DIRTY  (1u << 0)

int clapgpu_entities_update(void *stream, const clapgpu_entities *e,
                            const uint32_t *level_start, uint32_t n_levels,
                            uint32_t mode, const clapgpu_frustum *frustum);

int clapgpu_entities_update_level(void *stream, const clapgpu_entities *e,
                                  uint32_t first, uint32_t count,
                                  uint32_t mode, const clapgpu_frustum *frustum);

int clapgpu_entities_update_tiles(void *stream, const clapgpu_entities *e,
                                  const uint32_t *tile_row_start, uint32_t n_tiles,
                                  uint32_t mode, const clapgpu_frustum *frustum);

int clapgpu_entities_cull(void *stream, const clapgpu_entities *e, const clapgpu_frustum *frustum);

typedef struct clapgpu_entity_input {
    uint32_t slot, flags;
    float    pos_scale[4], rot[4];
} clapgpu_entity_input;
typedef struct clapgpu_entities_export {
    float    *mx, *inv_mx, *aabb, *center;
    uint64_t *vis_mask, *rebuilt_mask, *inside_mask;
    uint32_t *counter;
    uint32_t *done;
    uint32_t  done_value, pad;
    uint64_t *stale_mask;
} clapgpu_entities_export;
int clapgpu_entities_apply_inputs(void *stream, const clapgpu_entities *e, const clapgpu_entity_input *list, uint32_t n_list);
int clapgpu_entities_export_rebuilt(void *stream, const clapgpu_entities *e, const clapgpu_entities_export *x);
typedef struct clapgpu_entity_place { uint32_t slot; int32_t parent, model; uint32_t flags; } clapgpu_entity_place;
#define CLAPGPU_PLACE_ZERO_BOX    1u
#define CLAPGPU_PLACE_CLEAR_STALE 2u
int clapgpu_entities_place(void *stream, const clapgpu_entities *e, const clapgpu_entity_place *list, uint32_t n_list,
                           uint64_t *stale_mask);
int clapgpu_entities_export_rows(void *stream, const clapgpu_entities *e, const clapgpu_entities_export *x,
                                 const uint64_t *select_mask);

#define CLAPGPU_HOSTIO_EXPORT_STALE_READ 1u
typedef struct clapgpu_entities_hostio {
    const float    *pos_scale, *rot;
    const uint32_t *flags;
    const uint64_t *touched;
    float    *mx, *inv_mx, *aabb, *center;
    uint64_t *vis_mask, *rebuilt_mask, *inside_mask;
    uint32_t *counter;
    uint32_t *done;
    uint32_t  done_value, options;
    const uint64_t *keep_mask;
    uint64_t       *exported_mask;
    uint64_t       *stale_mask;
} clapgpu_entities_hostio;
int clapgpu_entities_update_tiles_hostio(void *stream, const clapgpu_entities *e, const uint32_t *tile_row_start,
                                         uint32_t n_tiles, uint32_t mode, const clapgpu_frustum *frustum,
                                         const clapgpu_entities_hostio *io);
int clapgpu_wait_word(const volatile uint32_t *word, uint32_t value, void *stream);

size_t clapgpu_visible_scratch_bytes(uint32_t n);
int clapgpu_visible_compact(void *stream, const uint64_t *vis_mask, const uint8_t *vis_row_pop,
                            uint32_t n, uint32_t index_base, uint32_t *visible, uint32_t *count,
                            void *scratch);

int clapgpu_entities_lod(void *stream, const clapgpu_entities *e, const uint32_t *visible,
                         const uint32_t *count, uint32_t index_base, const float cam_pos[3],
                         const int32_t *force_lod, int32_t *cur_lod, int32_t *draw_lod);
int clapgpu_visible_compact_lod(void *stream, const clapgpu_entities *e, uint32_t index_base, const float cam_pos[3],
                                const int32_t *force_lod, int32_t *cur_lod, uint32_t *visible, uint32_t *count,
                                int32_t *draw_lod, void *scratch);


int clapgpu_shard_tile_range(const uint32_t *tile_row_start, uint32_t n_tiles, uint32_t rank, uint32_t world,
                             uint32_t *first_tile, uint32_t *end_tile);

#define CLAPGPU_EXCHANGE_ID_BYTES 128
typedef struct clapgpu_exchange clapgpu_exchange;
void clapgpu_exchange_set_library(const char *path);
int  clapgpu_exchange_available(void);
int  clapgpu_exchange_unique_id(uint8_t id[CLAPGPU_EXCHANGE_ID_BYTES]);
int  clapgpu_exchange_create(clapgpu_exchange **out, const uint8_t id[CLAPGPU_EXCHANGE_ID_BYTES], int rank, int world);
int  clapgpu_exchange_info(const clapgpu_exchange *x, int *comm_ranks, int *comm_rank, char pci_bus_id[32]);
void clapgpu_exchange_destroy(clapgpu_exchange *x);
int  clapgpu_exchange_visible(void *stream, clapgpu_exchange *x, const uint64_t *vis_mask, uint32_t n_pad,
                              uint64_t *gathered_mask, uint32_t *visible, uint32_t *visible_count, void *scratch);
int  clapgpu_exchange_visible_ranges(void *stream, clapgpu_exchange *x, const uint64_t *vis_mask, uint32_t cap_pad,
                                     const uint32_t *base, const uint32_t *n_pad, uint64_t *gathered_mask,
                                     uint32_t *visible, uint32_t *visible_count, void *scratch);
int  clapgpu_visible_compact_ranges(void *stream, const uint64_t *gathered_mask, uint32_t n_ranges, uint32_t cap_pad,
                                    const uint32_t *base, const uint32_t *n_pad, uint32_t *visible, uint32_t *count, void *scratch);
uint32_t clapgpu_visible_expand_ranges_host(const uint64_t *gathered_mask, uint32_t n_ranges, uint32_t cap_pad,
                                            const uint32_t *base, const uint32_t *n_pad, uint32_t *visible, uint32_t capacity);
int  clapgpu_shard_bases(const uint32_t *tile_row_start, uint32_t n_tiles, uint32_t world, uint32_t *base, uint32_t *n_pad,
                         uint32_t *cap_pad);


#define CLAPGPU_PART_DIST_LIN     0
#define CLAPGPU_PART_DIST_SQRT    1
#define CLAPGPU_PART_DIST_CBRT    2
#define CLAPGPU_PART_DIST_POW075  3

typedef struct clapgpu_particle_system {
    float    center[3];
    uint32_t dist;
    double   radius, min_radius, radius_squared, velocity;
    uint32_t first, count;
    uint32_t pad[2];
} clapgpu_particle_system;

#define CLAPGPU_RESPAWN_GROUP_WORDS 132
typedef struct clapgpu_particles {
    uint32_t  n;
    uint32_t  n_sys;
    const clapgpu_particle_system *sys;
    const uint32_t *row_sys;
    float    *pos;
    float    *vel;
    uint64_t *rng_state;
    float    *billboard_mx;
    uint64_t *respawn_mask;
    uint8_t  *respawn_row_pop;
    uint32_t *respawn_list;
    uint32_t *respawn_count;
    void     *scratch;
    uint32_t *respawn_groups;
} clapgpu_particles;

int clapgpu_particles_update(void *stream, const clapgpu_particles *p, const float view_mx[16]);


typedef struct clapgpu_skeleton {
    uint32_t        nr_joints;
    uint32_t        n_levels;
    const int32_t  *parent;
    const int32_t  *depth;
    const float    *root_pose;
    const float    *invmx;
    const float    *bind;
} clapgpu_skeleton;

typedef struct clapgpu_animations {
    uint32_t        n_anims;
    uint32_t        n_times;
    const uint32_t *chan_table;
    const float    *times;
    const float    *data;
    const void     *packed;
    uint32_t        packed_keys, packed_layout;
    uint32_t        n_data, pad;
} clapgpu_animations;

size_t clapgpu_animations_packed_bytes(uint32_t n_anims, uint32_t max_keys, uint32_t nr_joints);
int    clapgpu_animations_pack(void *stream, const clapgpu_animations *an, uint32_t nr_joints, uint32_t max_keys, void *packed,
                               uint32_t *packed_layout);

#define CLAPGPU_POSE_SKIP_TRS        (1u << 0)
#define CLAPGPU_POSE_SKIP_JOINT_POS  (1u << 1)
#define CLAPGPU_POSE_JOINT_POS_MODEL (1u << 2)
typedef struct clapgpu_pose_batch {
    uint32_t        n_chars;
    uint32_t        skip;
    const uint32_t *anim;
    const float    *frame_time;
    const uint32_t *entity;
    const float    *entity_mx;
    float          *trs;
    float          *joint_transforms;
    float          *joint_pos;
} clapgpu_pose_batch;

typedef struct clapgpu_anim_clock {
    uint32_t        n_chars;
    uint32_t        n_anims;
    const uint32_t *anim;
    const float    *time_end;
    double         *ani_time;
    const float    *speed;
    const uint8_t  *restart;
    float          *frame_time;
    uint8_t        *ended;
} clapgpu_anim_clock;
int clapgpu_animation_time(void *stream, const clapgpu_anim_clock *clk, double now);
int clapgpu_animation_time_dev(void *stream, const clapgpu_anim_clock *clk, const double *now_dev);

int clapgpu_pose_update(void *stream, const clapgpu_skeleton *sk, const clapgpu_animations *an,
                        const clapgpu_pose_batch *pb);
int clapgpu_joint_pos_world(void *stream, const clapgpu_skeleton *sk, const clapgpu_pose_batch *pb);


typedef struct clapgpu_skin_batch {
    uint32_t        n_chars;
    uint32_t        nr_joints;
    const uint32_t *vert_first;
    const uint32_t *vert_count;
    const uint32_t *out_first;
    const float    *position;
    const float    *normal;
    const uint8_t  *joints;
    const float    *weights;
    const float    *joint_transforms;
    float          *out_position;
    float          *out_normal;
    float          *out_w;
} clapgpu_skin_batch;

int clapgpu_skin(void *stream, const clapgpu_skin_batch *b);


#define CLAPGPU_BODY_DISABLED      (1u << 0)
#define CLAPGPU_BODY_AUTO_DISABLE  (1u << 1)
#define CLAPGPU_BODY_NO_GRAVITY    (1u << 2)

typedef struct clapgpu_world {
    double  gravity[3];
    double  linear_damping;
    double  linear_damping_threshold_sq;
    double  adis_linear_threshold_sq;
    double  adis_angular_threshold_sq;
    double  adis_time;
    int32_t adis_steps;
    int32_t pad;
} clapgpu_world;

#define CLAPGPU_BODY_GYROSCOPIC    (1u << 3)
#define CLAPGPU_BODY_HAS_JOINT     (1u << 4)
#define CLAPGPU_GEOM_SPHERE  0
#define CLAPGPU_GEOM_CAPSULE 1
#define CLAPGPU_GEOM_BOX     2
#define CLAPGPU_GEOM_OTHER   3

typedef struct clapgpu_bodies {
    uint32_t        n;
    uint32_t        adis_average_samples;
    double         *pos;
    double         *quat;
    double         *lvel;
    double         *avel;
    const double   *mass;
    const double   *radius;
    const double   *yoffset;
    uint32_t       *bflags;
    int32_t        *adis_steps_left;
    double         *adis_time_left;
    const int32_t  *body_entity;
    const double   *length;
    const double   *inertia;
    double          geom_offset_R[12];
    double         *aabb;
    double         *axis;
    double         *adis_samples;
    uint32_t       *adis_counter;
    double         *geom_records;
} clapgpu_bodies;

void clapgpu_geom_offset_rotation(double R[12]);
void clapgpu_mass_sphere_total(double total_mass, double radius, double I[3]);
void clapgpu_mass_capsule_total(double total_mass, int direction, double radius, double length, double I[3]);
void clapgpu_capsule_geom(float X, float Y, float Z, double geom_radius, double geom_offset,
                          float *radius, float *length, float *yoffset, int *direction, float *ray_off);
int clapgpu_bodies_aabb(void *stream, const clapgpu_bodies *b);

int  clapgpu_phys_step_schedule(double *time_acc, double dt);
void clapgpu_world_defaults(clapgpu_world *w);

int clapgpu_bodies_step(void *stream, const clapgpu_bodies *b, const clapgpu_world *w, double h);
struct clapgpu_bp;
int clapgpu_bodies_step_prebin(void *stream, const clapgpu_bodies *b, const clapgpu_world *w, double h, struct clapgpu_bp *bp);
int clapgpu_bp_invalidate(void *stream, struct clapgpu_bp *bp);

int clapgpu_phys_body_update(void *stream, const clapgpu_bodies *b, uint32_t n_entities, float *pos_scale,
                             float *rot, uint32_t *entity_flags, uint8_t *moving);

int clapgpu_bodies_rotate_from_entities(void *stream, const clapgpu_bodies *b, const clapgpu_entities *e,
                                        uint32_t mode, uint32_t n_links, const uint32_t *link_body,
                                        const uint32_t *link_entity);

#define CLAPGPU_CONTACT_BOUNCE   0x004
#define CLAPGPU_CONTACT_SOFT_ERP 0x008
#define CLAPGPU_CONTACT_SOFT_CFM 0x010
typedef struct clapgpu_contact {
    double   pos[3], normal[3], depth;
    double   mu, bounce, bounce_vel, soft_erp, soft_cfm;
    uint32_t mode;
    uint32_t nc;
} clapgpu_contact;
int clapgpu_contacts_spheres(void *stream, const clapgpu_bodies *b, const uint32_t *pairs,
                             const uint32_t *pair_total, uint32_t capacity, const double *material,
                             clapgpu_contact *contacts, uint32_t *contact_total);
int clapgpu_contacts_sphere_box(void *stream, const clapgpu_bodies *b, uint32_t n_static,
                                const double *static_aabb, const uint32_t *pairs, const uint32_t *pair_total,
                                uint32_t capacity, const double *material, const double *static_material,
                                clapgpu_contact *contacts, uint32_t *contact_total);

typedef struct clapgpu_bp clapgpu_bp;
int  clapgpu_bp_create(clapgpu_bp **out, uint32_t n_max, double cell, uint32_t n_static, const double *static_aabb_host);
void clapgpu_bp_destroy(clapgpu_bp *bp);
int  clapgpu_bp_collide(void *stream, clapgpu_bp *bp, uint32_t n, const double *aabb,
                        uint32_t *pairs, uint32_t capacity, uint32_t *pair_total,
                        uint32_t *static_pairs, uint32_t static_capacity, uint32_t *static_pair_total);
int  clapgpu_bp_status(void *stream, clapgpu_bp *bp, uint32_t *status);
const double *clapgpu_bp_static_aabb(const clapgpu_bp *bp);

typedef struct clapgpu_geoms {
// ... 162 lines not shown
```

Baseline: 22.44 billion entity updates/s.

## Fuse ordered visible-list compaction into tiled entity update via decoupled lookback

Adds a list-producing variant of the tiled entity update kernel. Each wave counts its visible entities from the cull ballots, publishes the count through a decoupled-lookback prefix scan shared with physics (moved into a common header), and writes its ordered visible indices directly. compact_visible then skips its separate compaction kernel when the fused list already matches. The aim is to remove one launch and one reread of the visibility masks. In exchange, tiles now wait on each other through a cross-tile prefix chain, the kernel gains register pressure, and the new path is only taken when fused_list is enabled.

```diff
diff --git a/clap_amd/_lib.py b/clap_amd/_lib.py
--- a/clap_amd/_lib.py
+++ b/clap_amd/_lib.py
@@ -5,7 +5,7 @@
 _HERE = os.path.dirname(os.path.abspath(__file__))
 LIB_PATH = os.environ.get("CLAPGPU_LIB") or os.path.join(_HERE, "lib", "libclapgpu.so")
 CSRC = os.path.join(_HERE, "csrc")
-ABI_VERSION = 34
+ABI_VERSION = 35
 
 OK = 0
 ERR_NOMEM = -1
@@ -55,6 +55,11 @@
                 ("host_vis_mask", C.c_void_p * EXTRA_VIEWS_MAX)]
 
 
+class VisibleOut(C.Structure):
+    _fields_ = [("visible", C.c_void_p), ("count", C.c_void_p), ("index_base", C.c_uint32), ("pad", C.c_uint32),
+                ("state", C.c_void_p)]
+
+
 class Entities(C.Structure):
     _fields_ = [("n", C.c_uint32), ("n_models", C.c_uint32),
                 ("pos_scale", C.c_void_p), ("rot", C.c_void_p), ("parent", C.c_void_p),
@@ -64,7 +69,7 @@
                 ("vis_row_pop", C.c_void_p), ("n_attach", C.c_uint32), ("pad", C.c_uint32),
                 ("attach", C.c_void_p), ("jt_pool", C.c_void_p), ("bind_pool", C.c_void_p),
                 ("attach_local", C.c_void_p), ("bv", C.POINTER(BvQuery)), ("rebuilt_mask", C.c_void_p),
-                ("views", C.POINTER(Views))]
+                ("views", C.POINTER(Views)), ("list", C.POINTER(VisibleOut))]
 
 
 class Particles(C.Structure):
@@ -214,6 +219,7 @@
                                        C.POINTER(C.c_float), C.c_void_p, C.c_void_p, C.c_void_p]),
     "clapgpu_entities_cull": (C.c_int, [C.c_void_p, C.POINTER(Entities), C.POINTER(Frustum)]),
     "clapgpu_visible_scratch_bytes": (C.c_size_t, [C.c_uint32]),
+    "clapgpu_visible_state_bytes": (C.c_size_t, [C.c_uint32]),
     "clapgpu_visible_compact": (C.c_int, [C.c_void_p, C.c_void_p, C.c_void_p, C.c_uint32, C.c_uint32, C.c_void_p,
                                           C.c_void_p, C.c_void_p]),
     "clapgpu_animation_time": (C.c_int, [C.c_void_p, C.POINTER(AnimClock), C.c_double]),
diff --git a/clap_amd/csrc/entities.hip b/clap_amd/csrc/entities.hip
--- a/clap_amd/csrc/entities.hip
+++ b/clap_amd/csrc/entities.hip
@@ -4,95 +4,9 @@
 #include "common.h"
 #include "lm_dev.h"
 #include "entities_row.h"
+#include "entities_tile_row.h"
 
 namespace clapgpu {
-
-template <bool CULL, bool XV = false>
-__device__ __forceinline__ void process_row_fast(const EntK &e, const RowIn &in, float4 *tile, const float4 *mt,
-                                                 const int lane, const uint32_t row_first, const uint32_t mode,
-                                                 const lmd::FrustumK &fr, const int src, const uint32_t parent_seq_now,
-                                                 float (&carry_mx)[16], uint32_t &carry_seq, const XViewsK *xv = nullptr)
-{
-    const uint32_t i = row_first + lane;
-    const uint32_t fl = in.fl;
-    const int32_t p = in.p;
-    uint32_t seq = in.sq & 0xffffu, pseq = in.sq >> 16;
-    float pm[16];
-#pragma unroll
-    for (int k = 0; k < 16; k++) pm[k] = __shfl(carry_mx[k], src);
-    if (p >= 0) pseq = parent_seq_now;
-
-    const float4 lo = mt[2 * in.mi], hi = mt[2 * in.mi + 1];
-    float mx[16], inv[16], bb[6], ctr[3], local_mx[16];
-    lmd::trs(local_mx, in.ps.x, in.ps.y, in.ps.z, in.ps.w, in.q.x, in.q.y, in.q.z, in.q.w);
-    if (p >= 0) {
-        lmd::mul(mx, pm, local_mx);
-    } else {
-#pragma unroll
-        for (int k = 0; k < 16; k++) mx[k] = local_mx[k];
-    }
-#ifdef CLAPGPU_EXP_NO_INVERT
-#pragma unroll
-    for (int k = 0; k < 16; k++) inv[k] = mx[k];
-#else
-    lmd::invert(inv, mx);
-#endif
-#ifdef CLAPGPU_EXP_NO_AABB
-#pragma unroll
-    for (int k = 0; k < 6; k++) bb[k] = mx[12 + k % 3] + (k < 3 ? lo.x : hi.x);
-#pragma unroll
-    for (int k = 0; k < 3; k++) ctr[k] = mx[12 + k];
-#else
-    lmd::world_aabb(bb, ctr, mx, lo.x, lo.y, lo.z, hi.x, hi.y, hi.z);
-#endif
-    seq = (seq + 1) & 0xffffu;
-#pragma unroll
-    for (int k = 0; k < 16; k++) carry_mx[k] = mx[k];
-    carry_seq = seq;
-
-    const size_t e0 = row_first;
-    float4 *tile_a = tile, *tile_b = tile + 256;
-    float *tile_f = reinterpret_cast<float *>(tile);
-    float4 va[4], vb[4];
-    stage_mat4(tile_a, mx, lane);
-    stage_mat4(tile_b, inv, lane);
-    wave_lds_fence();
-    unstage_mat4(tile_a, va, lane);
-    unstage_mat4(tile_b, vb, lane);
-    store_mat4_rows(e.mx + 16 * e0, va, lane, WAVE);
-    store_mat4_rows(e.inv_mx + 16 * e0, vb, lane, WAVE);
-    e.seqs[i] = seq | (pseq << 16);
-    wave_lds_fence();
-    stage_rows<6>(tile_f, bb, lane);
-    wave_lds_fence();
-    {
-        float *ab = e.aabb + 6 * e0;
-        store_stream(&reinterpret_cast<float4 *>(ab)[lane], reinterpret_cast<const float4 *>(tile_f)[lane]);
-        const float2 t2 = reinterpret_cast<const float2 *>(tile_f + 4 * WAVE)[lane];
-        const clapgpu_f2 v2 = { t2.x, t2.y };
-        const clapgpu_f3 v3 = { ctr[0], ctr[1], ctr[2] };
-#ifdef CLAPGPU_PLAIN_STORES
-        reinterpret_cast<clapgpu_f2 *>(ab + 4 * WAVE)[lane] = v2;
-        *reinterpret_cast<clapgpu_f3 *>(e.center + 3 * (e0 + lane)) = v3;
-#else
-        __builtin_nontemporal_store(v2, reinterpret_cast<clapgpu_f2 *>(ab + 4 * WAVE) + lane);
-        __builtin_nontemporal_store(v3, reinterpret_cast<clapgpu_f3 *>(e.center + 3 * (e0 + lane)));
-#endif
-    }
-    wave_lds_fence();
-    if (!(mode & CLAPGPU_UPDATE_ALL_DIRTY) && (fl & CLAPGPU_E_DIRTY))
-        e.flags[i] = fl & ~CLAPGPU_E_DIRTY;
-    if (e.rebuilt_mask && lane == 0) e.rebuilt_mask[row_first >> 6] = ~0ull;
-    if (CULL) {
-        bool vis = (fl & CLAPGPU_E_VISIBLE) != 0;
-        if (vis && !(fl & CLAPGPU_E_SKIP_CULLING))
-            vis = lmd::aabb_in_frustum_fast(fr, bb);
-        const uint64_t m = __ballot(vis);
-        e.vis_mask[e0 >> 6] = m;
-        e.vis_row_pop[e0 >> 6] = (uint8_t)__popcll(m);
-        if constexpr (XV) cull_extra_views(*xv, (fl & CLAPGPU_E_VISIBLE) != 0, fl, bb, (uint32_t)(e0 >> 6), lane);
-    }
-}
 
 __global__ __launch_bounds__(ENT_BLOCK)
 void k_attach_prepare(EntK e)
@@ -133,8 +47,6 @@
                              false, 0, carry_mx, carry_seq, carry_valid);
 }
 
-constexpr int ENT_MT_CAP = 256;
-constexpr int ENT_TILE_WAVES = 1;
 template <bool CULL>
 __global__ __launch_bounds__(ENT_BLOCK, ENT_TILE_WAVES)
 void k_entities_tiles(lmd::FrustumK fr_arg, EntK e, const uint32_t *tile_row_start, uint32_t n_tiles, uint32_t n,
@@ -142,7 +54,9 @@
 {
 #define TILES_XV 0
 #define TILES_XV_PTR nullptr
+#define TILES_LIST 0
 #include "entities_tiles_body.inc"
+#undef TILES_LIST
 #undef TILES_XV
 #undef TILES_XV_PTR
 }
@@ -154,7 +68,9 @@
     constexpr bool CULL = true;
 #define TILES_XV 1
 #define TILES_XV_PTR (&xv)
+#define TILES_LIST 0
 #include "entities_tiles_body.inc"
+#undef TILES_LIST
 #undef TILES_XV
 #undef TILES_XV_PTR
 }
@@ -766,7 +682,12 @@
     const dim3 grid((n_tiles + per_block - 1) / per_block), block(ENT_BLOCK);
     if (frustum && xv.n)
         hipLaunchKernelGGL(k_entities_tiles_xv, grid, block, 0, as_stream(stream), fr, k, tile_row_start, n_tiles, e->n, mode, xv);
-    else if (frustum)
+    else if (frustum && e->list) {
+        const clapgpu_visible_out *l = e->list;
+        if (!l->visible || !l->count || !l->state || (reinterpret_cast<uintptr_t>(l->state) & 7u))
+            return CLAPGPU_ERR_INVALID_ARGUMENTS;
+        return launch_entities_tiles_list(as_stream(stream), fr, k, tile_row_start, n_tiles, e->n, mode, *l);
+    } else if (frustum)
         hipLaunchKernelGGL(k_entities_tiles<true>, grid, block, 0, as_stream(stream), fr, k, tile_row_start, n_tiles,
                            e->n, mode);
     else
@@ -900,6 +821,11 @@
     return CLAPGPU_OK;
 }
 
+extern "C" size_t clapgpu_visible_state_bytes(uint32_t n_tiles)
+{
+    return ((size_t)n_tiles + 1 + WAVE) * sizeof(uint64_t);
+}
+
 extern "C" size_t clapgpu_visible_scratch_bytes(uint32_t n)
 {
     const uint32_t n_groups = (n + GROUP_WORDS * 64 - 1) / (GROUP_WORDS * 64);
diff --git a/clap_amd/csrc/entities_list.hip b/clap_amd/csrc/entities_list.hip
--- /dev/null
+++ b/clap_amd/csrc/entities_list.hip
@@ -0,0 +1,40 @@
+#include <type_traits>
+#include "common.h"
+#include "lm_dev.h"
+#include "entities_row.h"
+#include "entities_tile_row.h"
+
+namespace clapgpu {
+
+constexpr int ENT_LIST_LB_K = 32;
+__global__ __launch_bounds__(ENT_BLOCK, ENT_TILE_WAVES)
+void k_entities_tiles_list(lmd::FrustumK fr_arg, EntK e, const uint32_t *tile_row_start, uint32_t n_tiles, uint32_t n,
+                           uint32_t mode, ListK lk)
+{
+    constexpr bool CULL = true;
+#define TILES_XV 0
+#define TILES_XV_PTR nullptr
+#define TILES_LIST 1
+#include "entities_tiles_body.inc"
+#undef TILES_LIST
+#undef TILES_XV
+#undef TILES_XV_PTR
+}
+
+template <class F> struct list_first_param;
+template <class R, class A0, class... A> struct list_first_param<R (*)(A0, A...)> { using type = A0; };
+static_assert(std::is_same<list_first_param<decltype(&k_entities_tiles_list)>::type, lmd::FrustumK>::value,
+              "k_entities_tiles_list: the frustum must stay the first kernel argument (it is read at kernarg offset 0)");
+
+int launch_entities_tiles_list(hipStream_t stream, const lmd::FrustumK &fr, const EntK &e, const uint32_t *tile_row_start,
+                               uint32_t n_tiles, uint32_t n, uint32_t mode, const clapgpu_visible_out &l)
+{
+    const ListK lk = { l.visible, l.count, static_cast<uint64_t *>(l.state), l.index_base, n };
+    const uint32_t per_block = ENT_BLOCK / WAVE;
+    hipLaunchKernelGGL(k_entities_tiles_list, dim3((n_tiles + per_block - 1) / per_block), dim3(ENT_BLOCK), 0, stream, fr, e,
+                       tile_row_start, n_tiles, n, mode, lk);
+    CLAPGPU_LAUNCH_CHECK("k_entities_tiles_list");
+    return CLAPGPU_OK;
+}
+
+}
diff --git a/clap_amd/csrc/entities_row.h b/clap_amd/csrc/entities_row.h
--- a/clap_amd/csrc/entities_row.h
+++ b/clap_amd/csrc/entities_row.h
@@ -195,7 +195,7 @@
                                             const bool have_prev, const uint32_t prev_first,
                                             float (&carry_mx)[16], uint32_t &carry_seq, bool &carry_valid,
                                             const HostIO *hio = nullptr, const RowPre *pre = nullptr,
-                                            const XViewsK *xv = nullptr)
+                                            const XViewsK *xv = nullptr, uint64_t *vis_out = nullptr)
 {
     const bool in_range = (uint32_t)lane < row_count;
     const uint32_t i = row_first + (in_range ? lane : 0);
@@ -393,6 +393,7 @@
         if (vis && !(fl & CLAPGPU_E_SKIP_CULLING))
             vis = lmd::aabb_in_frustum_fast(fr, bb);
         const uint64_t m = __ballot(vis);
+        if (vis_out) *vis_out = m;
         if (lane == 0) {
             e.vis_mask[e0 >> 6] = m;
             e.vis_row_pop[e0 >> 6] = (uint8_t)__popcll(m);
@@ -455,4 +456,7 @@
 int launch_entities_tiles_host(hipStream_t stream, bool cull, const lmd::FrustumK &fr, const EntK &e, const HostIO &h,
                                const uint32_t *tile_row_start, uint32_t n_tiles, uint32_t n, uint32_t mode, const XViewsK &xv);
 
-}
+int launch_entities_tiles_list(hipStream_t stream, const lmd::FrustumK &fr, const EntK &e, const uint32_t *tile_row_start,
+                               uint32_t n_tiles, uint32_t n, uint32_t mode, const clapgpu_visible_out &list);
+
+}
diff --git a/clap_amd/csrc/entities_tile_row.h b/clap_amd/csrc/entities_tile_row.h
--- /dev/null
+++ b/clap_amd/csrc/entities_tile_row.h
@@ -0,0 +1,138 @@
+#pragma once
+#include "entities_row.h"
+#include "lookback.h"
+
+namespace clapgpu {
+
+constexpr int ENT_MT_CAP = 256;
+constexpr int ENT_TILE_WAVES = 1;
+
+struct ListK {
+    uint32_t *visible, *count;
+    uint64_t *state;
+    uint32_t index_base, cap;
+};
+
+struct TileList {
+    uint64_t  keep;
+    uint32_t  cnt;
+    uint32_t  k;
+    uint32_t  t, epoch;
+    uint64_t *words;
+    bool      last;
+    bool      published;
+
+    __device__ __forceinline__ void note(const uint64_t m, const int lane)
+    {
+        if ((uint32_t)lane == k) keep = m;
+        cnt += (uint32_t)__popcll(m);
+        k++;
+    }
+    __device__ __forceinline__ void publish()
+    {
+        lb_publish(words, t, cnt, epoch);
+        published = true;
+    }
+};
+
+template <bool CULL, bool XV = false, bool LIST = false>
+__device__ __forceinline__ void process_row_fast(const EntK &e, const RowIn &in, float4 *tile, const float4 *mt,
+                                                 const int lane, const uint32_t row_first, const uint32_t mode,
+                                                 const lmd::FrustumK &fr, const int src, const uint32_t parent_seq_now,
+                                                 float (&carry_mx)[16], uint32_t &carry_seq, const XViewsK *xv = nullptr,
+                                                 TileList *tl = nullptr)
+{
+    const uint32_t i = row_first + lane;
+    const uint32_t fl = in.fl;
+    const int32_t p = in.p;
+    uint32_t seq = in.sq & 0xffffu, pseq = in.sq >> 16;
+    float pm[16];
+#pragma unroll
+    for (int k = 0; k < 16; k++) pm[k] = __shfl(carry_mx[k], src);
+    if (p >= 0) pseq = parent_seq_now;
+
+    const float4 lo = mt[2 * in.mi], hi = mt[2 * in.mi + 1];
+    float mx[16], inv[16], bb[6], ctr[3], local_mx[16];
+    lmd::trs(local_mx, in.ps.x, in.ps.y, in.ps.z, in.ps.w, in.q.x, in.q.y, in.q.z, in.q.w);
+    if (p >= 0) {
+        lmd::mul(mx, pm, local_mx);
+    } else {
+#pragma unroll
+        for (int k = 0; k < 16; k++) mx[k] = local_mx[k];
+    }
+#ifdef CLAPGPU_EXP_NO_INVERT
+#pragma unroll
+    for (int k = 0; k < 16; k++) inv[k] = mx[k];
+#else
+    lmd::invert(inv, mx);
+#endif
+#ifdef CLAPGPU_EXP_NO_AABB
+#pragma unroll
+    for (int k = 0; k < 6; k++) bb[k] = mx[12 + k % 3] + (k < 3 ? lo.x : hi.x);
+#pragma unroll
+    for (int k = 0; k < 3; k++) ctr[k] = mx[12 + k];
+#else
+    lmd::world_aabb(bb, ctr, mx, lo.x, lo.y, lo.z, hi.x, hi.y, hi.z);
+#endif
+    seq = (seq + 1) & 0xffffu;
+#pragma unroll
+    for (int k = 0; k < 16; k++) carry_mx[k] = mx[k];
+    carry_seq = seq;
+
+    uint64_t m_list = 0;
+    if constexpr (LIST) {
+        bool vis = (fl & CLAPGPU_E_VISIBLE) != 0;
+        if (vis && !(fl & CLAPGPU_E_SKIP_CULLING))
+            vis = lmd::aabb_in_frustum_fast(fr, bb);
+        m_list = __ballot(vis);
+        tl->note(m_list, lane);
+        if (tl->last) tl->publish();
+    }
+    const size_t e0 = row_first;
+    float4 *tile_a = tile, *tile_b = tile + 256;
+    float *tile_f = reinterpret_cast<float *>(tile);
+    float4 va[4], vb[4];
+    stage_mat4(tile_a, mx, lane);
+    stage_mat4(tile_b, inv, lane);
+    wave_lds_fence();
+    unstage_mat4(tile_a, va, lane);
+    unstage_mat4(tile_b, vb, lane);
+    store_mat4_rows(e.mx + 16 * e0, va, lane, WAVE);
+    store_mat4_rows(e.inv_mx + 16 * e0, vb, lane, WAVE);
+    e.seqs[i] = seq | (pseq << 16);
+    wave_lds_fence();
+    stage_rows<6>(tile_f, bb, lane);
+    wave_lds_fence();
+    {
+        float *ab = e.aabb + 6 * e0;
+        store_stream(&reinterpret_cast<float4 *>(ab)[lane], reinterpret_cast<const float4 *>(tile_f)[lane]);
+        const float2 t2 = reinterpret_cast<const float2 *>(tile_f + 4 * WAVE)[lane];
+        const clapgpu_f2 v2 = { t2.x, t2.y };
+        const clapgpu_f3 v3 = { ctr[0], ctr[1], ctr[2] };
+#ifdef CLAPGPU_PLAIN_STORES
+        reinterpret_cast<clapgpu_f2 *>(ab + 4 * WAVE)[lane] = v2;
+        *reinterpret_cast<clapgpu_f3 *>(e.center + 3 * (e0 + lane)) = v3;
+#else
+        __builtin_nontemporal_store(v2, reinterpret_cast<clapgpu_f2 *>(ab + 4 * WAVE) + lane);
+        __builtin_nontemporal_store(v3, reinterpret_cast<clapgpu_f3 *>(e.center + 3 * (e0 + lane)));
+#endif
+    }
+    wave_lds_fence();
+    if (!(mode & CLAPGPU_UPDATE_ALL_DIRTY) && (fl & CLAPGPU_E_DIRTY))
+        e.flags[i] = fl & ~CLAPGPU_E_DIRTY;
+    if (e.rebuilt_mask && lane == 0) e.rebuilt_mask[row_first >> 6] = ~0ull;
+    if constexpr (LIST) {
+        e.vis_mask[e0 >> 6] = m_list;
+        e.vis_row_pop[e0 >> 6] = (uint8_t)__popcll(m_list);
+    } else if (CULL) {
+        bool vis = (fl & CLAPGPU_E_VISIBLE) != 0;
+        if (vis && !(fl & CLAPGPU_E_SKIP_CULLING))
+            vis = lmd::aabb_in_frustum_fast(fr, bb);
+        const uint64_t m = __ballot(vis);
+        e.vis_mask[e0 >> 6] = m;
+        e.vis_row_pop[e0 >> 6] = (uint8_t)__popcll(m);
+        if constexpr (XV) cull_extra_views(*xv, (fl & CLAPGPU_E_VISIBLE) != 0, fl, bb, (uint32_t)(e0 >> 6), lane);
+    }
+}
+
+}
diff --git a/clap_amd/csrc/entities_tiles_body.inc b/clap_amd/csrc/entities_tiles_body.inc
--- a/clap_amd/csrc/entities_tiles_body.inc
+++ b/clap_amd/csrc/entities_tiles_body.inc
@@ -15,6 +15,15 @@
         for (uint32_t k = threadIdx.x; k < 2 * e.n_models; k += ENT_BLOCK) mt_lds[k] = e.model_table[k];
     __syncthreads();
     const uint32_t t = blockIdx.x * (ENT_BLOCK / WAVE) + wave;
+#if TILES_LIST
+    if (t >= n_tiles)
+        return;
+    uint32_t *const list_ctl = reinterpret_cast<uint32_t *>(lk.state);
+    TileList tl;
+    tl.keep = 0; tl.cnt = 0; tl.k = 0; tl.t = t; tl.words = lk.state + 1 + WAVE; tl.last = false; tl.published = false;
+    tl.epoch = __hip_atomic_load(&list_ctl[0], __ATOMIC_RELAXED, __HIP_MEMORY_SCOPE_AGENT);
+    [&]() {
+#endif
     if (t >= n_tiles)
         return;
     const uint32_t n_rows = (n + WAVE - 1) / WAVE;
@@ -57,8 +66,14 @@
             const RowIn nxt = load_row(e, lane, nfirst, ncount);
             frustum_ptr frr = frp;
             asm volatile("" : "+s"(frr));
+#if TILES_LIST
+            tl.last = !more;
+            process_row_fast<CULL, false, true>(e, cur, lds_tiles[wave], mt_lds, lane, row_first, mode, *(const lmd::FrustumK *)frr, src, parent_seq_now,
+                                                carry_mx, carry_seq, nullptr, &tl);
+#else
             process_row_fast<CULL, TILES_XV != 0>(e, cur, lds_tiles[wave], mt_lds, lane, row_first, mode, *(const lmd::FrustumK *)frr, src, parent_seq_now,
                                        carry_mx, carry_seq, TILES_XV_PTR);
+#endif
             carry_valid = true;
             if (!more)
                 return;
@@ -77,8 +92,15 @@
         const RowIn nxt = load_row(e, lane, nfirst, ncount);
         frustum_ptr frr = frp;
         asm volatile("" : "+s"(frr));
+#if TILES_LIST
+        uint64_t m_row = 0;
+        process_row<CULL, true, false, false>(e, cur, lds_tiles[wave], lane, row_first, row_count, mode, *(const lmd::FrustumK *)frr,
+                                              have_prev, row_first - WAVE, carry_mx, carry_seq, carry_valid, nullptr, nullptr, nullptr, &m_row);
+        tl.note(m_row, lane);
+#else
         process_row<CULL, true, false, TILES_XV != 0>(e, cur, lds_tiles[wave], lane, row_first, row_count, mode, *(const lmd::FrustumK *)frr,
                                            have_prev, row_first - WAVE, carry_mx, carry_seq, carry_valid, nullptr, nullptr, TILES_XV_PTR);
+#endif
         if (!more)
             break;
         have_prev = true;
@@ -87,3 +109,34 @@
         row_first = nfirst;
         row_count = ncount;
     }
+#if TILES_LIST
+    }();
+    if (!tl.published) tl.publish();
+    const uint32_t excl = t ? lb_look_back<ENT_LIST_LB_K, true>(tl.words, t, tl.epoch, &list_ctl[1]) : 0u;
+    lb_publish_prefix(tl.words, t, excl + tl.cnt, tl.epoch);
+    const uint32_t list_row0 = tile_row_start[t];
+    if (tl.k > (uint32_t)WAVE)
+        __builtin_amdgcn_s_waitcnt(0);
+    uint32_t list_base = excl;
+    for (uint32_t k = 0; k < tl.k; k++) {
+        uint64_t wk;
+        if (k < (uint32_t)WAVE)
+            wk = (uint64_t)(uint32_t)__builtin_amdgcn_readlane((uint32_t)tl.keep, k) |
+                 ((uint64_t)(uint32_t)__builtin_amdgcn_readlane((uint32_t)(tl.keep >> 32), k) << 32);
+        else {
+            const uint64_t v = __hip_atomic_load(&e.vis_mask[list_row0 + k], __ATOMIC_RELAXED, __HIP_MEMORY_SCOPE_AGENT);
+            wk = (uint64_t)(uint32_t)__builtin_amdgcn_readfirstlane((uint32_t)v) |
+                 ((uint64_t)(uint32_t)__builtin_amdgcn_readfirstlane((uint32_t)(v >> 32)) << 32);
+        }
+        if (wk == 0) continue;
+        if ((wk >> lane) & 1ull) {
+            const uint32_t slot = list_base + __popcll(wk & ((1ull << lane) - 1ull));
+            if (slot < lk.cap) lk.visible[slot] = lk.index_base + (list_row0 + k) * 64u + lane;
+        }
+        list_base += (uint32_t)__popcll(wk);
+    }
+    if (t == n_tiles - 1 && lane == 0) {
+        *lk.count = excl + tl.cnt;
+        __hip_atomic_store(&list_ctl[0], tl.epoch + 1u, __ATOMIC_RELAXED, __HIP_MEMORY_SCOPE_AGENT);
+    }
+#endif
diff --git a/clap_amd/csrc/lookback.h b/clap_amd/csrc/lookback.h
--- /dev/null
+++ b/clap_amd/csrc/lookback.h
@@ -0,0 +1,81 @@
+#pragma once
+#include "common.h"
+
+namespace clapgpu {
+
+constexpr uint64_t LB_AGG = 1ull << 62, LB_PREFIX = 2ull << 62, LB_FLAGS = 3ull << 62;
+constexpr uint32_t LB_STATUS_TIMEOUT = 4u;
+__device__ __forceinline__ uint64_t lb_word(uint64_t flag, uint32_t epoch, uint32_t value)
+{
+    return flag | ((uint64_t)(epoch & 0x3fffffffu) << 32) | value;
+}
+
+__device__ __forceinline__ void lb_publish(uint64_t *state, uint32_t b, uint32_t sum, uint32_t epoch)
+{
+    if (lane_id() == 0)
+        __hip_atomic_store(&state[b], lb_word(b ? LB_AGG : LB_PREFIX, epoch, sum), __ATOMIC_RELAXED, __HIP_MEMORY_SCOPE_AGENT);
+}
+
+template <int K = 1, bool PAD = false>
+__device__ __forceinline__ uint32_t lb_look_back(const uint64_t *state, uint32_t b, uint32_t epoch, uint32_t *status)
+{
+    const int lane = lane_id();
+    uint32_t excl = 0;
+    for (int64_t top = (int64_t)b - 1; top >= 0; top -= WAVE * K) {
+        uint64_t w[K];
+#pragma unroll
+        for (int j = 0; j < K; j++) {
+            const int64_t t = top - j * WAVE - lane;
+            w[j] = 0;
+            if (top - j * WAVE >= 0)
+                w[j] = __hip_atomic_load(&state[PAD || t >= 0 ? t : 0], __ATOMIC_RELAXED, __HIP_MEMORY_SCOPE_AGENT);
+        }
+        uint32_t v = 0;
+        bool found = false;
+#pragma unroll
+        for (int j = 0; j < K; j++) {
+            const int64_t t = top - j * WAVE - lane;
+            if (found || top - j * WAVE < 0) continue;
+            uint64_t x = 0;
+            if (t >= 0) {
+                uint32_t spins = 0;
+                x = w[j];
+                for (;;) {
+                    if ((x & LB_FLAGS) && (uint32_t)((x >> 32) & 0x3fffffffu) == (epoch & 0x3fffffffu)) break;
+                    x = 0;
+                    __builtin_amdgcn_s_sleep(1);
+                    if (++spins >= (1u << 22)) break;
+                    x = __hip_atomic_load(&state[t], __ATOMIC_RELAXED, __HIP_MEMORY_SCOPE_AGENT);
+                }
+                if (!x) atomicOr(status, LB_STATUS_TIMEOUT);
+            }
+            const uint64_t is_prefix = __ballot((x & LB_FLAGS) == LB_PREFIX);
+            const int stop = is_prefix ? __builtin_ctzll(is_prefix) : WAVE - 1;
+            v += lane <= stop ? (uint32_t)x : 0u;
+            found = is_prefix != 0;
+        }
+#pragma unroll
+        for (int o = 32; o > 0; o >>= 1) v += __shfl_xor(v, o);
+        excl += v;
+        if (found) break;
+    }
+    return excl;
+}
+
+__device__ __forceinline__ void lb_publish_prefix(uint64_t *state, uint32_t b, uint32_t incl, uint32_t epoch)
+{
+    if (b && lane_id() == 0)
+        __hip_atomic_store(&state[b], lb_word(LB_PREFIX, epoch, incl), __ATOMIC_RELAXED, __HIP_MEMORY_SCOPE_AGENT);
+}
+
+__device__ __forceinline__ uint32_t lb_exclusive(uint64_t *state, uint32_t b, uint32_t sum, uint32_t epoch, uint32_t *status)
+{
+    lb_publish(state, b, sum, epoch);
+    if (b == 0)
+        return 0;
+    const uint32_t excl = lb_look_back<1>(state, b, epoch, status);
+    lb_publish_prefix(state, b, excl + sum, epoch);
+    return excl;
+}
+
+}
diff --git a/clap_amd/csrc/physics2.hip b/clap_amd/csrc/physics2.hip
--- a/clap_amd/csrc/physics2.hip
+++ b/clap_amd/csrc/physics2.hip
@@ -4,6 +4,7 @@
 #include "common.h"
 #include "phys_dev.h"
 #include "bp_grid.h"
+#include "lookback.h"
 
 namespace clapgpu {
 
@@ -301,45 +302,6 @@
     k.rank[i] = atomicAdd(&k.cell_cnt[slot], 1u);
 }
 
-constexpr uint64_t LB_AGG = 1ull << 62, LB_PREFIX = 2ull << 62, LB_FLAGS = 3ull << 62;
-__device__ __forceinline__ uint64_t lb_word(uint64_t flag, uint32_t epoch, uint32_t value)
-{
-    return flag | ((uint64_t)(epoch & 0x3fffffffu) << 32) | value;
-}
-
-__device__ __forceinline__ uint32_t lb_exclusive(uint64_t *state, uint32_t b, uint32_t sum, uint32_t epoch, uint32_t *status)
-{
-    const int lane = lane_id();
-    if (b == 0) {
-        if (lane == 0) __hip_atomic_store(&state[0], lb_word(LB_PREFIX, epoch, sum), __ATOMIC_RELAXED, __HIP_MEMORY_SCOPE_AGENT);
-        return 0;
-    }
-    if (lane == 0) __hip_atomic_store(&state[b], lb_word(LB_AGG, epoch, sum), __ATOMIC_RELAXED, __HIP_MEMORY_SCOPE_AGENT);
-    uint32_t excl = 0;
-    for (int64_t top = (int64_t)b - 1; top >= 0; top -= WAVE) {
-        const int64_t t = top - lane;
-        uint64_t w = 0;
-        if (t >= 0) {
-            uint32_t spins = 0;
-            do {
-                w = __hip_atomic_load(&state[t], __ATOMIC_RELAXED, __HIP_MEMORY_SCOPE_AGENT);
-                if ((w & LB_FLAGS) && (uint32_t)((w >> 32) & 0x3fffffffu) == (epoch & 0x3fffffffu)) break;
-                w = 0;
-                __builtin_amdgcn_s_sleep(1);
-            } while (++spins < (1u << 22));
-            if (!w) atomicOr(status, 4u);
-        }
-        const uint64_t is_prefix = __ballot(t >= 0 && (w & LB_FLAGS) == LB_PREFIX);
-        const int stop = is_prefix ? __builtin_ctzll(is_prefix) : WAVE - 1;
-        uint32_t v = (t >= 0 && lane <= stop) ? (uint32_t)w : 0u;
-#pragma unroll
-        for (int o = 32; o > 0; o >>= 1) v += __shfl_xor(v, o);
-        excl += v;
-        if (is_prefix) break;
-    }
-    if (lane == 0) __hip_atomic_store(&state[b], lb_word(LB_PREFIX, epoch, excl + sum), __ATOMIC_RELAXED, __HIP_MEMORY_SCOPE_AGENT);
-    return excl;
-}
 
 constexpr int BP_CELLS_BLOCK = 1024;
 __global__ __launch_bounds__(BP_CELLS_BLOCK)
diff --git a/clap_amd/csrc/runtime.hip b/clap_amd/csrc/runtime.hip
--- a/clap_amd/csrc/runtime.hip
+++ b/clap_amd/csrc/runtime.hip
@@ -7,9 +7,9 @@
 #include "lm_dev.h"
 
 #ifdef CLAPGPU_EXPERIMENT
-#define CLAPGPU_ABI_VERSION (34u | 0x80000000u)
+#define CLAPGPU_ABI_VERSION (35u | 0x80000000u)
 #else
-#define CLAPGPU_ABI_VERSION 34u
+#define CLAPGPU_ABI_VERSION 35u
 #endif
 
 namespace clapgpu {
diff --git a/clap_amd/entities.py b/clap_amd/entities.py
--- a/clap_amd/entities.py
+++ b/clap_amd/entities.py
@@ -85,9 +85,22 @@
             seqs=self.seqs.data_ptr(), mx=self.mx.data_ptr(), inv_mx=self.inv_mx.data_ptr(),
             aabb=self.aabb.data_ptr(), center=self.center.data_ptr(), vis_mask=self.vis_mask.data_ptr(),
             vis_row_pop=self.vis_row_pop.data_ptr())
+        self._list_for = None
+        self.fused_list = False
+        self._list_base = 0
+        if self.tiled and self.n > 0 and self.n_tiles > 0:
+            nstate = _lib.lib().clapgpu_visible_state_bytes(self.n_tiles)
+            self.list_state = torch.zeros(((nstate + 7) // 8,), dtype=torch.int64, device=dev)
+            self._list = _lib.VisibleOut(visible=self.visible.data_ptr(), count=self.visible_count.data_ptr(), index_base=0,
+                                         state=self.list_state.data_ptr())
+
+    def list_status(self):
+        return (int(self.list_state[0].item()) >> 32) & 0xFFFFFFFF if hasattr(self, "list_state") else 0
 
     def use_vis_buffers(self, vis_mask, vis_row_pop):
         self.vis_mask, self.vis_row_pop = vis_mask, vis_row_pop
+        self.fused_list = False
+        self._list_for = None
         self._desc.vis_mask = vis_mask.data_ptr()
         self._desc.vis_row_pop = vis_row_pop.data_ptr()
 
@@ -104,8 +117,11 @@
             self.view_masks.append(m); self.view_row_pops.append(p)
             self._views.vis_mask[v] = m.data_ptr(); self._views.vis_row_pop[v] = p.data_ptr()
         self._desc.views = C.pointer(self._views) if frusta else None
+        if frusta:
+            self._list_for = None
 
     def compact_view(self, v, index_base=0):
+        self._list_for = None
         rc = _lib.lib().clapgpu_visible_compact(_stream(), _ptr(self.view_masks[v]), _ptr(self.view_row_pops[v]), self.n,
                                                 index_base, _ptr(self.visible), _ptr(self.visible_count), _ptr(self.scratch))
         _lib.check(rc, "clapgpu_visible_compact")
@@ -147,9 +163,18 @@
         mode = _lib.UPDATE_ALL_DIRTY if all_dirty else 0
         fr = C.byref(frustum) if frustum is not None else None
         if self.tiled:
+            fused = bool(self.fused_list and hasattr(self, "_list") and fr is not None and not self._desc.views)
+            if fused:
+                self._list.index_base = self._list_base
+                self._desc.list = C.pointer(self._list)
+            else:
+                self._desc.list = None
+            self._list_for = None
             rc = _lib.lib().clapgpu_entities_update_tiles(_stream(), C.byref(self._desc), _ptr(self.tile_row_start),
                                                           self.n_tiles, mode, fr)
             _lib.check(rc, "clapgpu_entities_update_tiles")
+            if fused:
+                self._list_for = (self._list_base, self.vis_mask.data_ptr())
         else:
             rc = _lib.lib().clapgpu_entities_update(_stream(), C.byref(self._desc), self._ls_ptr, self.n_levels,
                                                     mode, fr)
@@ -159,15 +184,21 @@
         first = int(self.level_start[level])
         count = int(self.level_start[level + 1]) - first
         mode = _lib.UPDATE_ALL_DIRTY if all_dirty else 0
+        self._list_for = None
         rc = _lib.lib().clapgpu_entities_update_level(_stream(), C.byref(self._desc), first, count, mode,
                                                       C.byref(frustum) if frustum is not None else None)
         _lib.check(rc, "clapgpu_entities_update_level")
 
     def cull(self, frustum):
+        self._list_for = None
         rc = _lib.lib().clapgpu_entities_cull(_stream(), C.byref(self._desc), C.byref(frustum))
         _lib.check(rc, "clapgpu_entities_cull")
 
     def compact_visible(self, index_base=0, two_pass=False):
+        self._list_base = int(index_base)
+        if not two_pass and self._list_for == (self._list_base, self.vis_mask.data_ptr()):
+            return
+        self._list_for = None
         rc = _lib.lib().clapgpu_visible_compact(_stream(), _ptr(self.vis_mask),
                                                 None if two_pass else _ptr(self.vis_row_pop), self.n, index_base,
                                                 _ptr(self.visible), _ptr(self.visible_count), _ptr(self.scratch))
@@ -191,6 +222,7 @@
 
     def compact_visible_lod(self, cam_pos, force_lod=None, index_base=0):
         self.alloc_lod()
+        self._list_for = None
         if force_lod is not None:
             self.force_lod = torch.from_numpy(np.ascontiguousarray(force_lod, np.int32)).to(self.device)
         cp = (C.c_float * 3)(*[float(v) for v in cam_pos])
diff --git a/clap_amd/frame.py b/clap_amd/frame.py
--- a/clap_amd/frame.py
+++ b/clap_amd/frame.py
@@ -125,6 +125,8 @@
         import ctypes as C
         from . import _lib
         f = self._desc or self._build()
+        self.batch._desc.list = None
+        self.batch._list_for = None
         if self.lights is not None:
             self.lights._upload()
         f.now_dev = self.characters.now_dev.data_ptr() if (now is None and self.characters is not None) else None
diff --git a/include/clapgpu.h b/include/clapgpu.h
--- a/include/clapgpu.h
+++ b/include/clapgpu.h
@@ -74,6 +74,15 @@
     uint8_t        *vis_row_pop[CLAPGPU_EXTRA_VIEWS_MAX];
     uint64_t       *host_vis_mask[CLAPGPU_EXTRA_VIEWS_MAX];
 } clapgpu_views;
+
+typedef struct clapgpu_visible_out {
+    uint32_t *visible;
+    uint32_t *count;
+    uint32_t  index_base;
+    uint32_t  pad;
+    void     *state;
+} clapgpu_visible_out;
+size_t clapgpu_visible_state_bytes(uint32_t n_tiles);
 
 typedef struct clapgpu_entities {
     uint32_t        n;
@@ -100,6 +109,7 @@
     const clapgpu_bv_query *bv;
     uint64_t       *rebuilt_mask;
     const clapgpu_views *views;
+    const clapgpu_visible_out *list;
 } clapgpu_entities;
 
 #define CLAPGPU_UPDATE_ALL_DIRTY  (1u << 0)
```

Measured after the change: 22.10 billion entity updates/s. 0.985x the previous value.
